# AdeeshKolluru/AdsorbDiff

Hardware: AMD Instinct MI355X
Metric: sampled adsorbate sites/sec (50 denoise steps, ~200-atom slabs) (higher is better)
Workload: dtype f32 (f16x3-split MFMA, fp32 accumulate; ADF_GEMM=f32 selects exact f32)

## Files before the change

adsorbdiff_amd/build.py:

```python
from __future__ import annotations

import os
import shutil
import subprocess
from pathlib import Path

PKG = Path(__file__).resolve().parent
CSRC = PKG / "csrc"
LIB = PKG / "libadsorbdiff_hip.so"
SOURCES = ["api.hip", "gemm.hip", "gemm16.hip", "graph.hip", "message.hip", "message_bwd.hip", "message_geo.hip", "energy_grad.hip", "rbf_wgrad.hip", "nodewise.hip", "stepper.hip", "peaks.hip", "collect.hip", "frames.hip", "train.hip", "optimizer.hip", "noising.hip", "s2ef_train.hip", "evaluate.hip", "incremental.hip", "eqv2_kernels.hip", "eqv2_gemm16.hip", "eqv2_api.hip", "lbfgs.hip", "active.hip", "anomaly.hip", "placement.hip", "unique.hip", "symmetry.hip", "sites.hip", "triangulate.hip", "voronoi.hip"]


def _hipcc() -> str:
    for cand in (os.environ.get("HIPCC"), shutil.which("hipcc"), "/opt/rocm/bin/hipcc"):
        if cand and Path(cand).exists():
            return cand
    raise RuntimeError("hipcc not found (set HIPCC or install ROCm)")


def needs_build() -> bool:
    if not LIB.exists():
        return True
    t = LIB.stat().st_mtime
    deps = [CSRC / s for s in SOURCES] + sorted(CSRC.glob("*.h")) + [PKG.parent / "include" / "adsorbdiff_hip.h"]
    return any(d.stat().st_mtime > t for d in deps)


FLAGS = [
    "--offload-arch=gfx950", "-O3", "-std=c++17", "-fPIC",
    "-fno-slp-vectorize",
]
EXTRA_FLAGS = {
    "lbfgs.hip": ["-ffp-contract=off"],
}
OBJ_DIR = CSRC / "build"


def _compile_one(args):
    cc, src, obj = args
    res = subprocess.run([cc, *FLAGS, *EXTRA_FLAGS.get(src.name, []), "-c", str(src), "-o", str(obj)],
                         capture_output=True, text=True)
    return src.name, res.returncode, res.stdout + res.stderr


def build(force: bool = False, verbose: bool = False) -> Path:
    if not force and not needs_build():
        return LIB
    from concurrent.futures import ThreadPoolExecutor

    cc = _hipcc()
    OBJ_DIR.mkdir(exist_ok=True)
    hdr_t = max([p.stat().st_mtime for p in CSRC.glob("*.h")] + [(PKG.parent / "include" / "adsorbdiff_hip.h").stat().st_mtime,
                                                                  Path(__file__).stat().st_mtime])
    jobs, objs = [], []
    for s in SOURCES:
        src, obj = CSRC / s, OBJ_DIR / (s + ".o")
        objs.append(obj)
        if force or not obj.exists() or obj.stat().st_mtime < max(src.stat().st_mtime, hdr_t):
            jobs.append((cc, src, obj))
    if verbose:
        print("compiling:", [j[1].name for j in jobs])
    with ThreadPoolExecutor(max_workers=min(8, max(1, len(jobs)))) as ex:
        for name, rc, out in ex.map(_compile_one, jobs):
            if rc != 0:
                raise RuntimeError(f"hipcc failed on {name}:\n{out}")
    res = subprocess.run([cc, "--offload-arch=gfx950", "-shared", "-fPIC", "-o", str(LIB)] + [str(o) for o in objs],
                         capture_output=True, text=True)
    if res.returncode != 0:
        raise RuntimeError(f"link failed:\n{res.stdout}\n{res.stderr}")
    return LIB


if __name__ == "__main__":
    print(build(force=True, verbose=True))
```

adsorbdiff_amd/csrc/api.hip:

```cpp
#include <stdarg.h>
#include <stdlib.h>
#include <string.h>

#include <new>

#include "common.h"

static thread_local char g_err[512] = "";

void adf_set_error(const char* fmt, ...) {
    va_list ap;
    va_start(ap, fmt);
    vsnprintf(g_err, sizeof(g_err), fmt, ap);
    va_end(ap);
}

extern "C" const char* adf_last_error(void) { return g_err; }
extern "C" const char* adf_version(void) { return "adsorbdiff_hip 0.5.0 (gfx950)"; }

adf_tune adf_tune_from_env() {
    auto off_is_0 = [](const char* name) { const char* e = getenv(name); return (e && atoi(e) == 0) ? 0 : 1; };
    auto is_f32 = [](const char* name) { const char* e = getenv(name); return e && strcmp(e, "f32") == 0; };
    adf_tune t = {};
    t.gemm_stream = off_is_0("ADF_GEMM_STREAM");
    t.head_gate_fused = off_is_0("ADF_HEAD_GATE_FUSED");
    t.lift_emit = off_is_0("ADF_LIFT_EMIT");
    t.graph_sys_csr = off_is_0("ADF_GRAPH_SYS_CSR");
    t.train_gemm16 = is_f32("ADF_TRAIN_GEMM") ? 0 : 1;
    t.wgrad_f32 = is_f32("ADF_WGRAD") ? 1 : 0;
    const char* gt = getenv("ADF_EQV2_GEMM_TILE");
    t.eqv2_gemm_tile256 = (gt && atoi(gt) == 128) ? 0 : 1;
    t.eqv2_rotin_generic = getenv("ADF_EQV2_ROTIN_GENERIC") != nullptr;
    t.eqv2_rotout_generic = getenv("ADF_EQV2_ROTOUT_GENERIC") != nullptr;
    return t;
}
const adf_tune& adf_tune_process() {
    static const adf_tune t = adf_tune_from_env();
    return t;
}
int adf_current_num_cus() {
    int dev = 0, n = 0;
    if (hipGetDevice(&dev) != hipSuccess || hipDeviceGetAttribute(&n, hipDeviceAttributeMultiprocessorCount, dev) != hipSuccess) return 0;
    return n;
}

extern "C" int32_t adf_profile_enable(adf_painn_t h, int32_t on) {
    if (!h) { adf_set_error("null handle"); return ADF_EINVAL; }
    h->prof.enable(on != 0);
    ADF_HIP_CHECK(hipMemset(h->kcount, 0, 8 * sizeof(unsigned long long)));
    return ADF_OK;
}

extern "C" int32_t adf_profile_read(adf_painn_t h, float* ms, int64_t* count, int64_t* message_ksteps, void* stream) {
    if (!h || !ms || !count) { adf_set_error("null argument"); return ADF_EINVAL; }
    ADF_HIP_CHECK(hipStreamSynchronize((hipStream_t)stream));
    if (message_ksteps) {
        unsigned long long k[8];
        ADF_HIP_CHECK(hipMemcpy(k, h->kcount, sizeof(k), hipMemcpyDeviceToHost));
        ADF_HIP_CHECK(hipMemset(h->kcount, 0, sizeof(k)));
        *message_ksteps = (int64_t)k[0];
    }
    return h->prof.read(ms, count, ADF_PROF_NCAT);
}

extern "C" int32_t adf_painn_create(const adf_painn_hparams* hp, adf_painn_t* out) {
    if (!hp || !out) { adf_set_error("null argument"); return ADF_EINVAL; }
    if (hp->hidden_channels % ADF_SLICE_CH != 0 || hp->hidden_channels < 128 || hp->hidden_channels > 1024) {
        adf_set_error("hidden_channels=%d must be a multiple of %d in [128,1024]", hp->hidden_channels, ADF_SLICE_CH);
        return ADF_EINVAL;
    }
    if (hp->num_rbf % 2 != 0 || hp->num_rbf > 128 || hp->num_rbf < 2) {
        adf_set_error("num_rbf=%d must be even and <= 128", hp->num_rbf);
        return ADF_EINVAL;
    }
    if (hp->max_neighbors < 1 || hp->max_neighbors > ADF_MAX_K) {
        adf_set_error("max_neighbors=%d must be in [1,%d]", hp->max_neighbors, ADF_MAX_K);
        return ADF_EINVAL;
    }
    if (hp->num_layers < 1 || hp->num_layers > 16 || hp->num_heads < 0 || hp->num_heads > 2) {
        adf_set_error("num_layers must be in [1,16], num_heads in [0,2]");
        return ADF_EINVAL;
    }
    adf_painn* h = new (std::nothrow) adf_painn();
    if (!h) { adf_set_error("host allocation failed"); return ADF_EOOM; }
    h->hp = *hp;
    hipDeviceProp_t prop;
    if (hipGetDevice(&h->device) != hipSuccess || hipGetDeviceProperties(&prop, h->device) != hipSuccess) {
        adf_set_error("no usable HIP device: %s", hipGetErrorString(hipGetLastError()));
        adf_painn_destroy(h);
        return ADF_EHIP;
    }
    h->num_cus = prop.multiProcessorCount;
    h->dist_floor = 1.0e-3f;
    {
        const char* e = getenv("ADF_INCREMENTAL");
        h->inc_on = !(e && e[0] == '0');
        const char* e2 = getenv("ADF_INC_SYNC");
        h->inc_sync = e2 && e2[0] == '1';
    }
    const int H = hp->hidden_channels, R = hp->num_rbf, L = hp->num_layers;
    adf_pool& m = h->m_life;
    int32_t st = m.alloc(&h->rbf_pack, (size_t)L * (H / ADF_SLICE_CH) * R * 192);
    if (st == ADF_OK) st = m.alloc(&h->rbf_bias_pack, (size_t)L * (H / ADF_SLICE_CH) * 192);
    if (st == ADF_OK) st = m.alloc(&h->rbf_pack16, (size_t)L * (H / ADF_SLICE_CH) * R * 192 * 2 * sizeof(uint16_t));
    if (st == ADF_OK) st = m.alloc(&h->rbf_bias_pack16, (size_t)L * (H / ADF_SLICE_CH) * 192);
    if (st == ADF_OK) st = m.alloc(&h->rbf_scales, 16);
    if (st == ADF_OK) st = m.alloc(&h->flags, ADF_NFLAGS);
    if (st == ADF_OK && hipMemset(h->flags, 0, sizeof(int32_t) * ADF_NFLAGS) != hipSuccess) st = ADF_EHIP;
    {
        const size_t HH = (size_t)H * H;
        const size_t per_layer = HH + 3 * HH + 2 * HH + 2 * HH + 3 * HH;
        const size_t per_head = HH + HH / 2 + 2 * HH + HH + HH / 4 + HH / 2;
        const size_t elems = (size_t)L * per_layer + (size_t)hp->num_heads * per_head;
        h->w16_bytes = elems * 2 * sizeof(uint16_t) + 4096;
        if (st == ADF_OK) st = m.alloc(&h->w16_arena, h->w16_bytes);
        if (st == ADF_OK) st = m.alloc(&h->w16_scales, 256);
        if (st == ADF_OK) st = m.alloc(&h->w16_bias_perm, (size_t)L * 2 * 3 * H);
        if (st == ADF_OK) st = m.alloc(&h->w16_scratch, 1);
        if (st == ADF_OK) st = m.alloc(&h->wfrag_arena, h->w16_bytes);
        const char* e = getenv("ADF_GEMM");
        h->gemm_f32 = e && strcmp(e, "f32") == 0;
        const char* el = getenv("ADF_LIFT");
        h->lift_on = !(el && strcmp(el, "0") == 0);
        const char* e2 = getenv("ADF_MSG");
        h->msg_f32 = e2 ? strcmp(e2, "f32") == 0 : h->gemm_f32;
        h->msg_f32_only = hp->num_rbf % 8 != 0;
        h->msg_f32 = h->msg_f32 || h->msg_f32_only;
        const char* er = getenv("ADF_ROW_MAXIMA");
        h->rmx = (er && atoi(er) == 0) ? 0 : 1;
        h->tune = adf_tune_from_env();
    }
    if (st == ADF_OK) st = m.alloc(&h->kcount, 8);
    if (st == ADF_OK && hipMemset(h->kcount, 0, 8 * sizeof(unsigned long long)) != hipSuccess) st = ADF_EHIP;
    if (st != ADF_OK) { adf_painn_destroy(h); return st; }
    *out = h;
    return ADF_OK;
}

static void inc_free(adf_painn* h) {
    h->m_inc.release();
    h->inc_tmp_bytes = 0;
    h->inc_capN = 0; h->inc_valid = false;
}

static void free_workspaces(adf_painn* h) {
    h->m_ws.release();
    h->inc_valid = false;
    h->scan_tmp_bytes = 0;
    h->lift.cap = 0; h->mag_v3_valid = false;
    h->xpart = h->catpart = h->vpart = nullptr; h->part_stride = 0;
    h->part_x = h->part_vec = nullptr; h->dbg_msg_rows = h->dbg_cat_rows = h->dbg_comb_rows = 0; h->dbg_mag = nullptr;
    h->cache_valid = false;
    h->capN = h->capB = h->capE = 0;
}

extern "C" int32_t adf_painn_destroy(adf_painn_t h) {
    if (!h) return ADF_OK;
    if (h->inc_cnt_host) (void)hipHostFree(h->inc_cnt_host);
    for (int i = 0; i < 2; ++i)
        if (h->inc_ev[i]) (void)hipEventDestroy((hipEvent_t)h->inc_ev[i]);
    adf_grad_free(h);
    delete h;
    return ADF_OK;
}

extern "C" int32_t adf_painn_set_weights(adf_painn_t h, int32_t n_weights, const void* const* w,
                                         const float* scale_factors, void* stream) {
    if (!h || !w || !scale_factors) { adf_set_error("null argument"); return ADF_EINVAL; }
    const int L = h->hp.num_layers;
    const int expect = 2 + ADF_WEIGHTS_PER_LAYER * L + ADF_WEIGHTS_PER_HEAD * h->hp.num_heads;
    if (n_weights != expect) {
        adf_set_error("expected %d weight tensors, got %d", expect, n_weights);
        return ADF_EINVAL;
    }
    for (int i = 0; i < n_weights; ++i)
        if (!w[i]) { adf_set_error("weight %d is null", i); return ADF_EINVAL; }
    auto f = [&](int i) { return reinterpret_cast<const float*>(w[i]); };
    h->emb = f(0);
    h->rbf_offset = f(1);
    int k = 2;
    for (int l = 0; l < L; ++l) {
        adf_layer_weights& lw = h->layer[l];
        lw.ln_w = f(k++); lw.ln_b = f(k++); lw.xp0_w = f(k++); lw.xp0_b = f(k++); lw.xp2_w = f(k++); lw.xp2_b = f(k++);
        lw.rbf_w = f(k++); lw.rbf_b = f(k++); lw.vp_w = f(k++); lw.xv0_w = f(k++); lw.xv0_b = f(k++);
        lw.xv2_w = f(k++); lw.xv2_b = f(k++);
        h->scale[l] = scale_factors[l];
    }
    for (int hd = 0; hd < h->hp.num_heads; ++hd)
        for (int b = 0; b < 2; ++b) {
            adf_block_weights& bw = h->head[hd][b];
            bw.vec1_w = f(k++); bw.vec2_w = f(k++); bw.un0_w = f(k++); bw.un0_b = f(k++); bw.un2_w = f(k++);
            bw.un2_b = f(k++);
        }
    ADF_TRY(adf_pack_rbf(h, (hipStream_t)stream));
    {
        hipStream_t s = (hipStream_t)stream;
        const long long H = h->hp.hidden_channels, HH = H * H;
        unsigned char* cur = h->w16_arena;
        unsigned char* fcur = h->wfrag_arena;
        int nscale = 0;
        float* bperm = h->w16_bias_perm;
        auto split = [&](const float* w, long long rows, long long K, adf_w16* out, const float* fused_bias = nullptr,
                         bool pair_perm = false) -> int32_t {
            const long long n = rows * K;
            out->hi = cur; cur += n * 2;
            out->lo = cur; cur += n * 2;
            out->inv_scale = h->w16_scales + nscale++;
            out->bias_perm = nullptr;
            out->frag = nullptr;
            if (fused_bias) {
                out->bias_perm = bperm; bperm += 3 * H;
                ADF_TRY(adf_split_weight(w, n, out, h->w16_scratch, s, (int)H, (int)H, fused_bias));
            } else if (pair_perm) {
                ADF_TRY(adf_split_weight(w, n, out, h->w16_scratch, s, (int)H, (int)H, nullptr, 2));
            } else {
                ADF_TRY(adf_split_weight(w, n, out, h->w16_scratch, s));
            }
            if (rows % 32 == 0 && K % 16 == 0) {
                out->frag = fcur; fcur += n * 4;
                ADF_TRY(adf_pack_frag(out, (int)rows, (int)K, out->frag, s));
            }
            return ADF_OK;
        };
        for (int l = 0; l < L; ++l) {
            adf_layer_weights& lw = h->layer[l];
            ADF_TRY(split(lw.xp0_w, H, H, &lw.xp0_16));
            ADF_TRY(split(lw.xp2_w, 3 * H, H, &lw.xp2_16, lw.xp2_b));
            ADF_TRY(split(lw.vp_w, 2 * H, H, &lw.vp_16, nullptr, true));
            ADF_TRY(split(lw.xv0_w, H, 2 * H, &lw.xv0_16));
            ADF_TRY(split(lw.xv2_w, 3 * H, H, &lw.xv2_16, lw.xv2_b));
        }
        for (int hd = 0; hd < h->hp.num_heads; ++hd) {
            adf_block_weights& b0 = h->head[hd][0];
            adf_block_weights& b1 = h->head[hd][1];
            ADF_TRY(split(b0.vec1_w, H, H, &b0.vec1_16));
            ADF_TRY(split(b0.vec2_w, H / 2, H, &b0.vec2_16));
            ADF_TRY(split(b0.un0_w, H, 2 * H, &b0.un0_16));
            ADF_TRY(split(b0.un2_w, H, H, &b0.un2_16));
            ADF_TRY(split(b1.vec1_w, H / 2, H / 2, &b1.vec1_16));
            ADF_TRY(split(b1.un0_w, H / 2, H, &b1.un0_16));
        }
        if ((size_t)(cur - h->w16_arena) > h->w16_bytes || (size_t)(fcur - h->wfrag_arena) > h->w16_bytes || nscale > 256) {
            adf_set_error("internal: fp16 weight arena overflow");
            return ADF_EINVAL;
        }
    }
    h->weights_set = true;
    h->rec0_valid = false;
    h->inc_valid = false;
    adf_grad_invalidate(h);
    return ADF_OK;
}

static int32_t ensure_capacity(adf_painn* h, int64_t N, int64_t B) {
    if (N <= h->capN && B <= h->capB) return ADF_OK;
    const int64_t capN = N > h->capN ? N : h->capN;
    const int64_t capB = B > h->capB ? B : h->capB;
    ADF_HIP_CHECK(hipDeviceSynchronize());
    free_workspaces(h);
    const int64_t H = h->hp.hidden_channels, K = h->hp.max_neighbors;
    const int64_t capE = 2 * capN * K;
    int32_t st = ADF_OK;
#define ALLOC(field, count) if (st == ADF_OK) st = h->m_ws.alloc(&h->field, (size_t)(count))
    ALLOC(nbr_cnt, capN);
    ALLOC(nbr_src, capN * K);
    ALLOC(nbr_shift, capN * K);
    ALLOC(cache_d2, capN * K);
    ALLOC(cache_cid, capN * K);
    ALLOC(cache_cnt, capN);
    ALLOC(deg, capN + 1);
    ALLOC(nptr, capN + 1);
    ALLOC(cursor, capN);
    ALLOC(img_cnt, capB);
    ALLOC(sys_slow, capB);
    ALLOC(e_src, capE);
    ALLOC(e_geom, capE);
    if (h->inc_on) {
        ALLOC(prev_nptr, capN + 1);
        ALLOC(prev_src, capE);
        ALLOC(prev_geom, capE);
    }
    if (st == ADF_OK) {
        h->scan_tmp_bytes = adf_scan_temp_bytes(capN + 1);
        st = h->m_ws.alloc(&h->scan_tmp, h->scan_tmp_bytes + 16);
    }
    ALLOC(x, capN * H);
    ALLOC(vecA, capN * 3 * H);
    ALLOC(vecB, capN * 3 * H);
    ALLOC(rec, (capN + 1) * 5 * H);
    ALLOC(y, capN * H);
    ALLOC(xh, capN * 3 * H);
    ALLOC(vv, capN * 6 * H);
    ALLOC(cat, capN * 2 * H);
    ALLOC(dot, capN * H);
    ALLOC(sys, capB * 16);
    ALLOC(lift.buf, capN * 3);
    ALLOC(mag_a, capN);
    ALLOC(mag_b, capN);
    ALLOC(mag_v3, capN * 3);
    const int64_t ps = (capN + 31) / 32 * 32, ns = H / ADF_SLICE_CH;
    if (h->rmx) ALLOC(rmx_part, (4 * ns + H / 32 + 4) * ps);
#undef ALLOC
    h->lift.cap = st == ADF_OK ? capN * 3 : 0;
    if (st != ADF_OK) { free_workspaces(h); return st; }
    if (h->rmx) {
        h->part_stride = ps;
        h->xpart = h->rmx_part; h->catpart = h->xpart + ns * ps; h->vpart = h->catpart + (H / 32) * ps;
        h->dbg_mag = h->vpart + 3 * ns * ps;
    }
    h->capN = capN; h->capB = capB; h->capE = capE;
    return ADF_OK;
}

static int32_t check_batch(const adf_painn* h, const adf_batch* b) {
    if (!h || !b) { adf_set_error("null argument"); return ADF_EINVAL; }
    if (b->num_atoms <= 0 || b->num_systems <= 0) { adf_set_error("empty batch"); return ADF_EINVAL; }
    if (!b->pos || !b->cell || !b->batch || !b->atom_offset) { adf_set_error("null batch array"); return ADF_EINVAL; }
    for (int k = 0; k < 3; ++k)
        if (b->reps[k] < 0 || b->reps[k] > 16) { adf_set_error("reps[%d]=%d out of range", k, b->reps[k]); return ADF_EINVAL; }
    return ADF_OK;
}

static int32_t read_flags(adf_painn* h, hipStream_t s) {
    int32_t f[ADF_NFLAGS];
    ADF_HIP_CHECK(hipMemcpyAsync(f, h->flags, sizeof(f), hipMemcpyDeviceToHost, s));
    ADF_HIP_CHECK(hipMemsetAsync(h->flags, 0, sizeof(f), s));
    ADF_HIP_CHECK(hipStreamSynchronize(s));
    if (f[4]) { adf_set_error("atomic number outside [1, %d] (rows of the embedding table)", h->hp.num_elements); return ADF_EINVAL; }
    if (f[0]) { adf_set_error("a centre atom has more than %d in-cutoff candidates", ADF_MAX_CAND); return ADF_EOVERFLOW; }
    if (f[2]) { adf_set_error("edge buffer overflow"); return ADF_EOVERFLOW; }
    if (f[3]) { adf_set_error("an atom has more than %d incoming edges", ADF_MAX_INDEG); return ADF_EOVERFLOW; }
    if (f[1]) { adf_set_error("An image has no neighbors"); return ADF_ENONEIGHBOR; }
    if (f[6]) { adf_set_error("energy gradient: an edge row has no reverse row in its partner's segment (asymmetric graph)"); return ADF_EINVAL; }
    if (f[5]) {
        adf_set_error("non-finite model output%s", h->gemm_f32 ? " (exact-f32 arithmetic: the inputs or weights are not finite)"
                      : " in f16x3 arithmetic: an activation left the fp16 range or the inputs are not finite; "
                        "adf_painn_set_arithmetic(h, 1) selects exact f32");
        return ADF_ENUMERIC;
    }
    return ADF_OK;
}

extern "C" int32_t adf_graph_set_moving(adf_painn_t h, const int32_t* moving, const int32_t* mov_idx,
                                        const int32_t* mov_off) {
    if (!h) { adf_set_error("null handle"); return ADF_EINVAL; }
    if (moving && (!mov_idx || !mov_off)) { adf_set_error("moving mask needs mov_idx and mov_off"); return ADF_EINVAL; }
    h->moving = moving; h->mov_idx = mov_idx; h->mov_off = mov_off;
    ADF_HIP_CHECK(hipMemset(h->flags, 0, sizeof(int32_t) * ADF_NFLAGS));
    h->cache_valid = false;
    h->rec0_valid = false;
    h->inc_valid = false;
    return ADF_OK;
}

extern "C" int32_t adf_graph_build(adf_painn_t h, const adf_batch* b, void* stream, int64_t* num_edges) {
    ADF_TRY(check_batch(h, b));
    ADF_TRY(ensure_capacity(h, b->num_atoms, b->num_systems));
    hipStream_t s = (hipStream_t)stream;
    ADF_TRY(adf_graph_build_impl(h, b, s));
    if (num_edges) {
        int32_t e = 0;
        ADF_HIP_CHECK(hipMemcpyAsync(&e, h->nptr + b->num_atoms, sizeof(int32_t), hipMemcpyDeviceToHost, s));
        ADF_TRY(read_flags(h, s));
        *num_edges = e;
    }
    return ADF_OK;
}

__global__ void adf_export_edges_kernel(const int32_t* nptr, const int32_t* e_src, const float4* eg, int N,
                                        int32_t* src, int32_t* dst, float* dist, float* vec, long long cap) {
    const int n = blockIdx.x * 4 + (threadIdx.x >> 6);
    if (n >= N) return;
    for (int e = nptr[n] + (threadIdx.x & 63); e < nptr[n + 1]; e += 64) {
        if (e >= cap) continue;
        if (src) src[e] = e_src[e];
        if (dst) dst[e] = n;
        const float4 q = eg[e];
        if (dist) dist[e] = q.w;
        if (vec) { vec[3 * (size_t)e] = q.x; vec[3 * (size_t)e + 1] = q.y; vec[3 * (size_t)e + 2] = q.z; }
    }
}

__global__ void adf_export_shift_kernel(const int32_t* nbr_shift, int32_t* out, long long n, int r0, int r1, int r2) {
    const long long i = (long long)blockIdx.x * blockDim.x + threadIdx.x;
    if (i >= n) return;
    const int c = nbr_shift[i];
    const int n2 = 2 * r2 + 1, n1 = 2 * r1 + 1;
    const int ia = c / (n1 * n2), rem = c - ia * (n1 * n2);
    out[3 * i] = ia - r0;
    out[3 * i + 1] = rem / n2 - r1;
    out[3 * i + 2] = rem % n2 - r2;
}

extern "C" int32_t adf_graph_export(adf_painn_t h, int32_t* nbr_count, int32_t* nbr_src, int32_t* nbr_shift,
                                    int64_t edge_capacity, int32_t* edge_src, int32_t* edge_dst, float* edge_dist,
                                    float* edge_vec, int64_t* num_edges, void* stream) {
    if (!h || h->lastN <= 0) { adf_set_error("no graph built"); return ADF_EINVAL; }
    hipStream_t s = (hipStream_t)stream;
    const int64_t N = h->lastN, K = h->hp.max_neighbors;
    if (nbr_count) ADF_HIP_CHECK(hipMemcpyAsync(nbr_count, h->nbr_cnt, sizeof(int32_t) * N, hipMemcpyDeviceToDevice, s));
    if (nbr_src) ADF_HIP_CHECK(hipMemcpyAsync(nbr_src, h->nbr_src, sizeof(int32_t) * N * K, hipMemcpyDeviceToDevice, s));
    if (nbr_shift)
        hipLaunchKernelGGL(adf_export_shift_kernel, dim3((unsigned)((N * K + 255) / 256)), dim3(256), 0, s, h->nbr_shift,
                           nbr_shift, (long long)(N * K), h->last_reps[0], h->last_reps[1], h->last_reps[2]);
    if (edge_src || edge_dst || edge_dist || edge_vec)
        hipLaunchKernelGGL(adf_export_edges_kernel, dim3((unsigned)((N + 3) / 4)), dim3(256), 0, s, h->nptr, h->e_src,
                           h->e_geom, (int)N, edge_src, edge_dst, edge_dist, edge_vec, (long long)edge_capacity);
    ADF_HIP_CHECK(hipGetLastError());
    int32_t e = 0;
    ADF_HIP_CHECK(hipMemcpyAsync(&e, h->nptr + N, sizeof(int32_t), hipMemcpyDeviceToHost, s));
    ADF_HIP_CHECK(hipStreamSynchronize(s));
    if (num_edges) *num_edges = e;
    return ADF_OK;
}

static int32_t zero_pad_rows(adf_painn* h, int N, hipStream_t s) {
    const size_t row = (size_t)5 * h->hp.hidden_channels;
    ADF_HIP_CHECK(hipMemsetAsync(h->rec + (size_t)N * row, 0, sizeof(float) * row, s));
    return ADF_OK;
}

static int32_t make_records(adf_painn* h, int l, int n, const float* x, const float* vec, bool vec_is_zero, float* rec,
                            const int32_t* row_map, hipStream_t s) {
    const int H = h->hp.hidden_channels;
    const adf_layer_weights& w = h->layer[l];
    if (n <= 0) return ADF_OK;
    adf_prof_begin(h, ADF_PROF_NODE, s);
    const bool lift = h->lift_on && !h->gemm_f32;
    const bool em = lift && h->tune.lift_emit;
    ADF_TRY(adf_nodewise_layernorm(x, w.ln_w, w.ln_b, h->y, n, H, s, em ? h->mag_a : nullptr, h->rows_dev));
    ADF_TRY(adf_linear(h, h->y, H, w.xp0_w, &w.xp0_16, w.xp0_b, h->cat, H, n, H, H, 1, s, em ? h->mag_a : nullptr,
                       em ? h->mag_b : nullptr));
    if (h->gemm_f32) {
        if (row_map) { adf_set_error("internal: mapped records need the f16x3 path"); return ADF_EINVAL; }
        ADF_TRY(adf_launch_gemm(h->cat, H, w.xp2_w, H, w.xp2_b, h->xh, 3 * H, n, 3 * H, H, 0, s));
        ADF_TRY(adf_pack_records(h, n, h->xh, vec, vec_is_zero, s, rec));
    } else {
        adf_epi ep = {};
        ep.vec_in = vec; ep.rec = rec ? rec : h->rec; ep.H = H; ep.vec_is_zero = vec_is_zero ? 1 : 0;
        ep.row_map = row_map;
        ep.rmag = em ? h->mag_b : nullptr;
        ep.m_dev = h->rows_dev;
        ADF_TRY(adf_launch_gemm16_fused(h->cat, H, &w.xp2_16, n, H, H, 1, &ep, s, h->tune, lift ? &h->lift : nullptr));
    }
    adf_prof_end(h, s);
    return ADF_OK;
}

static int32_t message_layer(adf_painn* h, int l, int N, const float* x, const float* vec, float* x_out,
                             float* vec_out, bool vec_is_zero, hipStream_t s, const int32_t* tlist = nullptr,
                             int n_targets = 0, float* rec = nullptr, bool records_ready = false) {
    if (!records_ready) ADF_TRY(make_records(h, l, N, x, vec, vec_is_zero, rec, nullptr, s));
    adf_prof_begin(h, ADF_PROF_MESSAGE, s);
    const int items = tlist ? n_targets : N;
    const bool emit = h->rmx && h->lift_on && !h->gemm_f32 && !h->msg_f32 && items > 0 && items <= h->part_stride;
    h->part_x = h->part_vec = nullptr;
    const int32_t st = adf_message_impl(h, l, N, x, h->xh, vec, x_out, vec_out, vec_is_zero, s, tlist, n_targets, rec,
                                        tlist ? h->rows_dev : nullptr, emit ? h->xpart : nullptr, h->vpart, h->part_stride);
    if (st == ADF_OK && emit) {
        h->part_x = x_out; h->part_vec = vec_out; h->part_n = items; h->part_dev = tlist ? h->rows_dev : nullptr;
        h->dbg_msg_rows = items;
    }
    adf_prof_end(h, s);
    return st;
}

static int32_t update_layer(adf_painn* h, int l, int N, float* x, float* vec, hipStream_t s, bool from_message = true) {
    const int H = h->hp.hidden_channels;
    const adf_layer_weights& w = h->layer[l];
    adf_prof_begin(h, ADF_PROF_NODE, s);
    const bool parts = from_message && h->rmx && h->lift_on && !h->gemm_f32 && N > 0 && h->part_x == x && h->part_vec == vec &&
                       h->part_n == N && h->part_dev == h->rows_dev;
    h->part_x = h->part_vec = nullptr;
    if (h->gemm_f32) {
        ADF_TRY(adf_launch_gemm(vec, H, w.vp_w, H, nullptr, h->vv, 2 * H, 3 * N, 2 * H, H, 0, s));
        ADF_TRY(adf_nodewise_update_prep(h->vv, x, h->cat, h->dot, N, H, s));
        ADF_TRY(adf_linear(h, h->cat, 2 * H, w.xv0_w, &w.xv0_16, w.xv0_b, h->y, H, N, H, 2 * H, 1, s));
    } else {
        adf_epi ep = {};
        ep.v1 = h->vv; ep.dotw = h->dot; ep.cat = h->cat; ep.H = H; ep.m_dev = h->rows_dev;
        const adf_lift* lf = h->lift_on ? &h->lift : nullptr;
        if (parts) {
            ADF_TRY(adf_launch_rowmax_combine(h->vpart, 3 * h->part_stride, H / ADF_SLICE_CH, 3ll * N, h->lift.buf, s, h->rows_dev, 3));
            ep.rmag = h->lift.buf;
            if (h->dbg_capture) ADF_HIP_CHECK(hipMemcpyAsync(h->dbg_mag, h->lift.buf, sizeof(float) * 3 * (size_t)N, hipMemcpyDeviceToDevice, s));
        }
        if (parts || (h->dbg_capture && h->rmx && lf && N <= h->part_stride)) {
            ep.catpart = h->catpart; ep.part_stride = h->part_stride; h->dbg_cat_rows = N;
        }
        ADF_TRY(adf_launch_gemm16_fused(vec, H, &w.vp_16, N, H, H, 3, &ep, s, h->tune, lf));
        if (parts) {
            ADF_TRY(adf_launch_rowmax_combine(h->xpart, h->part_stride, H / ADF_SLICE_CH + H / 32, N, h->lift.buf, s, h->rows_dev, 1));
            if (h->dbg_capture) {
                ADF_HIP_CHECK(hipMemcpyAsync(h->dbg_mag + 3 * h->part_stride, h->lift.buf, sizeof(float) * (size_t)N, hipMemcpyDeviceToDevice, s));
                h->dbg_comb_rows = N;
            }
        }
        adf_epi e0 = {};
        e0.A2 = h->cat; e0.K1 = H; e0.m_dev = h->rows_dev;
        e0.rmag = parts ? h->lift.buf : nullptr;
        e0.out_mag = h->lift_on ? reinterpret_cast<unsigned int*>(h->mag_b) : nullptr;
        ADF_TRY(adf_launch_gemm16(x, H, &w.xv0_16, w.xv0_b, h->y, H, N, H, 2 * H, 1, &e0, s, lf, h->tune, h->num_cus));
    }
    int32_t st;
    if (h->gemm_f32) {
        ADF_TRY(adf_launch_gemm(h->y, H, w.xv2_w, H, w.xv2_b, h->xh, 3 * H, N, 3 * H, H, 0, s));
        st = adf_nodewise_update_apply(h->xh, h->dot, h->vv, x, vec, h->scale[l], N, H, s);
    } else {
        adf_epi ep = {};
// ... 158 lines not shown
    const size_t cap = (size_t)h->inc_capN, row = (size_t)5 * H;
    if (out_idx && n_out == 0) return ADF_OK;
    adf_prof_begin(h, ADF_PROF_GRAPH, s);
    if (first) {
        ADF_TRY(adf_nodewise_embed(h, Z, N, h->incX[0], s));
        for (int l = 0; l < L; ++l) ADF_HIP_CHECK(hipMemsetAsync(h->incR[l] + (size_t)N * row, 0, sizeof(float) * row, s));
        ADF_HIP_CHECK(hipMemsetAsync(h->inc_pend, 0, cap * L, s));
    } else {
        ADF_TRY(adf_inc_compare(h, N, s));
    }
    ADF_HIP_CHECK(hipMemsetAsync(h->inc_cnt, 0, sizeof(int32_t) * (2 * ADF_MAX_LAYERS + 1), s));
    if (out_idx) ADF_TRY(adf_inc_need_from_list(h, N, L, out_idx, n_out, s));
    for (int l = 0; l < L; ++l) ADF_TRY(adf_inc_plan_layer(h, l, N, first, out_idx != nullptr, s));
    ADF_HIP_CHECK(hipMemcpyAsync(h->inc_cnt + 2 * L, h->nptr + N, sizeof(int32_t), hipMemcpyDeviceToDevice, s));
    const int slot = h->inc_slot;
    h->inc_slot ^= 1;
    if (h->inc_ev_live[slot]) ADF_TRY(inc_harvest(h, slot, true));
    int32_t* host = h->inc_cnt_host + (size_t)slot * (2 * ADF_MAX_LAYERS + 1);
    ADF_HIP_CHECK(hipMemcpyAsync(host, h->inc_cnt, sizeof(int32_t) * (2 * L + 1), hipMemcpyDeviceToHost, s));
    ADF_HIP_CHECK(hipEventRecord((hipEvent_t)h->inc_ev[slot], s));
    h->inc_ev_live[slot] = true;
    h->inc_pend_N[slot] = N;
    ADF_TRY(inc_harvest(h, slot ^ 1, false));
    if (h->inc_sync) ADF_TRY(inc_harvest(h, slot, true, true));
    adf_prof_end(h, s);
    if (first) ADF_TRY(make_records(h, 0, N, h->incX[0], nullptr, true, h->incR[0], nullptr, s));
    for (int l = 0; l < L; ++l) {
        const int n_seen = h->inc_seen_valid ? h->inc_seen[l] : N;
        const bool whole = first || !h->inc_seen_valid || h->inc_pend_Nseen != N || (long long)n_seen * 10 >= (long long)N * 9;
        h->inc_pend_whole[slot][l] = whole ? 1 : 0;
        if (h->inc_sync && !whole && n_seen == 0) continue;
        const float* vin = l == 0 ? h->vecA : h->incV[l];
        if (whole) {
            ADF_TRY(message_layer(h, l, N, h->incX[l], vin, h->incX[l + 1], h->incV[l + 1], l == 0, s, nullptr, 0,
                                  h->incR[l], true));
            ADF_TRY(update_layer(h, l, N, h->incX[l + 1], h->incV[l + 1], s));
            if (l + 1 < L)
                ADF_TRY(make_records(h, l + 1, N, h->incX[l + 1], h->incV[l + 1], false, h->incR[l + 1], nullptr, s));
            continue;
        }
        const int32_t* list = h->inc_list + cap * l;
        const int ncap = h->inc_sync ? n_seen : N;
        h->rows_dev = h->inc_cnt + l;
        int32_t st = message_layer(h, l, N, h->incX[l], vin, h->x, h->vecB, l == 0, s, list, ncap, h->incR[l], true);
        if (st == ADF_OK) st = update_layer(h, l, ncap, h->x, h->vecB, s);
        if (st == ADF_OK) {
            adf_prof_begin(h, ADF_PROF_NODE, s);
            st = adf_inc_scatter_rows(h->x, list, ncap, H, h->incX[l + 1], s, h->rows_dev);
            if (st == ADF_OK) st = adf_inc_scatter_rows(h->vecB, list, ncap, 3 * H, h->incV[l + 1], s, h->rows_dev);
            adf_prof_end(h, s);
        }
        if (st == ADF_OK && l + 1 < L) st = make_records(h, l + 1, ncap, h->x, h->vecB, false, h->incR[l + 1], list, s);
        h->rows_dev = nullptr;
        ADF_TRY(st);
    }
    adf_prof_begin(h, ADF_PROF_HEADS, s);
    if (!out_idx) {
        if (heads >= 1) ADF_TRY(adf_head_forward(h, 0, N, h->incX[L], h->incV[L], f1, s));
        if (heads == 2) ADF_TRY(adf_head_forward(h, 1, N, h->incX[L], h->incV[L], f2, s));
        h->x_last = h->incX[L];
    } else {
        ADF_TRY(ensure_subset(h, n_out));
        ADF_TRY(adf_inc_gather_rows(h->incX[L], out_idx, n_out, H, h->sub_x, s));
        ADF_TRY(adf_inc_gather_rows(h->incV[L], out_idx, n_out, 3 * H, h->sub_vec, s));
        for (int hd = 0; hd < heads; ++hd) {
            ADF_TRY(adf_head_forward(h, hd, n_out, h->sub_x, h->sub_vec, h->sub_f, s));
            hipLaunchKernelGGL(adf_scatter_rows3_kernel, dim3((3 * n_out + 255) / 256), dim3(256), 0, s, h->sub_f, out_idx,
                               n_out, hd == 0 ? f1 : f2);
        }
        ADF_HIP_CHECK(hipGetLastError());
    }
    adf_prof_end(h, s);
    h->inc_valid = true;
    return ADF_OK;
}

static int32_t forward_impl(adf_painn_t h, const adf_batch* b, const int32_t* out_idx, int32_t n_out, float* f1,
                            float* f2, void* stream, bool head1_only = false) {
    ADF_TRY(check_batch(h, b));
    if (!h->weights_set) { adf_set_error("weights not set"); return ADF_EINVAL; }
    const int heads = head1_only ? 1 : h->hp.num_heads;
    if (heads > h->hp.num_heads) { adf_set_error("the model has no force head"); return ADF_EINVAL; }
    if (!b->atomic_numbers || (heads >= 1 && !f1) || (heads == 2 && !f2)) { adf_set_error("null argument"); return ADF_EINVAL; }
    h->x_last = nullptr;
    hipStream_t s = (hipStream_t)stream;
    const int N = b->num_atoms;
    ADF_TRY(ensure_capacity(h, N, b->num_systems));
    const int inc = inc_prepare(h, N);
    adf_prof_begin(h, ADF_PROF_GRAPH, s);
    ADF_TRY(adf_graph_build_impl(h, b, s));
    adf_prof_end(h, s);
    if (inc) {
        h->inc_serial = h->build_serial;
        return forward_incremental(h, N, b->atomic_numbers, out_idx, n_out, f1, f2, inc == 2, heads, s);
    }
    ADF_TRY(zero_pad_rows(h, N, s));
    ADF_TRY(adf_nodewise_embed(h, b->atomic_numbers, N, h->x, s));
    float* vin = h->vecA;
    float* vout = h->vecB;
    const int L = h->hp.num_layers, H = h->hp.hidden_channels;
    float* rec0 = nullptr;
    bool rec0_ready = false;
    if (h->moving) {
        const size_t row = (size_t)5 * H;
        if ((int64_t)N + 1 > h->rec0_cap) {
            h->rec0_cap = 0; h->rec0_valid = false;
            ADF_TRY(h->m_rec0.alloc(&h->rec0, ((size_t)N + 1) * row));
            h->rec0_cap = (int64_t)N + 1;
        }
        rec0 = h->rec0;
        rec0_ready = h->rec0_valid && h->rec0_N == N;
        if (!rec0_ready) ADF_HIP_CHECK(hipMemsetAsync(rec0 + (size_t)N * row, 0, sizeof(float) * row, s));
        h->rec0_valid = true; h->rec0_N = N;
    }
    if (!out_idx) {
        for (int l = 0; l < L; ++l) {
            if (l == 0) ADF_TRY(message_layer(h, 0, N, h->x, vin, h->x, vout, true, s, nullptr, 0, rec0, rec0_ready));
            else
            ADF_TRY(message_layer(h, l, N, h->x, vin, h->x, vout, l == 0, s));
            ADF_TRY(update_layer(h, l, N, h->x, vout, s));
            float* t = vin; vin = vout; vout = t;
        }
        adf_prof_begin(h, ADF_PROF_HEADS, s);
        if (heads >= 1) ADF_TRY(adf_head_forward(h, 0, N, h->x, vin, f1, s));
        if (heads == 2) ADF_TRY(adf_head_forward(h, 1, N, h->x, vin, f2, s));
        adf_prof_end(h, s);
        h->x_last = h->x;
        return ADF_OK;
    }
    if (n_out == 0) return ADF_OK;
    ADF_TRY(ensure_subset(h, n_out));
    for (int l = 0; l + 1 < L; ++l) {
        if (l == 0) ADF_TRY(message_layer(h, 0, N, h->x, vin, h->x, vout, true, s, nullptr, 0, rec0, rec0_ready));
        else
        ADF_TRY(message_layer(h, l, N, h->x, vin, h->x, vout, l == 0, s));
        ADF_TRY(update_layer(h, l, N, h->x, vout, s));
        float* t = vin; vin = vout; vout = t;
    }
    ADF_TRY(message_layer(h, L - 1, N, h->x, vin, h->sub_x, h->sub_vec, L == 1, s, out_idx, n_out,
                          L == 1 ? rec0 : nullptr, L == 1 && rec0_ready));
    ADF_TRY(update_layer(h, L - 1, n_out, h->sub_x, h->sub_vec, s));
    adf_prof_begin(h, ADF_PROF_HEADS, s);
    for (int hd = 0; hd < heads; ++hd) {
        ADF_TRY(adf_head_forward(h, hd, n_out, h->sub_x, h->sub_vec, h->sub_f, s));
        hipLaunchKernelGGL(adf_scatter_rows3_kernel, dim3((3 * n_out + 255) / 256), dim3(256), 0, s, h->sub_f, out_idx,
                           n_out, hd == 0 ? f1 : f2);
    }
    ADF_HIP_CHECK(hipGetLastError());
    adf_prof_end(h, s);
    return ADF_OK;
}

extern "C" int32_t adf_painn_forward(adf_painn_t h, const adf_batch* b, float* f1, float* f2, void* stream) {
    return forward_impl(h, b, nullptr, 0, f1, f2, stream);
}

extern "C" int32_t adf_painn_forward_subset(adf_painn_t h, const adf_batch* b, const int32_t* out_idx, int32_t n_out,
                                            float* f1, float* f2, void* stream) {
    if (!out_idx || n_out < 0) { adf_set_error("forward_subset: null index list"); return ADF_EINVAL; }
    return forward_impl(h, b, out_idx, n_out, f1, f2, stream);
}

extern "C" int32_t adf_painn_set_energy_head(adf_painn_t h, int32_t n_weights, const void* const* w, void* stream) {
    if (!h || !w) { adf_set_error("null argument"); return ADF_EINVAL; }
    if (n_weights != 4) { adf_set_error("set_energy_head: expected 4 tensors (out_energy.0.weight/bias, out_energy.2.weight/bias), got %d", n_weights); return ADF_EINVAL; }
    for (int i = 0; i < 4; ++i)
        if (!w[i]) { adf_set_error("energy-head tensor %d is null", i); return ADF_EINVAL; }
    const int H = h->hp.hidden_channels, H2 = H / 2;
    const size_t n = (size_t)H2 * H;
    if (!h->oe0_buf) ADF_TRY(h->m_life.alloc(&h->oe0_buf, n * 4 + 64));
    h->oe0_w = reinterpret_cast<const float*>(w[0]);
    h->oe0_b = reinterpret_cast<const float*>(w[1]);
    h->oe2_w = reinterpret_cast<const float*>(w[2]);
    h->oe2_b = reinterpret_cast<const float*>(w[3]);
    adf_w16& e = h->oe0_16;
    e = adf_w16{};
    e.hi = h->oe0_buf; e.lo = h->oe0_buf + n * 2; e.inv_scale = reinterpret_cast<float*>(h->oe0_buf + n * 4);
    ADF_TRY(adf_split_weight(h->oe0_w, (long long)n, &e, reinterpret_cast<unsigned int*>(h->oe0_buf + n * 4 + 16),
                             (hipStream_t)stream));
    h->energy_set = true;
    adf_grad_invalidate(h);
    return ADF_OK;
}

extern "C" int32_t adf_painn_set_distance_floor(adf_painn_t h, float floor) {
    if (!h || !(floor > 0.f)) { adf_set_error("set_distance_floor: null handle or non-positive floor"); return ADF_EINVAL; }
    if (floor != h->dist_floor) {
        h->dist_floor = floor;
        h->cache_valid = false;
        h->rec0_valid = false;
        h->inc_valid = false;
    }
    return ADF_OK;
}

__global__ __launch_bounds__(256) void adf_energy_sum_kernel(const float* __restrict__ y, int H2, const float* __restrict__ w,
                                                             const float* __restrict__ bias, const int32_t* __restrict__ atom_offset,
                                                             float* __restrict__ energy) {
    __shared__ float part[4];
    const int b = blockIdx.x, lane = threadIdx.x & 63, wave = threadIdx.x >> 6;
    const int a0 = atom_offset[b], a1 = atom_offset[b + 1];
    const float b0 = bias[0];
    float acc = 0.f;
    for (int a = a0 + wave; a < a1; a += 4) {
        const float* row = y + (size_t)a * H2;
        float d = 0.f;
        for (int c = lane; c < H2; c += 64) d = fmaf(row[c], w[c], d);
        d = adf_wave_sum(d);
        acc = __fadd_rn(acc, __fadd_rn(d, b0));
    }
    if (lane == 0) part[wave] = acc;
    __syncthreads();
    if (threadIdx.x == 0) energy[b] = __fadd_rn(__fadd_rn(part[0], part[1]), __fadd_rn(part[2], part[3]));
}

int32_t adf_energy_sum(const float* y, int H2, const float* w, const float* bias, const int32_t* atom_offset, float* energy,
                       int num_systems, hipStream_t s) {
    hipLaunchKernelGGL(adf_energy_sum_kernel, dim3(num_systems), dim3(256), 0, s, y, H2, w, bias, atom_offset, energy);
    ADF_HIP_CHECK(hipGetLastError());
    return ADF_OK;
}

extern "C" int32_t adf_painn_forward_energy(adf_painn_t h, const adf_batch* b, float* energy, float* forces, void* stream) {
    ADF_TRY(check_batch(h, b));
    if (!h->energy_set) { adf_set_error("forward_energy: energy head not set (adf_painn_set_energy_head)"); return ADF_EINVAL; }
    if (!energy || (h->hp.num_heads >= 1 && !forces)) { adf_set_error("forward_energy: null output"); return ADF_EINVAL; }
    if (h->hp.num_heads > 1) { adf_set_error("forward_energy: the S2EF model has one force head"); return ADF_EINVAL; }
    hipStream_t s = (hipStream_t)stream;
    ADF_TRY(forward_impl(h, b, nullptr, 0, forces, nullptr, stream));
    if (!h->x_last) { adf_set_error("internal: no node features after the forward"); return ADF_EINVAL; }
    const int N = b->num_atoms, H = h->hp.hidden_channels, H2 = H / 2;
    adf_prof_begin(h, ADF_PROF_HEADS, s);
    ADF_TRY(adf_linear(h, h->x_last, H, h->oe0_w, &h->oe0_16, h->oe0_b, h->y, H2, N, H2, H, 1, s));
    ADF_TRY(adf_energy_sum(h->y, H2, h->oe2_w, h->oe2_b, b->atom_offset, energy, b->num_systems, s));
    adf_prof_end(h, s);
    return ADF_OK;
}

extern "C" int32_t adf_linear_forward(const float* A, const float* W, const float* bias, float* C, int32_t M,
                                      int32_t N, int32_t K, int32_t act_ssilu, int32_t mode, void* stream) {
    hipStream_t s = (hipStream_t)stream;
    if (!A || !W || !C || M <= 0 || N <= 0 || K <= 0) { adf_set_error("bad argument"); return ADF_EINVAL; }
    if (mode == 0) return adf_launch_gemm(A, K, W, K, bias, C, N, M, N, K, act_ssilu, s);
    adf_pool tmp;
    unsigned char* buf = nullptr;
    const size_t n = (size_t)N * K;
    ADF_TRY(tmp.alloc(&buf, n * 4 + 64));
    adf_w16 w16 = {};
    w16.hi = buf; w16.lo = buf + n * 2; w16.inv_scale = reinterpret_cast<float*>(buf + n * 4);
    unsigned int* scratch = reinterpret_cast<unsigned int*>(buf + n * 4 + 16);
    int32_t st = adf_split_weight(W, (long long)n, &w16, scratch, s);
    float* mags = nullptr;
    const char* el = getenv("ADF_LIFT");
    const bool lift = !(el && strcmp(el, "0") == 0);
    if (st == ADF_OK && lift) st = tmp.alloc(&mags, (size_t)M);
    adf_lift lf = {mags, M};
    if (st == ADF_OK) st = adf_launch_gemm16(A, K, &w16, bias, C, N, M, N, K, act_ssilu, nullptr, s, lift ? &lf : nullptr,
                                             adf_tune_process(), adf_current_num_cus());
    (void)hipStreamSynchronize(s);
    return st;
}

extern "C" int32_t adf_painn_set_arithmetic(adf_painn_t h, int32_t exact_f32) {
    if (!h) { adf_set_error("null handle"); return ADF_EINVAL; }
    h->gemm_f32 = exact_f32 != 0;
    h->msg_f32 = exact_f32 != 0 || h->msg_f32_only;
    h->rec0_valid = false;
    h->inc_valid = false;
    return ADF_OK;
}

extern "C" int32_t adf_painn_set_incremental(adf_painn_t h, int32_t on) {
    if (!h) { adf_set_error("null handle"); return ADF_EINVAL; }
    if ((on != 0) != h->inc_on) {
        ADF_HIP_CHECK(hipDeviceSynchronize());
        h->inc_on = on != 0;
        if (!h->inc_on) inc_free(h);
        if (h->inc_on && h->capN > 0 && !h->prev_nptr) {
            int32_t st = h->m_ws.alloc(&h->prev_nptr, (size_t)h->capN + 1);
            if (st == ADF_OK) st = h->m_ws.alloc(&h->prev_src, (size_t)h->capE);
            if (st == ADF_OK) st = h->m_ws.alloc(&h->prev_geom, (size_t)h->capE);
            if (st != ADF_OK) { h->inc_on = false; return st; }
        }
    }
    h->inc_valid = false;
    (void)inc_harvest(h, h->inc_slot, true);
    (void)inc_harvest(h, h->inc_slot ^ 1, true);
    h->inc_seen_valid = false;
    h->inc_rows = h->inc_rows_full = h->inc_edges = h->inc_launches = 0;
    return ADF_OK;
}

extern "C" int32_t adf_check_flags(adf_painn_t h, void* stream) {
    if (!h) { adf_set_error("null handle"); return ADF_EINVAL; }
    return read_flags(h, (hipStream_t)stream);
}

static int32_t model_check(void* h, const adf_batch* b) { return check_batch((adf_painn*)h, b); }
static int32_t model_grow(void* h, const adf_batch* b, float** sys) {
    adf_painn* p = (adf_painn*)h;
    ADF_TRY(ensure_capacity(p, b->num_atoms, b->num_systems));
    *sys = p->sys;
    return ADF_OK;
}
static int32_t model_forward(void* h, const adf_batch* b, const int32_t* out_idx, int32_t n_out, float* f1, float* f2,
                             hipStream_t s) {
    return forward_impl((adf_painn*)h, b, out_idx, out_idx ? n_out : 0, f1, f2, s, !f2);
}
static void model_prof(void* h, bool begin, hipStream_t s) {
    if (begin) adf_prof_begin((adf_painn*)h, ADF_PROF_STEPPER, s);
    else adf_prof_end((adf_painn*)h, s);
}
static adf_model model(adf_painn_t h) {
    return {h, model_check, model_grow, model_forward, model_prof, h ? h->ps_state : nullptr, h ? h->ps_B : 0};
}

extern "C" int32_t adf_painn_set_per_system_stop(adf_painn_t h, int32_t* sys_state, int32_t B) {
    if (!h) { adf_set_error("null handle"); return ADF_EINVAL; }
    return adf_model_set_per_system_stop(&h->ps_state, &h->ps_B, sys_state, B);
}

extern "C" int32_t adf_sde_init_placement(adf_painn_t h, const adf_batch* b, float* pos, const int32_t* tags,
                                          const float* noise, void* stream) {
    return adf_model_init_placement(model(h), b, pos, tags, noise, (hipStream_t)stream);
}

extern "C" int32_t adf_sde_step(adf_painn_t h, const adf_batch* b, float* pos, const int32_t* tags,
                                const int32_t* fixed, const float* f1, const float* f2, const adf_step_coef* coef,
                                const float* z_tr, const float* z_rot, int32_t early_stop_count, int32_t* state,
                                float* dcom, float* drot, void* stream) {
    return adf_model_sde_step(model(h), b, pos, tags, fixed, f1, f2, coef, nullptr, 0, z_tr, z_rot, early_stop_count, state,
                              dcom, drot, (hipStream_t)stream);
}

extern "C" int32_t adf_sde_step_scheduled(adf_painn_t h, const adf_batch* b, float* pos, const int32_t* tags,
                                          const int32_t* fixed, const float* f1, const float* f2,
                                          const adf_step_coef* coefs_dev, int32_t num_steps, const float* z_tr,
                                          const float* z_rot, int32_t early_stop_count, int32_t* state, float* dcom,
                                          float* drot, void* stream) {
    return adf_model_sde_step(model(h), b, pos, tags, fixed, f1, f2, nullptr, coefs_dev, num_steps, z_tr, z_rot,
                              early_stop_count, state, dcom, drot, (hipStream_t)stream);
}

extern "C" int32_t adf_sample(adf_painn_t h, const adf_batch* b, float* pos, const int32_t* tags, const int32_t* fixed,
                              const adf_step_coef* coefs_dev, int32_t num_steps, const float* z_tr_all,
                              const float* z_rot_all, int32_t early_stop_count, int32_t poll_every, int32_t* state,
                              const int32_t* out_idx, int32_t n_out, float* f1, float* f2, void* stream) {
    return adf_model_sample(model(h), b, pos, tags, fixed, coefs_dev, num_steps, z_tr_all, z_rot_all, early_stop_count,
                            poll_every, state, out_idx, n_out, f1, f2, nullptr, 0, (hipStream_t)stream);
}

extern "C" int32_t adf_sample_traj(adf_painn_t h, const adf_batch* b, float* pos, const int32_t* tags, const int32_t* fixed,
                                   const adf_step_coef* coefs_dev, int32_t num_steps, const float* z_tr_all,
                                   const float* z_rot_all, int32_t early_stop_count, int32_t poll_every, int32_t* state,
                                   const int32_t* out_idx, int32_t n_out, float* f1, float* f2, adf_frames_t sink,
                                   int32_t frame_every, void* stream) {
    if (!sink) { adf_set_error("sample_traj: null sink"); return ADF_EINVAL; }
    return adf_model_sample(model(h), b, pos, tags, fixed, coefs_dev, num_steps, z_tr_all, z_rot_all, early_stop_count,
                            poll_every, state, out_idx, n_out, f1, f2, sink, frame_every, (hipStream_t)stream);
}

extern "C" int32_t adf_tr_step(adf_painn_t h, const adf_batch* b, float* pos, const int32_t* tags, const float* f1,
                               const adf_tr_coef* coef, const adf_tr_coef* coefs_dev, int32_t num_steps, const float* z,
                               int32_t early_stop_count, int32_t* state, float* dcom, void* stream) {
    return adf_model_tr_step(model(h), b, pos, tags, f1, coef, coefs_dev, num_steps, z, early_stop_count, state, dcom,
                             (hipStream_t)stream);
}

extern "C" int32_t adf_tr_sample(adf_painn_t h, const adf_batch* b, float* pos, const int32_t* tags,
                                 const adf_tr_coef* coefs_dev, int32_t num_steps, const float* z_all,
                                 int32_t early_stop_count, int32_t poll_every, int32_t* state, const int32_t* out_idx,
                                 int32_t n_out, float* f1, void* stream) {
    return adf_model_tr_sample(model(h), b, pos, tags, coefs_dev, num_steps, z_all, early_stop_count, poll_every, state,
                               out_idx, n_out, f1, nullptr, 0, (hipStream_t)stream);
}

extern "C" int32_t adf_tr_sample_traj(adf_painn_t h, const adf_batch* b, float* pos, const int32_t* tags,
                                      const adf_tr_coef* coefs_dev, int32_t num_steps, const float* z_all,
                                      int32_t early_stop_count, int32_t poll_every, int32_t* state, const int32_t* out_idx,
                                      int32_t n_out, float* f1, adf_frames_t sink, int32_t frame_every, void* stream) {
    if (!sink) { adf_set_error("tr_sample_traj: null sink"); return ADF_EINVAL; }
    return adf_model_tr_sample(model(h), b, pos, tags, coefs_dev, num_steps, z_all, early_stop_count, poll_every, state,
                               out_idx, n_out, f1, sink, frame_every, (hipStream_t)stream);
}

extern "C" int32_t adf_get_counters(adf_painn_t h, adf_counters* out, void* stream) {
    if (!h || !out || h->lastN <= 0) { adf_set_error("no forward has run"); return ADF_EINVAL; }
    hipStream_t s = (hipStream_t)stream;
    const int64_t N = h->lastN, H = h->hp.hidden_channels, R = h->hp.num_rbf, L = h->hp.num_layers;
    int32_t e = 0;
    ADF_HIP_CHECK(hipMemcpyAsync(&e, h->nptr + N, sizeof(int32_t), hipMemcpyDeviceToHost, s));
    ADF_HIP_CHECK(hipStreamSynchronize(s));
    const int64_t E = e;
    out->num_edges = E;
    out->num_atoms = N;
    out->message_bytes_per_layer = E * (3 * H * 4 + 12 + 8) + N * (3 * H * 4 + 3 * H * 4) + N * (H * 4 + 3 * H * 4);
    const int64_t head = 2 * (3 * N * H * H + 3 * N * H * H / 2 + N * 2 * H * H + N * H * H + 3 * N * (H / 2) * (H / 2) +
                              N * H * H / 2);
    out->dense_flops = L * (30 * H * H * N + 2 * R * 3 * H * E) + h->hp.num_heads * head;
    ADF_TRY(inc_harvest(h, h->inc_slot, true));
    ADF_TRY(inc_harvest(h, h->inc_slot ^ 1, true));
    out->inc_rows = (int64_t)h->inc_rows; out->inc_rows_full = (int64_t)h->inc_rows_full;
    out->inc_msg_launches = (int64_t)h->inc_launches; out->inc_msg_edges = (int64_t)h->inc_edges;
    return ADF_OK;
}
```

adsorbdiff_amd/csrc/base.h:

```cpp
#pragma once
#include <hip/hip_runtime.h>
#include <stdint.h>
#include <stdio.h>
#include <string>
#include <vector>

#include "../../include/adsorbdiff_hip.h"

void adf_set_error(const char* fmt, ...);

#define ADF_HIP_CHECK(expr)                                                             \
    do {                                                                                \
        hipError_t _e = (expr);                                                         \
        if (_e != hipSuccess) {                                                         \
            adf_set_error("%s failed: %s (%s:%d)", #expr, hipGetErrorString(_e),        \
                          __FILE__, __LINE__);                                          \
            return (_e == hipErrorOutOfMemory) ? ADF_EOOM : ADF_EHIP;                   \
        }                                                                               \
    } while (0)

#define ADF_TRY(expr)                     \
    do {                                  \
        int32_t _s = (expr);              \
        if (_s != ADF_OK) return _s;      \
    } while (0)

struct adf_pool {
    std::vector<void**> slots;
    adf_pool() = default;
    adf_pool(const adf_pool&) = delete;
    adf_pool& operator=(const adf_pool&) = delete;
    ~adf_pool() { release(); }
    int32_t alloc(void** field, size_t bytes) {
        bool known = false;
        for (void** s : slots) known = known || s == field;
        if (known) { if (*field) (void)hipFree(*field); } else slots.push_back(field);
        *field = nullptr;
        if (bytes == 0) bytes = 16;
        const hipError_t e = hipMalloc(field, bytes);
        if (e == hipSuccess) return ADF_OK;
        *field = nullptr;
        (void)hipGetLastError();
        adf_set_error("device allocation of %zu bytes failed: %s", bytes, hipGetErrorString(e));
        return ADF_EOOM;
    }
    template <typename T>
    int32_t alloc(T** field, size_t count) { return alloc(reinterpret_cast<void**>(field), count * sizeof(T)); }
    void release() {
        for (void** s : slots) {
            if (*s) (void)hipFree(*s);
            *s = nullptr;
        }
        slots.clear();
    }
};

struct adf_prof {
    bool on = false;
    bool open = false;
    std::vector<hipEvent_t> ev;
    std::vector<int> cat;
    size_t used = 0;
    adf_prof() = default;
    adf_prof(const adf_prof&) = delete;
    adf_prof& operator=(const adf_prof&) = delete;
    ~adf_prof() { for (hipEvent_t e : ev) (void)hipEventDestroy(e); }
    void begin(int c, hipStream_t s) {
        open = false;
        if (!on) return;
        if (used + 2 > ev.size())
            for (int i = 0; i < 512; ++i) {
                hipEvent_t e;
                if (hipEventCreate(&e) != hipSuccess) { (void)hipGetLastError(); break; }
                ev.push_back(e);
            }
        if (used + 2 > ev.size()) return;
        cat.resize(used / 2);
        cat.push_back(c);
        (void)hipEventRecord(ev[used], s);
        open = true;
    }
    void end(hipStream_t s) {
        if (!on || !open) return;
        (void)hipEventRecord(ev[used + 1], s);
        used += 2;
        open = false;
    }
    void enable(bool o) { on = o; open = false; used = 0; cat.clear(); }
    int32_t read(float* ms, int64_t* count, int ncat) {
        for (int c = 0; c < ncat; ++c) { ms[c] = 0.f; count[c] = 0; }
        for (size_t i = 0; i < used; i += 2) {
            float t = 0.f;
            ADF_HIP_CHECK(hipEventElapsedTime(&t, ev[i], ev[i + 1]));
            ms[cat[i / 2]] += t;
            count[cat[i / 2]] += 1;
        }
        enable(on);
        return ADF_OK;
    }
    struct scope {
        adf_prof& p; hipStream_t s;
        scope(adf_prof& p_, int c, hipStream_t s_) : p(p_), s(s_) { p.begin(c, s); }
        ~scope() { p.end(s); }
    };
};
```

adsorbdiff_amd/csrc/common.h:

```cpp
#pragma once
#include "base.h"
#include "arith.h"
#include "lanes.h"

#define ADF_GROUP_NODES 32
#define ADF_SLICE_CH 64
#define ADF_MAX_CAND 1024
#define ADF_MAX_K 128
#define ADF_NFLAGS 8
#define ADF_MAX_INDEG 1024
#define ADF_MAX_LAYERS 16

struct adf_w16 {
    void* hi;
    void* lo;
    float* inv_scale;
    float* bias_perm;
    void* frag;
};
struct adf_epi {
    const float* vec_in;
    float* rec;
    float* x;
    float* vec;
    const float* dot;
    const float* vv;
    float* v1;
    float* dotw;
    float* cat;
    float scale;
    int H;
    int vec_is_zero;
    const float* A2;
    int K1;
    const int32_t* row_map;
    const float* rmag;
    unsigned int* out_mag;
    const int32_t* m_dev;
    int accumulate;
    const float* gate;
    int gate_ld;
    float* catpart;
    long long part_stride;
};
struct adf_lift {
    float* buf;
    long long cap;
};
struct adf_layer_weights {
    const float *ln_w, *ln_b, *xp0_w, *xp0_b, *xp2_w, *xp2_b, *rbf_w, *rbf_b;
    const float *vp_w, *xv0_w, *xv0_b, *xv2_w, *xv2_b;
    adf_w16 xp0_16, xp2_16, vp_16, xv0_16, xv2_16;
};
struct adf_block_weights {
    const float *vec1_w, *vec2_w, *un0_w, *un0_b, *un2_w, *un2_b;
    adf_w16 vec1_16, vec2_16, un0_16, un2_16;
};

struct adf_painn {
    adf_painn_hparams hp;
    int device;
    bool weights_set;
    const float* emb;
    const float* rbf_offset;
    adf_layer_weights layer[16];
    adf_block_weights head[2][2];
    float scale[16];
    float* rbf_pack;
    float* rbf_bias_pack;
    void* rbf_pack16;
    float* rbf_bias_pack16;
    float* rbf_scales;
    unsigned char* w16_arena;
    size_t w16_bytes;
    float* w16_scales;
    float* w16_bias_perm;
    unsigned int* w16_scratch;
    unsigned char* wfrag_arena;
    bool gemm_f32;
    bool msg_f32;
    bool msg_f32_only;
    adf_tune tune;
    bool lift_on;
    adf_lift lift;
    float *mag_a, *mag_b;
    float* mag_v3;
    bool mag_v3_valid;
    int rmx;
    float* rmx_part;
    float *xpart, *catpart, *vpart;
    int64_t part_stride;
    const float *part_x, *part_vec;
    int part_n;
    const int32_t* part_dev;
    int dbg_msg_rows, dbg_cat_rows;
    bool dbg_capture;
    float* dbg_mag;
    int dbg_comb_rows;

    int64_t capN, capB, capE;
    int32_t* nbr_cnt;
    int32_t* nbr_src;
    int32_t* nbr_shift;
    int32_t* deg;
    int32_t* nptr;
    int32_t* cursor;
    int32_t* img_cnt;
    int32_t* sys_slow;
    void* scan_tmp;
    size_t scan_tmp_bytes;
    const int32_t* moving;
    const int32_t* mov_idx;
    const int32_t* mov_off;
    float* cache_d2;
    int32_t* cache_cid;
    int32_t* cache_cnt;
    bool cache_valid;
    int32_t* e_src;
    float4* e_geom;
    int32_t* flags;
    float *x, *vecA, *vecB, *y, *xh, *vv, *cat, *dot;
    float* rec;
    bool rbf_uniform;
    float* rec0;
    int64_t rec0_cap, rec0_N;
    bool rec0_valid;
    bool inc_on;
    bool inc_valid;
    int64_t inc_capN, inc_N;
    int inc_layers;
    float* incX[ADF_MAX_LAYERS + 1];
    float* incV[ADF_MAX_LAYERS + 1];
    float* incR[ADF_MAX_LAYERS];
    int32_t *prev_nptr, *prev_src;
    float4* prev_geom;
    unsigned char *inc_c0, *inc_chg;
    unsigned char *inc_pend, *inc_need, *inc_tf;
    int32_t* inc_list;
    int32_t* inc_cnt;
    int32_t* inc_cnt_host;
    void* inc_ev[2];
    bool inc_ev_live[2];
    int inc_slot;
    bool inc_sync;
    int32_t inc_seen[2 * ADF_MAX_LAYERS + 1];
    bool inc_seen_valid;
    unsigned char inc_pend_whole[2][ADF_MAX_LAYERS];
    int32_t inc_pend_N[2];
    int32_t inc_pend_Nseen;
    const int32_t* rows_dev;
    void* inc_tmp; size_t inc_tmp_bytes;
    unsigned long long inc_rows, inc_rows_full, inc_edges, inc_launches;
    unsigned long long build_serial, inc_serial;
    float *sub_x, *sub_vec, *sub_f;
    int64_t capS;
    float* sys;
    int32_t* ps_state = nullptr; int32_t ps_B = 0;
    const float *oe0_w, *oe0_b, *oe2_w, *oe2_b;
    adf_w16 oe0_16;
    unsigned char* oe0_buf;
    bool energy_set;
    const float* x_last;
    float dist_floor;
    void* grad;
    int64_t lastN, lastB;
    int32_t last_reps[3];
    int num_cus;
    adf_prof prof;
    unsigned long long* kcount;
    adf_pool m_life;
    adf_pool m_ws;
    adf_pool m_inc;
    adf_pool m_sub;
    adf_pool m_rec0;
};

enum { ADF_PROF_GRAPH = 0, ADF_PROF_MESSAGE = 1, ADF_PROF_NODE = 2, ADF_PROF_HEADS = 3, ADF_PROF_STEPPER = 4 };
static inline void adf_prof_begin(adf_painn* h, int cat, hipStream_t s) { h->prof.begin(cat, s); }
static inline void adf_prof_end(adf_painn* h, hipStream_t s) { h->prof.end(s); }

int32_t adf_launch_gemm(const float* A, int lda, const float* W, int ldw, const float* bias, float* C, int ldc,
                        int M, int N, int K, int act_ssilu, hipStream_t s);
adf_tune adf_tune_from_env();
const adf_tune& adf_tune_process();
int adf_current_num_cus();
int32_t adf_launch_gemm16(const float* A, int lda, const adf_w16* W, const float* bias, float* C, int ldc, int M,
                          int N, int K, int act_ssilu, const adf_epi* ep, hipStream_t s, const adf_lift* lf,
                          const adf_tune& tune, int num_cus);
int32_t adf_launch_rowmag(const float* A, int lda, int K1, const float* A2, int K2, long long M, float* mag, hipStream_t s,
                          const int32_t* m_dev = nullptr, int m_mul = 1);
int32_t adf_launch_rowmax_combine(const float* part, long long stride, int nparts, long long M, float* mag, hipStream_t s,
                                  const int32_t* m_dev = nullptr, int m_mul = 1);
int32_t adf_split_weight(const float* w, long long n, adf_w16* out, unsigned int* scratch_bits, hipStream_t s,
                         int perm_H = 0, int K = 0, const float* bias = nullptr, int parts = 3);
int32_t adf_launch_gemm16_vecnorm(const float* A, int lda, const adf_w16* W, float* nrm, int M, int N, int K,
                                  hipStream_t s, const adf_tune& tune, const adf_lift* lf = nullptr,
                                  const float* premag = nullptr);
int32_t adf_launch_gemm16_fused(const float* A, int lda, const adf_w16* W, int M, int H, int K, int epi,
                                const adf_epi* ep, hipStream_t s, const adf_tune& tune, const adf_lift* lf = nullptr);
static inline int32_t adf_linear(const adf_painn* h, const float* A, int lda, const float* W, const adf_w16* W16,
                                 const float* bias, float* C, int ldc, int M, int N, int K, int act, hipStream_t s,
                                 const float* premag = nullptr, float* out_mag = nullptr) {
    if (h->gemm_f32) return adf_launch_gemm(A, lda, W, K, bias, C, ldc, M, N, K, act, s);
    adf_epi ep = {};
    ep.m_dev = h->rows_dev;
    if (h->lift_on) { ep.rmag = premag; ep.out_mag = reinterpret_cast<unsigned int*>(out_mag); }
    return adf_launch_gemm16(A, lda, W16, bias, C, ldc, M, N, K, act, &ep, s, h->lift_on ? &h->lift : nullptr, h->tune,
                             h->num_cus);
}
int32_t adf_pack_frag(const adf_w16* w, int N, int K, void* out, hipStream_t s);
int32_t adf_graph_build_impl(adf_painn* h, const adf_batch* b, hipStream_t s);
int32_t adf_energy_sum(const float* y, int H2, const float* w, const float* bias, const int32_t* atom_offset, float* energy,
                       int num_systems, hipStream_t s);
void adf_grad_invalidate(adf_painn* h);
void adf_grad_free(adf_painn* h);
bool adf_message_geo_supported(const adf_painn* h);
int32_t adf_message_geo(adf_painn* h, int layer, const float* xh, const float* vec, bool vec_is_zero, float4* part,
                        long long ecap, bool accumulate, hipStream_t s);
size_t adf_inc_temp_bytes(int64_t n);
int32_t adf_inc_compare(adf_painn* h, int N, hipStream_t s);
int32_t adf_inc_need_from_list(adf_painn* h, int N, int L, const int32_t* out_idx, int n_out, hipStream_t s);
int32_t adf_inc_plan_layer(adf_painn* h, int l, int N, bool first, bool have_need, hipStream_t s);
int32_t adf_inc_scatter_rows(const float* src, const int32_t* idx, int n, int width, float* dst, hipStream_t s,
                             const int32_t* n_dev = nullptr);
int32_t adf_inc_gather_rows(const float* src, const int32_t* idx, int n, int width, float* dst, hipStream_t s);
size_t adf_scan_temp_bytes(int64_t n);
int32_t adf_message_impl(adf_painn* h, int layer, int N, const float* x, const float* xh, const float* vec,
                         float* x_out, float* vec_out, bool vec_is_zero, hipStream_t s,
                         const int32_t* tlist = nullptr, int n_targets = 0, const float* rec = nullptr,
                         const int32_t* n_targets_dev = nullptr,
                         float* xpart = nullptr, float* vpart = nullptr, long long part_stride = 0);
int32_t adf_pack_rbf(adf_painn* h, hipStream_t s);
int32_t adf_pack_rbf_layer(adf_painn* h, int l, hipStream_t s);
int32_t adf_pack_records(adf_painn* h, int N, const float* xh, const float* vec, bool vec_is_zero, hipStream_t s,
                         float* rec = nullptr);
int32_t adf_nodewise_embed(adf_painn* h, const int32_t* Z, int N, float* x, hipStream_t s);
int32_t adf_nodewise_layernorm(const float* x, const float* w, const float* b, float* y, int N, int H, hipStream_t s,
                               float* out_mag = nullptr, const int32_t* n_dev = nullptr);
int32_t adf_nodewise_update_prep(const float* vv, const float* x, float* cat, float* dot, int N, int H, hipStream_t s);
int32_t adf_nodewise_update_apply(const float* h3, const float* dot, const float* vv, float* x, float* vec,
                                  float scale, int N, int H, hipStream_t s);
int32_t adf_head_forward(adf_painn* h, int head, int N, const float* x, const float* vec, float* out, hipStream_t s);
int32_t adf_stepper_init(const adf_batch* b, float* pos, const int32_t* tags, const float* noise,
                         hipStream_t s);
int32_t adf_stepper_step(float* sys, const adf_batch* b, float* pos, const int32_t* tags, const int32_t* fixed,
                         const float* f1, const float* f2, const adf_step_coef* coef, const adf_step_coef* coefs_dev,
                         int num_steps, const float* z_tr, const float* z_rot, int32_t early_stop_count,
                         int32_t* state, float* dcom, float* drot, hipStream_t s, int32_t* sys_state = nullptr);
int32_t adf_stepper_tr_step(float* sys, const adf_batch* b, float* pos, const int32_t* tags, const float* f1,
                            const adf_tr_coef* coef, const adf_tr_coef* coefs_dev, int num_steps, const float* z,
                            int32_t early_stop_count, int32_t* state, float* dcom, hipStream_t s,
                            int32_t* sys_state = nullptr);

struct adf_model {
    void* h;
    int32_t (*check)(void* h, const adf_batch* b);
    int32_t (*grow)(void* h, const adf_batch* b, float** sys);
    int32_t (*forward)(void* h, const adf_batch* b, const int32_t* out_idx, int32_t n_out, float* f1, float* f2,
                       hipStream_t s);
    void (*prof)(void* h, bool begin, hipStream_t s);
    int32_t* sys_state;
    int32_t sys_B;
};
int32_t adf_model_set_per_system_stop(int32_t** slot, int32_t* slot_B, int32_t* sys_state, int32_t B);
int32_t adf_frames_push_impl(adf_frames* f, const float* src, hipStream_t s);
int32_t adf_model_init_placement(const adf_model& m, const adf_batch* b, float* pos, const int32_t* tags,
                                 const float* noise, hipStream_t s);
int32_t adf_model_sde_step(const adf_model& m, const adf_batch* b, float* pos, const int32_t* tags, const int32_t* fixed,
                           const float* f1, const float* f2, const adf_step_coef* coef, const adf_step_coef* coefs_dev,
                           int32_t num_steps, const float* z_tr, const float* z_rot, int32_t early_stop_count,
                           int32_t* state, float* dcom, float* drot, hipStream_t s);
int32_t adf_model_tr_step(const adf_model& m, const adf_batch* b, float* pos, const int32_t* tags, const float* f1,
                          const adf_tr_coef* coef, const adf_tr_coef* coefs_dev, int32_t num_steps, const float* z,
                          int32_t early_stop_count, int32_t* state, float* dcom, hipStream_t s);
int32_t adf_model_sample(const adf_model& m, const adf_batch* b, float* pos, const int32_t* tags, const int32_t* fixed,
                         const adf_step_coef* coefs_dev, int32_t num_steps, const float* z_tr_all, const float* z_rot_all,
                         int32_t early_stop_count, int32_t poll_every, int32_t* state, const int32_t* out_idx,
                         int32_t n_out, float* f1, float* f2, adf_frames* sink, int32_t frame_every, hipStream_t s);
int32_t adf_model_tr_sample(const adf_model& m, const adf_batch* b, float* pos, const int32_t* tags,
                            const adf_tr_coef* coefs_dev, int32_t num_steps, const float* z_all, int32_t early_stop_count,
                            int32_t poll_every, int32_t* state, const int32_t* out_idx, int32_t n_out, float* f1,
                            adf_frames* sink, int32_t frame_every, hipStream_t s);
```

adsorbdiff_amd/csrc/stepper.hip:

```cpp
#include "common.h"

struct StepParams {
    const float* cell;
    const int32_t* atom_offset;
    const int32_t* tags;
    const int32_t* fixed;
    float* pos;
    const float* f1;
    const float* f2;
    const float* z_tr;
    const float* z_rot;
    float* sys;
    int32_t* state;
    float* dcom_out;
    float* drot_out;
    int B;
    adf_step_coef c;
    const adf_step_coef* coefs_dev;
    int num_steps;
    int early_stop_count;
};

__device__ __forceinline__ float pymod1(float x) {
    float r = fmodf(x, 1.0f);
    if (r < 0.f) r += 1.0f;
    return r;
}

__device__ void solve3(const float* A, const float* v, float* f) {
    float m[3][4];
    for (int r = 0; r < 3; ++r) { for (int c = 0; c < 3; ++c) m[r][c] = A[3 * r + c]; m[r][3] = v[r]; }
    for (int col = 0; col < 3; ++col) {
        int piv = col;
        for (int r = col + 1; r < 3; ++r) if (fabsf(m[r][col]) > fabsf(m[piv][col])) piv = r;
        if (piv != col) for (int c = 0; c < 4; ++c) { float t = m[col][c]; m[col][c] = m[piv][c]; m[piv][c] = t; }
        for (int r = col + 1; r < 3; ++r) {
            const float l = m[r][col] / m[col][col];
            for (int c = col; c < 4; ++c) m[r][c] = m[r][c] - l * m[col][c];
        }
    }
    f[2] = m[2][3] / m[2][2];
    f[1] = (m[1][3] - m[1][2] * f[2]) / m[1][1];
    f[0] = (m[0][3] - m[0][1] * f[1] - m[0][2] * f[2]) / m[0][0];
}

__global__ __launch_bounds__(64) void adf_init_placement_kernel(const float* cell, const int32_t* atom_offset,
                                                                 const int32_t* tags, float* pos, const float* noise,
                                                                 int B) {
    const int b = blockIdx.x, lane = threadIdx.x;
    const int a0 = atom_offset[b], a1 = atom_offset[b + 1];
    float sx = 0.f, sy = 0.f, sz = 0.f, cnt = 0.f;
    for (int a = a0 + lane; a < a1; a += 64)
        if (tags[a] == 2) { sx += pos[3 * a]; sy += pos[3 * a + 1]; sz += pos[3 * a + 2]; cnt += 1.f; }
    sx = adf_wave_sum(sx); sy = adf_wave_sum(sy); sz = adf_wave_sum(sz); cnt = adf_wave_sum(cnt);
    const float inv = 1.0f / fmaxf(cnt, 1.0f);
    const float cx = sx * inv, cy = sy * inv, cz = sz * inv;
    const float* cl = cell + 9 * b;
    const float* nz = noise + 3 * b;
    const float nx = cl[0] * nz[0] + cl[1] * nz[1] + cl[2] * nz[2];
    const float ny = cl[3] * nz[0] + cl[4] * nz[1] + cl[5] * nz[2];
    (void)cz;
    for (int a = a0 + lane; a < a1; a += 64)
        if (tags[a] == 2) {
            pos[3 * a] = (pos[3 * a] - cx) + nx;
            pos[3 * a + 1] = (pos[3 * a + 1] - cy) + ny;
            pos[3 * a + 2] = (pos[3 * a + 2] - cz) + cz;
        }
}

__device__ __forceinline__ void step_sums(const StepParams& p, int a0, int a1, int lane, float* s) {
#pragma unroll
    for (int i = 0; i < 10; ++i) s[i] = 0.f;
    for (int a = a0 + lane; a < a1; a += 64)
        if (p.tags[a] == 2) {
            const float keep = (p.fixed && p.fixed[a] == 1) ? 0.f : 1.f;
            s[0] += p.pos[3 * a]; s[1] += p.pos[3 * a + 1]; s[2] += p.pos[3 * a + 2];
            s[3] += p.f1[3 * a]; s[4] += p.f1[3 * a + 1]; s[5] += p.f1[3 * a + 2];
            s[6] += p.f2[3 * a] * keep; s[7] += p.f2[3 * a + 1] * keep; s[8] += p.f2[3 * a + 2] * keep;
            s[9] += 1.f;
        }
#pragma unroll
    for (int i = 0; i < 10; ++i) s[i] = adf_wave_sum(s[i]);
}

__device__ __forceinline__ bool step_wrap(const float* cl, const float* tgt, const float* com, float* dcom) {
    float fr[3];
    solve3(cl, tgt, fr);
    for (int k = 0; k < 3; ++k) fr[k] = pymod1(pymod1(fr[k]));
    bool conv = true;
    for (int j = 0; j < 3; ++j) {
        const float w = cl[3 * j] * fr[0] + cl[3 * j + 1] * fr[1] + cl[3 * j + 2] * fr[2];
        dcom[j] = w - com[j];
        conv = conv && (fabsf(dcom[j]) <= 1.0e-3f);
    }
    return conv;
}

__device__ __forceinline__ bool step_increment(const StepParams& p, int b, const float* s, float* com, float* dcom,
                                               float* drot) {
    const float cnt = fmaxf(s[9], 1.0f);
    adf_step_coef c = p.c;
    if (p.coefs_dev) c = p.coefs_dev[min(p.state[4], p.num_steps - 1)];
    for (int k = 0; k < 3; ++k) {
        com[k] = s[k] / cnt;
        const float str = s[3 + k] / cnt;
        const float srot = s[6 + k] / cnt;
        float d = __fmul_rn(c.coef_tr, str);
        float r = __fmul_rn(__fmul_rn(__fmul_rn(c.rot_pre, srot), c.rot_dt), c.rot_g2);
        if (p.z_tr) d = __fadd_rn(d, __fmul_rn(c.noise_tr, p.z_tr[3 * b + k]));
        if (p.z_rot) r = __fadd_rn(r, __fmul_rn(c.noise_rot, p.z_rot[3 * b + k]));
        dcom[k] = d;
        drot[k] = r;
    }
    dcom[2] = 0.f;
    const float tgt[3] = {com[0] + dcom[0], com[1] + dcom[1], com[2] + dcom[2]};
    return step_wrap(p.cell + 9 * b, tgt, com, dcom);
}

__device__ __forceinline__ void step_rigid_update(float* pos, const int32_t* tags, int a0, int a1, int lane, float cx,
                                                  float cy, float cz, float tx, float ty, float tz, float ax, float ay,
                                                  float az) {
    const float ang = sqrtf(ax * ax + ay * ay + az * az);
    const float half = 0.5f * ang;
    float k;
    if (fabsf(ang) < 1e-6f) k = 0.5f - (ang * ang) / 48.0f;
    else k = sinf(half) / ang;
    const float qr = cosf(half), qi = ax * k, qj = ay * k, qk = az * k;
    const float two_s = 2.0f / (qr * qr + qi * qi + qj * qj + qk * qk);
    const float R00 = 1 - two_s * (qj * qj + qk * qk), R01 = two_s * (qi * qj - qk * qr), R02 = two_s * (qi * qk + qj * qr);
    const float R10 = two_s * (qi * qj + qk * qr), R11 = 1 - two_s * (qi * qi + qk * qk), R12 = two_s * (qj * qk - qi * qr);
    const float R20 = two_s * (qi * qk - qj * qr), R21 = two_s * (qj * qk + qi * qr), R22 = 1 - two_s * (qi * qi + qj * qj);
    for (int a = a0 + lane; a < a1; a += 64)
        if (tags[a] == 2) {
            const float rx = pos[3 * a] - cx, ry = pos[3 * a + 1] - cy, rz = pos[3 * a + 2] - cz;
            pos[3 * a] = ((rx * R00 + ry * R01 + rz * R02) + tx) + cx;
            pos[3 * a + 1] = ((rx * R10 + ry * R11 + rz * R12) + ty) + cy;
            pos[3 * a + 2] = ((rx * R20 + ry * R21 + rz * R22) + tz) + cz;
        }
}

__global__ __launch_bounds__(64) void adf_step_reduce_kernel(StepParams p) {
    const int b = blockIdx.x, lane = threadIdx.x;
    const int a0 = p.atom_offset[b], a1 = p.atom_offset[b + 1];
    float s[10];
    step_sums(p, a0, a1, lane, s);
    if (lane != 0) return;
    float com[3], dcom[3], drot[3];
    const bool conv = step_increment(p, b, s, com, dcom, drot);
    float* o = p.sys + 16 * b;
    for (int k = 0; k < 3; ++k) { o[k] = com[k]; o[3 + k] = dcom[k]; o[6 + k] = drot[k]; }
    if (!conv) atomicAnd(&p.state[2], 0);
    if (p.dcom_out) for (int k = 0; k < 3; ++k) p.dcom_out[3 * b + k] = dcom[k];
    if (p.drot_out) for (int k = 0; k < 3; ++k) p.drot_out[3 * b + k] = drot[k];
}

__global__ void adf_step_decide_kernel(int32_t* state, int early_stop_count) {
    if (threadIdx.x == 0 && blockIdx.x == 0) {
        if (!state[1]) {
            if (state[2]) {
                state[0] += 1;
                if (early_stop_count > 0 && state[0] == early_stop_count) state[1] = 1;
            }
            if (!state[1]) state[3] += 1;
        }
        state[2] = 1;
        state[4] += 1;
    }
}

__global__ __launch_bounds__(64) void adf_step_apply_kernel(StepParams p) {
    if (p.state[1]) return;
    const int b = blockIdx.x, lane = threadIdx.x;
    const int a0 = p.atom_offset[b], a1 = p.atom_offset[b + 1];
    const float* o = p.sys + 16 * b;
    step_rigid_update(p.pos, p.tags, a0, a1, lane, o[0], o[1], o[2], o[3], o[4], o[5], o[6], o[7], o[8]);
}

__device__ __forceinline__ bool system_decide(int32_t* st, int32_t* state, int cvg, bool conv, int early_stop_count,
                                              int lane) {
    bool freeze = false;
    if (conv) {
        cvg += 1;
        freeze = early_stop_count > 0 && cvg == early_stop_count;
    }
    if (lane == 0) {
        st[0] = cvg;
        if (freeze) {
            st[1] = 1;
            st[3] = state[4];
            atomicAdd(&state[0], 1);
        } else {
            const int applied = st[2] + 1;
            st[2] = applied;
            atomicMax(&state[3], applied);
        }
    }
    return !freeze;
}

__global__ __launch_bounds__(64) void adf_step_system_kernel(StepParams p, int32_t* sys_state) {
    const int b = blockIdx.x, lane = threadIdx.x;
    int32_t* st = sys_state + 4 * b;
    const int cvg = st[0], frozen = st[1];
    if (frozen) {
        if (lane < 3) {
            if (p.dcom_out) p.dcom_out[3 * b + lane] = 0.f;
            if (p.drot_out) p.drot_out[3 * b + lane] = 0.f;
        }
        return;
    }
    const int a0 = p.atom_offset[b], a1 = p.atom_offset[b + 1];
    float s[10];
    step_sums(p, a0, a1, lane, s);
    float com[3], dcom[3], drot[3];
    const bool conv = step_increment(p, b, s, com, dcom, drot);
    if (lane < 3) {
        if (p.dcom_out) p.dcom_out[3 * b + lane] = dcom[lane];
        if (p.drot_out) p.drot_out[3 * b + lane] = drot[lane];
    }
    if (system_decide(st, p.state, cvg, conv, p.early_stop_count, lane))
        step_rigid_update(p.pos, p.tags, a0, a1, lane, com[0], com[1], com[2], dcom[0], dcom[1], dcom[2], drot[0], drot[1],
                          drot[2]);
}

__global__ void adf_step_system_finish_kernel(int32_t* state, int B) {
    if (threadIdx.x == 0 && blockIdx.x == 0) {
        state[1] = state[0] >= B ? 1 : 0;
        state[4] += 1;
    }
}

int32_t adf_stepper_init(const adf_batch* b, float* pos, const int32_t* tags, const float* noise,
                         hipStream_t s) {
    hipLaunchKernelGGL(adf_init_placement_kernel, dim3(b->num_systems), dim3(64), 0, s, b->cell, b->atom_offset, tags,
                       pos, noise, b->num_systems);
    ADF_HIP_CHECK(hipGetLastError());
    return ADF_OK;
}

int32_t adf_stepper_step(float* sys, const adf_batch* b, float* pos, const int32_t* tags, const int32_t* fixed,
                         const float* f1, const float* f2, const adf_step_coef* coef, const adf_step_coef* coefs_dev,
                         int num_steps, const float* z_tr, const float* z_rot, int32_t early_stop_count,
                         int32_t* state, float* dcom, float* drot, hipStream_t s, int32_t* sys_state) {
    StepParams p;
    p.cell = b->cell; p.atom_offset = b->atom_offset; p.tags = tags; p.fixed = fixed; p.pos = pos;
    p.f1 = f1; p.f2 = f2; p.z_tr = z_tr; p.z_rot = z_rot; p.sys = sys; p.state = state;
    p.dcom_out = dcom; p.drot_out = drot; p.B = b->num_systems; p.early_stop_count = early_stop_count;
    if (coef) p.c = *coef; else p.c = adf_step_coef{};
    p.coefs_dev = coefs_dev; p.num_steps = num_steps;
    if (sys_state) {
        hipLaunchKernelGGL(adf_step_system_kernel, dim3(p.B), dim3(64), 0, s, p, sys_state);
        hipLaunchKernelGGL(adf_step_system_finish_kernel, dim3(1), dim3(64), 0, s, state, p.B);
        ADF_HIP_CHECK(hipGetLastError());
        return ADF_OK;
    }
    hipLaunchKernelGGL(adf_step_reduce_kernel, dim3(p.B), dim3(64), 0, s, p);
    hipLaunchKernelGGL(adf_step_decide_kernel, dim3(1), dim3(64), 0, s, state, early_stop_count);
    hipLaunchKernelGGL(adf_step_apply_kernel, dim3(p.B), dim3(64), 0, s, p);
    ADF_HIP_CHECK(hipGetLastError());
    return ADF_OK;
}

struct TrParams {
    const float* cell;
    const int32_t* atom_offset;
    const int32_t* tags;
    float* pos;
    const float* f1;
    const float* z;
    float* sys;
    int32_t* state;
    float* dcom_out;
    adf_tr_coef c;
    const adf_tr_coef* coefs_dev;
    int num_steps;
};

__device__ __forceinline__ void tr_sums(const TrParams& p, int a0, int a1, int lane, float* s) {
#pragma unroll
    for (int i = 0; i < 7; ++i) s[i] = 0.f;
    for (int a = a0 + lane; a < a1; a += 64)
        if (p.tags[a] == 2) {
            s[0] += p.pos[3 * a]; s[1] += p.pos[3 * a + 1]; s[2] += p.pos[3 * a + 2];
            s[3] += p.f1[3 * a]; s[4] += p.f1[3 * a + 1]; s[5] += p.f1[3 * a + 2];
            s[6] += 1.f;
        }
#pragma unroll
    for (int i = 0; i < 7; ++i) s[i] = adf_wave_sum(s[i]);
}

__device__ __forceinline__ bool tr_increment(const TrParams& p, int b, const float* s, float* com, float* dcom) {
    const float cnt = fmaxf(s[6], 1.0f);
    adf_tr_coef c = p.c;
    if (p.coefs_dev) c = p.coefs_dev[min(p.state[4], p.num_steps - 1)];
    for (int k = 0; k < 3; ++k) {
        com[k] = s[k] / cnt;
        float d = __fmul_rn(c.coef, s[3 + k] / cnt);
        if (p.z) d = __fadd_rn(d, __fmul_rn(c.noise, p.z[3 * b + k]));
        dcom[k] = d;
    }
    dcom[2] = 0.f;
    const float tgt[3] = {__fadd_rn(com[0], dcom[0]), __fadd_rn(com[1], dcom[1]), __fadd_rn(com[2], dcom[2])};
    return step_wrap(p.cell + 9 * b, tgt, com, dcom);
}

__device__ __forceinline__ void tr_update(float* pos, const int32_t* tags, int a0, int a1, int lane, float tx, float ty,
                                          float tz) {
    for (int a = a0 + lane; a < a1; a += 64)
        if (tags[a] == 2) {
            pos[3 * a] = __fadd_rn(pos[3 * a], tx);
            pos[3 * a + 1] = __fadd_rn(pos[3 * a + 1], ty);
            pos[3 * a + 2] = __fadd_rn(pos[3 * a + 2], tz);
        }
}

__global__ __launch_bounds__(64) void adf_tr_reduce_kernel(TrParams p) {
    const int b = blockIdx.x, lane = threadIdx.x;
    const int a0 = p.atom_offset[b], a1 = p.atom_offset[b + 1];
    float s[7];
    tr_sums(p, a0, a1, lane, s);
    if (lane != 0) return;
    float com[3], dcom[3];
    const bool conv = tr_increment(p, b, s, com, dcom);
    float* o = p.sys + 16 * b;
    for (int k = 0; k < 3; ++k) { o[k] = com[k]; o[3 + k] = dcom[k]; }
    if (!conv) atomicAnd(&p.state[2], 0);
    if (p.dcom_out) for (int k = 0; k < 3; ++k) p.dcom_out[3 * b + k] = dcom[k];
}

__global__ __launch_bounds__(64) void adf_tr_apply_kernel(TrParams p) {
    if (p.state[1]) return;
    const int b = blockIdx.x, lane = threadIdx.x;
    const int a0 = p.atom_offset[b], a1 = p.atom_offset[b + 1];
    const float* o = p.sys + 16 * b;
    tr_update(p.pos, p.tags, a0, a1, lane, o[3], o[4], o[5]);
}

__global__ __launch_bounds__(64) void adf_tr_system_kernel(TrParams p, int32_t* sys_state, int early_stop_count) {
    const int b = blockIdx.x, lane = threadIdx.x;
    int32_t* st = sys_state + 4 * b;
    const int cvg = st[0], frozen = st[1];
    if (frozen) {
        if (lane < 3 && p.dcom_out) p.dcom_out[3 * b + lane] = 0.f;
        return;
    }
    const int a0 = p.atom_offset[b], a1 = p.atom_offset[b + 1];
    float s[7];
    tr_sums(p, a0, a1, lane, s);
    float com[3], dcom[3];
    const bool conv = tr_increment(p, b, s, com, dcom);
    if (lane < 3 && p.dcom_out) p.dcom_out[3 * b + lane] = dcom[lane];
    if (system_decide(st, p.state, cvg, conv, early_stop_count, lane))
        tr_update(p.pos, p.tags, a0, a1, lane, dcom[0], dcom[1], dcom[2]);
}

int32_t adf_stepper_tr_step(float* sys, const adf_batch* b, float* pos, const int32_t* tags, const float* f1,
                            const adf_tr_coef* coef, const adf_tr_coef* coefs_dev, int num_steps, const float* z,
                            int32_t early_stop_count, int32_t* state, float* dcom, hipStream_t s, int32_t* sys_state) {
    TrParams p;
    p.cell = b->cell; p.atom_offset = b->atom_offset; p.tags = tags; p.pos = pos; p.f1 = f1; p.z = z; p.sys = sys;
    p.state = state; p.dcom_out = dcom;
    if (coef) p.c = *coef; else p.c = adf_tr_coef{};
    p.coefs_dev = coef ? nullptr : coefs_dev; p.num_steps = num_steps;
    const int B = b->num_systems;
    if (sys_state) {
        hipLaunchKernelGGL(adf_tr_system_kernel, dim3(B), dim3(64), 0, s, p, sys_state, early_stop_count);
        hipLaunchKernelGGL(adf_step_system_finish_kernel, dim3(1), dim3(64), 0, s, state, B);
        ADF_HIP_CHECK(hipGetLastError());
        return ADF_OK;
    }
    hipLaunchKernelGGL(adf_tr_reduce_kernel, dim3(B), dim3(64), 0, s, p);
    hipLaunchKernelGGL(adf_step_decide_kernel, dim3(1), dim3(64), 0, s, state, early_stop_count);
    hipLaunchKernelGGL(adf_tr_apply_kernel, dim3(B), dim3(64), 0, s, p);
    ADF_HIP_CHECK(hipGetLastError());
    return ADF_OK;
}

int32_t adf_model_set_per_system_stop(int32_t** slot, int32_t* slot_B, int32_t* sys_state, int32_t B) {
    if (sys_state && B <= 0) { adf_set_error("set_per_system_stop: B must be positive"); return ADF_EINVAL; }
    *slot = sys_state;
    *slot_B = sys_state ? B : 0;
    return ADF_OK;
}
static int32_t check_per_system(const adf_model& m, const adf_batch* b) {
    if (m.sys_state && m.sys_B != b->num_systems) {
        adf_set_error("per-system stop is set for %d systems, the batch has %d", (int)m.sys_B, (int)b->num_systems);
        return ADF_EINVAL;
    }
    return ADF_OK;
}

int32_t adf_model_init_placement(const adf_model& m, const adf_batch* b, float* pos, const int32_t* tags,
                                 const float* noise, hipStream_t s) {
    ADF_TRY(m.check(m.h, b));
    if (!pos || !tags || !noise) { adf_set_error("null argument"); return ADF_EINVAL; }
    return adf_stepper_init(b, pos, tags, noise, s);
}

int32_t adf_model_sde_step(const adf_model& m, const adf_batch* b, float* pos, const int32_t* tags, const int32_t* fixed,
                           const float* f1, const float* f2, const adf_step_coef* coef, const adf_step_coef* coefs_dev,
                           int32_t num_steps, const float* z_tr, const float* z_rot, int32_t early_stop_count,
                           int32_t* state, float* dcom, float* drot, hipStream_t s) {
    ADF_TRY(m.check(m.h, b));
    if (!pos || !tags || !f1 || !f2 || (!coef && !coefs_dev) || !state) { adf_set_error("null argument"); return ADF_EINVAL; }
    if (!coef && num_steps <= 0) { adf_set_error("num_steps must be positive"); return ADF_EINVAL; }
    ADF_TRY(check_per_system(m, b));
    float* sys = nullptr;
    ADF_TRY(m.grow(m.h, b, &sys));
    m.prof(m.h, true, s);
    const int32_t st = adf_stepper_step(sys, b, pos, tags, fixed, f1, f2, coef, coef ? nullptr : coefs_dev, num_steps, z_tr,
                                        z_rot, early_stop_count, state, dcom, drot, s, m.sys_state);
    m.prof(m.h, false, s);
    return st;
}

int32_t adf_model_tr_step(const adf_model& m, const adf_batch* b, float* pos, const int32_t* tags, const float* f1,
                          const adf_tr_coef* coef, const adf_tr_coef* coefs_dev, int32_t num_steps, const float* z,
                          int32_t early_stop_count, int32_t* state, float* dcom, hipStream_t s) {
    ADF_TRY(m.check(m.h, b));
    if (!pos || !tags || !f1 || (!coef && !coefs_dev) || !state) { adf_set_error("tr_step: null argument"); return ADF_EINVAL; }
    if (!coef && num_steps <= 0) { adf_set_error("tr_step: num_steps must be positive"); return ADF_EINVAL; }
    ADF_TRY(check_per_system(m, b));
    float* sys = nullptr;
    ADF_TRY(m.grow(m.h, b, &sys));
    m.prof(m.h, true, s);
    const int32_t st = adf_stepper_tr_step(sys, b, pos, tags, f1, coef, coefs_dev, num_steps, z, early_stop_count, state,
                                           dcom, s, m.sys_state);
    m.prof(m.h, false, s);
    return st;
}

template <class Step>
static int32_t sample_loop(const adf_model& m, const adf_batch* b, float* pos, const int32_t* tags, const void* coefs_dev,
                           int32_t num_steps, int32_t early_stop_count, int32_t poll_every, int32_t* state,
                           const int32_t* out_idx, int32_t n_out, float* f1, float* f2, adf_frames* sink,
                           int32_t frame_every, hipStream_t s, Step step) {
    ADF_TRY(m.check(m.h, b));
    if (num_steps <= 0 || !f1 || !state || !coefs_dev || !pos || !tags || (out_idx && n_out < 0)) {
        adf_set_error("sample: bad argument");
        return ADF_EINVAL;
    }
    if (sink && frame_every <= 0) { adf_set_error("sample: frame_every must be positive"); return ADF_EINVAL; }
    ADF_TRY(check_per_system(m, b));
    for (int t = 0; t < num_steps; ++t) {
        ADF_TRY(m.forward(m.h, b, out_idx, n_out, f1, f2, s));
        ADF_TRY(step((size_t)t * b->num_systems * 3));
        if (sink && ((t + 1) % frame_every == 0 || t + 1 == num_steps)) ADF_TRY(adf_frames_push_impl(sink, pos, s));
        if (early_stop_count > 0 && poll_every > 0 && (t % poll_every) == poll_every - 1 && t + 1 < num_steps) {
            int32_t frozen = 0;
            ADF_HIP_CHECK(hipMemcpyAsync(&frozen, state + 1, sizeof(int32_t), hipMemcpyDeviceToHost, s));
            ADF_HIP_CHECK(hipStreamSynchronize(s));
            if (frozen) break;
        }
    }
    return ADF_OK;
}

int32_t adf_model_sample(const adf_model& m, const adf_batch* b, float* pos, const int32_t* tags, const int32_t* fixed,
                         const adf_step_coef* coefs_dev, int32_t num_steps, const float* z_tr_all, const float* z_rot_all,
                         int32_t early_stop_count, int32_t poll_every, int32_t* state, const int32_t* out_idx,
                         int32_t n_out, float* f1, float* f2, adf_frames* sink, int32_t frame_every, hipStream_t s) {
    if (!f2) { adf_set_error("sample: f2 is null"); return ADF_EINVAL; }
    if ((z_tr_all == nullptr) != (z_rot_all == nullptr)) { adf_set_error("sample: need both noise tables or none"); return ADF_EINVAL; }
    return sample_loop(m, b, pos, tags, coefs_dev, num_steps, early_stop_count, poll_every, state, out_idx, n_out, f1, f2,
                       sink, frame_every, s, [&](size_t z) {
                           return adf_model_sde_step(m, b, pos, tags, fixed, f1, f2, nullptr, coefs_dev, num_steps,
                                                     z_tr_all ? z_tr_all + z : nullptr, z_rot_all ? z_rot_all + z : nullptr,
                                                     early_stop_count, state, nullptr, nullptr, s);
                       });
}

int32_t adf_model_tr_sample(const adf_model& m, const adf_batch* b, float* pos, const int32_t* tags,
                            const adf_tr_coef* coefs_dev, int32_t num_steps, const float* z_all, int32_t early_stop_count,
                            int32_t poll_every, int32_t* state, const int32_t* out_idx, int32_t n_out, float* f1,
                            adf_frames* sink, int32_t frame_every, hipStream_t s) {
    return sample_loop(m, b, pos, tags, coefs_dev, num_steps, early_stop_count, poll_every, state, out_idx, n_out, f1,
                       nullptr, sink, frame_every, s, [&](size_t z) {
                           return adf_model_tr_step(m, b, pos, tags, f1, nullptr, coefs_dev, num_steps,
                                                    z_all ? z_all + z : nullptr, early_stop_count, state, nullptr, s);
                       });
}

__global__ __launch_bounds__(64) void adf_lift_kernel(float* pos, const int32_t* tags, const int32_t* atom_offset,
                                                       float min_gap, float* lifted) {
    const int b = blockIdx.x, lane = threadIdx.x;
    const int a0 = atom_offset[b], a1 = atom_offset[b + 1];
    float zs = -3.0e38f, za = 3.0e38f;
    for (int a = a0 + lane; a < a1; a += 64) {
        const float z = pos[3 * a + 2];
        if (tags[a] == 1) zs = fmaxf(zs, z);
        if (tags[a] == 2) za = fminf(za, z);
    }
#pragma unroll
    for (int o = 32; o > 0; o >>= 1) { zs = fmaxf(zs, __shfl_xor(zs, o)); za = fminf(za, __shfl_xor(za, o)); }
    float shift = 0.f;
    if (zs > -1.0e38f && za < 1.0e38f) {
        const float diff = za - zs;
        if (diff < min_gap) shift = fabsf(diff) + min_gap;
    }
    if (shift != 0.f)
        for (int a = a0 + lane; a < a1; a += 64)
            if (tags[a] == 2) pos[3 * a + 2] = pos[3 * a + 2] + shift;
    if (lifted && lane == 0) lifted[b] = shift;
}

extern "C" int32_t adf_lift_adsorbates(float* pos, const int32_t* tags, const int32_t* atom_offset, int32_t B, float min_gap,
                                       float* lifted, void* stream) {
    if (!pos || !tags || !atom_offset || B <= 0) { adf_set_error("lift_adsorbates: bad argument"); return ADF_EINVAL; }
    hipLaunchKernelGGL(adf_lift_kernel, dim3(B), dim3(64), 0, (hipStream_t)stream, pos, tags, atom_offset, min_gap, lifted);
    ADF_HIP_CHECK(hipGetLastError());
    return ADF_OK;
}
```

adsorbdiff_amd/denoising_torch.py:

```python
from __future__ import annotations

import logging
from pathlib import Path
from typing import Callable, List, Optional

import numpy as np
import torch

from . import lib as _lib


def schedule_coefs(params: dict) -> List[_lib.StepCoef]:
    lo, hi = params["ads_std_low"], params["ads_std_high"]
    rlo, rhi = params["rot_std_low"], params["rot_std_high"]
    T = int(params["num_steps"])
    ode = params.get("ode", True)
    sched = torch.tensor(np.linspace(1, 0, T + 1)[:-1], dtype=torch.float32)
    out = []
    for t_idx in range(T):
        t = sched[t_idx]
        tr_sigma = lo ** (1 - t) * hi**t
        rot_sigma = rlo ** (1 - t) * rhi**t
        tr_g = tr_sigma * (2 * np.log(hi / lo)) ** 0.5
        rot_g = 2 * rot_sigma * torch.sqrt(torch.tensor(np.log(rhi / rlo)))
# ... 51 lines not shown
def per_system_stop_steps(conv, count: int = 10):
    conv = torch.as_tensor(conv).to(torch.bool)
    if conv.dim() != 2:
        raise ValueError(f"per_system_stop_steps: [T,B] expected, got {list(conv.shape)}")
    T, B = conv.shape
    cum = torch.cumsum(conv.to(torch.int64), 0)
    hit = (cum == int(count)) & conv if count > 0 else torch.zeros_like(conv)
    any_hit = hit.any(0)
    first = torch.argmax(hit.to(torch.int64), 0)
    stop_step = torch.where(any_hit, first, torch.full_like(first, -1))
    steps = torch.where(any_hit, first, torch.full_like(first, T))
    return steps, stop_step


class DiffTorchCalc:

    def __init__(self, model, transform=None) -> None:
        self.model = model
        self.transform = transform

    def get_denoising_prediction(self, atoms, apply_constraint: bool = True):
        predictions = self.model.predict_denoising(atoms, per_image=False, disable_tqdm=True)
        positions = predictions["positions"]
        if "positions_free" in predictions and apply_constraint:
            positions_free = predictions["positions_free"]
            positions_free[atoms.fixed.to(positions_free.device) == 1] = 0
            return positions, positions_free
        return positions

    def update_graph(self, atoms):
        raise NotImplementedError(
            "pre-computed graphs (otf_graph=False) are not part of the HIP sampling path; "
            "the graph is rebuilt on the device every step"
        )


class Denoiser:
    def __init__(
        self,
        batch,
        model: DiffTorchCalc,
        denoising_pos_params: dict,
        device: str = "cuda:0",
        save_full_traj: bool = True,
        traj_dir: Optional[Path] = None,
        traj_names=None,
        early_stop_batch: bool = False,
        logger=None,
        noise_fn: Optional[Callable[[int, int], tuple]] = None,
    ) -> None:
        self.batch = batch
        self.model = model
        self.device = device
        self.save_full = save_full_traj
        self.traj_dir = traj_dir
        self.traj_names = traj_names
        self.early_stop_batch = early_stop_batch
        self.otf_graph = model.model._unwrapped_model.otf_graph
        self.denoising_pos_params = denoising_pos_params
        self.noise_fn = noise_fn
        self.steps_applied = 0
        self.stop_step = None
        self.per_system = bool(denoising_pos_params.get("per_system", False))
        if self.per_system and denoising_pos_params.get("use_graph", False):
            raise ValueError("denoising_pos_params: per_system with use_graph - the per-system rule ends the loop by a read "
                             "of the frozen count, which a replayed graph does not make")
        self.noise_seed = denoising_pos_params.get("noise_seed")
        self._noise_keys = self._noise_site = None
        if self.noise_seed is not None:
            self._init_noise_keys()
        assert not self.traj_dir or (
            traj_dir and len(traj_names)
        ), "Trajectory names should be specified to save trajectories"
        if not self.otf_graph:
            raise NotImplementedError("the HIP sampling path requires otf_graph=True")

    def _init_noise_keys(self) -> None:
        from .noising import noise_key_source, noise_keys

        batch = self.batch
        B = int(batch.natoms.shape[0])
        keys = noise_keys(batch).detach().cpu().reshape(-1)
        if noise_key_source(batch) == "index":
            logging.warning("adsorbdiff_amd: noise_seed without batch.noise_key or batch.sid: the keys are the positions in "
                            "the batch, so this run is NOT batch-invariant")
        site = getattr(batch, "site_index", None)
        site = torch.zeros(B, dtype=torch.int32) if site is None else torch.as_tensor(site).detach().cpu().reshape(-1).to(torch.int32)
        if site.numel() != B:
            raise ValueError(f"batch.site_index: [{B}] expected, got [{site.numel()}]")
        if site.numel() and (int(site.min()) < 0 or int(site.max()) >= (1 << 30)):
            raise ValueError("batch.site_index outside [0, 2^30)")
        pairs = set(zip(keys.tolist(), site.tolist()))
        if len(pairs) != B:
            raise ValueError("noise_seed: two systems of the batch share (noise key, site_index) and would be sampled "
                             "identically; give them distinct batch.noise_key / sid or batch.site_index")
        self._noise_keys, self._noise_site = keys, site

    def _keyed_draws(self, dev, T: int, place: bool = False, z_a: bool = False, z_b: bool = False):
        from .engine import sampler_draws

        return sampler_draws(int(self.noise_seed), self._noise_keys, self._noise_site, T, dev, place=place, z_a=z_a, z_b=z_b)

    SAMPLERS = ("sde_rot", "sde", "langevin")

    def run(self):
        sampler = self.denoising_pos_params.get("sampler", "sde_rot")
        if sampler not in self.SAMPLERS:
            raise ValueError(f"denoising_pos_params['sampler'] = {sampler!r}: expected one of {self.SAMPLERS}")
        if sampler == "sde":
            self.reverse_sde_sampling()
        elif sampler == "langevin":
            self.langevin_dynamics()
        else:
            self.reverse_sde_sampling_rot()
        return self.batch

    def _engine(self):
        net = self.model.model._unwrapped_model
        if not hasattr(net, "engine"):
            raise RuntimeError(
                "Denoiser needs an adsorbdiff_amd score model (PaiNN with a HIP engine); got "
                f"{type(net).__name__}"
            )
        return net.engine(torch.device(self.device))

    def reverse_sde_sampling_rot(self):
        params = self.denoising_pos_params
        if "ads_std_low" not in params:
            return
        T = int(params["num_steps"])
        ode = params.get("ode", True)
        coefs = schedule_coefs(params)
        early = 10 if params.get("early_stop", True) else 0
        use_graph = bool(params.get("use_graph", False))

        def begin(eng, prep, pos):
            B, N, dev = prep.num_systems, prep.num_atoms, pos.device
            coefs_dev = torch.tensor(
                [[c.coef_tr, c.rot_pre, c.rot_dt, c.rot_g2, c.noise_tr, c.noise_rot] for c in coefs],
                dtype=torch.float32, device=dev)

            def fused(f1, state, out_idx, poll_every, sink):
                f2 = torch.zeros(N, 3, dtype=torch.float32, device=dev)
                zt = zr = None
                if not ode and self.noise_seed is not None:
                    _, zt, zr = self._keyed_draws(dev, T, z_a=True, z_b=True)
                elif not ode:
                    zt = torch.empty(T, B, 3, dtype=torch.float32, device=dev)
                    zr = torch.empty(T, B, 3, dtype=torch.float32, device=dev)
                    for t_idx in range(T):
                        zt[t_idx].normal_()
                        zr[t_idx].normal_()
                eng.sample(prep, pos, f1, f2, coefs_dev, T, state, zt, zr, early_stop_count=early, poll_every=poll_every,
                           out_idx=out_idx, sink=sink, frame_every=1)

            def per_step(f1, state, out_idx):
                f2 = torch.zeros(N, 3, dtype=torch.float32, device=dev)
                z_tr = z_rot = graph = keyed = None
                if not ode:
                    z_tr = torch.empty(B, 3, dtype=torch.float32, device=dev)
                    z_rot = torch.empty(B, 3, dtype=torch.float32, device=dev)
                    if self.noise_fn is None and self.noise_seed is not None:
                        keyed = self._keyed_draws(dev, T, z_a=True, z_b=True)[1:]

                def one_step():
                    eng.forward_prepared(prep, pos, f1, f2, out_idx)
                    eng.sde_step_scheduled(prep, pos, f1, f2, coefs_dev, T, state, z_tr, z_rot, early_stop_count=early)

                def step(t_idx):
                    nonlocal graph
                    if not ode:
                        if self.noise_fn is not None:
                            a, b_ = self.noise_fn(t_idx, B)
                            z_tr.copy_(a.to(dev, torch.float32))
                            z_rot.copy_(b_.to(dev, torch.float32))
                        elif keyed is not None:
                            z_tr.copy_(keyed[0][t_idx])
                            z_rot.copy_(keyed[1][t_idx])
                        else:
                            z_tr.normal_()
                            z_rot.normal_()
                    if graph is not None:
                        graph.replay()
                        return
                    one_step()
                    if use_graph and t_idx == 0 and T > 2:
                        torch.cuda.synchronize(dev)
                        graph = torch.cuda.CUDAGraph()
                        snapshot = (pos.clone(), state.clone())
                        with torch.cuda.graph(graph):
                            one_step()
                        assert torch.equal(state, snapshot[1])

                return step

            return fused, per_step

        self._sample(T, early, begin, fused=not use_graph and self.noise_fn is None and params.get("step_hook") is None,
                     incremental=not use_graph)

    def reverse_sde_sampling(self):
        params = self.denoising_pos_params
        if "ads_std_low" not in params:
            return
        coefs = ode_tr_coefs(params)
        self._tr_sampling(coefs, False, None, 10 if params.get("early_stop", True) else 0)

    def langevin_dynamics(self):
        params = self.denoising_pos_params
        if "ads_std_low" not in params:
            return
        coefs = langevin_coefs(params)
        self._tr_sampling(coefs, True, params.get("langevin_noise"), 0)

    def _tr_sampling(self, coefs, langevin: bool, noise_table, early: int) -> None:
        T = len(coefs)

        def begin(eng, prep, pos):
            B, N, dev = prep.num_systems, prep.num_atoms, pos.device
            z_all = None
            if langevin:
                if noise_table is None and self.noise_seed is not None:
                    z_all = self._keyed_draws(dev, T, z_a=True)[1]
                elif noise_table is None:
                    z_all = torch.empty(T, B, 3, dtype=torch.float32, device=dev)
                    for t_idx in range(T):
                        z_all[t_idx].normal_()
                else:
                    z_all = torch.as_tensor(noise_table, dtype=torch.float32)
                    if tuple(z_all.shape) != (T, B, 3):
                        raise ValueError(f"langevin_noise has shape {tuple(z_all.shape)}, expected {(T, B, 3)}")
                    z_all = z_all.to(dev).contiguous()
            coefs_dev = torch.tensor([[c.coef, c.noise] for c in coefs], dtype=torch.float32, device=dev)

            def fused(f1, state, out_idx, poll_every, sink):
                eng.tr_sample(prep, pos, f1, coefs_dev, T, state, z_all, early_stop_count=early, poll_every=poll_every,
                              out_idx=out_idx, sink=sink, frame_every=1)

            def per_step(f1, state, out_idx):
                f2 = torch.zeros(N, 3, dtype=torch.float32, device=dev) if eng.num_heads == 2 else None

                def step(t_idx):
                    eng.forward_prepared(prep, pos, f1, f2, out_idx)
                    eng.tr_step(prep, pos, f1, state, coefs_dev=coefs_dev, num_steps=T,
                                z=z_all[t_idx] if z_all is not None else None, early_stop_count=early)

                return step

            return fused, per_step

        self._sample(T, early, begin, fused=self.denoising_pos_params.get("step_hook") is None, incremental=True)

    def _sample(self, T: int, early: int, begin, fused: bool, incremental: bool) -> None:
        params = self.denoising_pos_params
        trainer = self.model.model
        dev = torch.device(self.device)
        trainer._unwrapped_model.eval()
        ema = getattr(trainer, "ema", None)
        if ema:
            ema.store()
            ema.copy_to()
        try:
            eng = self._engine()
            batch = self.batch.to(dev)
            if batch.pos.dtype != torch.float32 or not batch.pos.is_contiguous():
                batch.pos = batch.pos.to(torch.float32).contiguous()
            pos = batch.pos
            prep = eng.prepare(batch, params.get("image_repeats"))
            if prep.tags is None:
                raise ValueError("batch.tags is required (tag 2 marks the adsorbate)")
            eng.bind_condition(batch, prep.num_systems)
            B, N = prep.num_systems, prep.num_atoms
            fused_run, per_step = begin(eng, prep, pos)

            noise = params.get("placement_noise")
            if noise is None and self.noise_seed is not None:
                noise = self._keyed_draws(dev, 0, place=True)[0]
            elif noise is None:
                noise = torch.rand(B, 3)
            else:
                noise = torch.as_tensor(noise, dtype=torch.float32).reshape(B, 3).cpu()
            eng.init_placement(prep, pos, noise.to(dev))
            if params.get("static_atom_cache", True):
                eng.set_moving_atoms(prep, prep.tags == 2)
            eng.set_incremental(bool(params.get("incremental_layers", True)) and incremental)

            step_hook = params.get("step_hook")
            check_every = 1 if B <= 8 else 5
            ads_only = params.get("scores_on_adsorbate_only")
            if ads_only is None:
                ads_only = fused
            pos0 = pos.clone()

            def attempt():
                f1 = torch.zeros(N, 3, dtype=torch.float32, device=dev)
                state = torch.tensor([0, 0, 1, 0, 0, 0, 0, 0], dtype=torch.int32, device=dev)
                sys_state = None
                if self.per_system:
                    sys_state = torch.tensor([[0, 0, 0, -1]] * B, dtype=torch.int32, device=dev)
                    eng.set_per_system_stop(sys_state)
                out_idx = torch.nonzero(prep.tags == 2).reshape(-1).to(torch.int32).contiguous() if ads_only else None
                if fused:
                    self._run_fused(eng, batch, pos, state, T,
                                    lambda sink: fused_run(f1, state, out_idx, check_every if early else 0, sink), sys_state)
                    return state, None, sys_state
                frames = [] if self.traj_dir else None
                step = per_step(f1, state, out_idx)
# ... 146 lines not shown
```

adsorbdiff_amd/engine.py:

```python
from __future__ import annotations

import ctypes as C
import logging
import os
from dataclasses import dataclass
from typing import List, Optional, Sequence

import torch

from . import lib as _lib


def cell_repeats(cell: torch.Tensor, radius: float, pbc: Sequence[bool] = (True, True, True)) -> List[int]:
    cell = cell.detach().to("cpu", torch.float32).reshape(-1, 3, 3)
    a1, a2, a3 = cell[:, 0], cell[:, 1], cell[:, 2]
    c23 = torch.cross(a2, a3, dim=-1)
    vol = torch.sum(a1 * c23, dim=-1, keepdim=True)
    crosses = (c23, torch.cross(a3, a1, dim=-1), torch.cross(a1, a2, dim=-1))
    reps = []
    for k in range(3):
        if pbc[k]:
            inv_min_dist = torch.norm(crosses[k] / vol, p=2, dim=-1)
            reps.append(int(torch.ceil(radius * inv_min_dist).max().item()))
        else:
            reps.append(0)
    return reps


def batch_pbc(data) -> List[bool]:
    pbc = [True, True, True]
    if hasattr(data, "pbc") and getattr(data, "pbc") is not None:
        flags = torch.atleast_2d(data.pbc).to("cpu")
        for i in range(3):
            if not torch.any(flags[:, i]).item():
                pbc[i] = False
            elif torch.all(flags[:, i]).item():
                pbc[i] = True
            else:
                raise RuntimeError(
                    "Different structures in the batch have different PBC configurations. "
                    "This is not currently supported."
                )
    return pbc


@dataclass
class PreparedBatch:

    num_systems: int
    num_atoms: int
    cell: torch.Tensor
    atomic_numbers: torch.Tensor
    batch: torch.Tensor
    atom_offset: torch.Tensor
    reps: List[int]
    tags: Optional[torch.Tensor] = None
    fixed: Optional[torch.Tensor] = None

    def desc(self, pos: torch.Tensor) -> _lib.BatchDesc:
        d = _lib.BatchDesc()
        d.num_systems, d.num_atoms = self.num_systems, self.num_atoms
        d.pos = pos.data_ptr()
        d.cell = self.cell.data_ptr()
        d.atomic_numbers = self.atomic_numbers.data_ptr()
        d.batch = self.batch.data_ptr()
        d.atom_offset = self.atom_offset.data_ptr()
        d.reps[0], d.reps[1], d.reps[2] = self.reps
        return d


def image_repeats(batch, cutoff: float) -> List[int]:
    return cell_repeats(batch.cell, float(cutoff), batch_pbc(batch))


def _require_gpu(t: torch.Tensor, what: str) -> None:
    if not t.is_cuda:
        raise RuntimeError(
            f"{what} is on {t.device}: the adsorbdiff_amd HIP path only runs on a ROCm device "
            "(there is no CPU fallback)"
        )


def _ptr(t: Optional[torch.Tensor]):
    return t.data_ptr() if t is not None else None


def _numel(t: Optional[torch.Tensor]) -> int:
    return int(t.numel()) if t is not None else 0


def sampler_draws(seed: int, keys: torch.Tensor, site: Optional[torch.Tensor], num_steps: int, device, place: bool = True,
                  z_a: bool = False, z_b: bool = False):
    dev = torch.device(device)
    keys = torch.as_tensor(keys, dtype=torch.int64).reshape(-1).to(dev).contiguous()
    B, T = int(keys.shape[0]), int(num_steps)
    if site is not None:
        site = torch.as_tensor(site).reshape(-1).to(dev, torch.int32).contiguous()
        if site.shape[0] != B:
            raise ValueError(f"sampler_draws: {B} keys, {site.shape[0]} site indices")
    out = [torch.empty(shape, dtype=torch.float32, device=dev) if want else None
           for want, shape in ((place, (B, 3)), (z_a, (T, B, 3)), (z_b, (T, B, 3)))]
    seed = int(seed) & 0xFFFFFFFFFFFFFFFF
    seed = seed - (1 << 64) if seed >= (1 << 63) else seed
    with torch.cuda.device(dev):
        _lib.check(_lib.load().adf_sampler_draws(seed, keys.data_ptr(), _ptr(site), B, T, *[_ptr(t) for t in out],
                                                 C.c_void_p(torch.cuda.current_stream(dev).cuda_stream)))
    return tuple(out)


class Engine:

    SYMBOLS: dict = {}

    def __init__(self, model, device) -> None:
        self.lib = _lib.load()
        self.device = torch.device(device)
        if self.device.type != "cuda":
            raise RuntimeError(f"{type(self).__name__} needs a ROCm device, got {self.device} (no CPU fallback)")
        self.model = model
        self.exact_f32 = os.environ.get("ADF_GEMM") == "f32"
        self._weights_keepalive: List[torch.Tensor] = []
        self._moving_keepalive = None
        self._sys_state_keepalive = None

    def _c(self, role: str):
        return getattr(self.lib, self.SYMBOLS[role])

    def _stream(self) -> C.c_void_p:
        return C.c_void_p(torch.cuda.current_stream(self.device).cuda_stream)

    def prepare(self, data, image_repeats: Optional[Sequence[int]] = None) -> PreparedBatch:
        _require_gpu(data.pos, "data.pos")
        dev = self.device
        natoms = data.natoms.to(dev, torch.int64).reshape(-1)
        B = int(natoms.shape[0])
        N = int(data.pos.shape[0])
        off = torch.zeros(B + 1, dtype=torch.int32, device=dev)
        off[1:] = torch.cumsum(natoms, 0).to(torch.int32)
        cell = data.cell.to(dev, torch.float32).reshape(B, 3, 3).contiguous()
        reps = cell_repeats(cell, float(self.model.cutoff), batch_pbc(data))
        if image_repeats is not None:
            if len(image_repeats) != 3:
                raise ValueError(f"image_repeats: three counts expected, got {list(image_repeats)}")
            reps = [max(int(r), int(f)) if r > 0 else 0 for r, f in zip(reps, image_repeats)]
        prep = PreparedBatch(
            num_systems=B, num_atoms=N, cell=cell,
            atomic_numbers=data.atomic_numbers.to(dev).long().to(torch.int32).contiguous(),
            batch=data.batch.to(dev, torch.int32).contiguous(),
            atom_offset=off, reps=reps,
        )
        if hasattr(data, "tags") and data.tags is not None:
            prep.tags = data.tags.to(dev, torch.int32).contiguous()
        if hasattr(data, "fixed") and data.fixed is not None:
            prep.fixed = data.fixed.to(dev, torch.int32).contiguous()
        return prep

    def bind_condition(self, data, num_systems: int) -> None:
        """What a conditional model reads from the batch besides the atoms; nothing for the others."""

    def set_moving_atoms(self, prep: Optional[PreparedBatch], moving_mask: Optional[torch.Tensor]) -> None:
        if moving_mask is None or prep is None:
            self._moving_keepalive = None
            _lib.check(self._c("set_moving")(self.handle, None, None, None))
            return
        mask = moving_mask.to(self.device, torch.int32).contiguous()
        idx = torch.nonzero(mask).reshape(-1).to(torch.int32).contiguous()
        per_sys = torch.bincount(prep.batch[idx.long()].long(), minlength=prep.num_systems)
        off = torch.zeros(prep.num_systems + 1, dtype=torch.int32, device=self.device)
        off[1:] = torch.cumsum(per_sys, 0).to(torch.int32)
        self._moving_keepalive = (mask, idx, off)
        _lib.check(self._c("set_moving")(self.handle, mask.data_ptr(), idx.data_ptr(), off.data_ptr()))

    def check_flags(self) -> None:
        with torch.cuda.device(self.device):
            _lib.check(self._c("check_flags")(self.handle, self._stream()))

    def use_exact_f32(self) -> bool:
        if self.exact_f32:
            return False
        logging.warning("adsorbdiff_amd: non-finite output in f16x3 arithmetic; re-running in exact f32 "
                        "(this engine stays in exact f32)")
        _lib.check(self._c("set_arithmetic")(self.handle, 1))
        self.exact_f32 = True
        return True

    def set_incremental(self, on: bool = True) -> None:
        _lib.check(self._c("set_incremental")(self.handle, 1 if on else 0))

    def set_per_system_stop(self, sys_state: Optional[torch.Tensor]) -> None:
        if sys_state is None:
            self._sys_state_keepalive = None
            _lib.check(self._c("set_per_system_stop")(self.handle, None, 0))
            return
        if (sys_state.dtype != torch.int32 or sys_state.dim() != 2 or sys_state.shape[1] != 4 or not sys_state.is_contiguous()
                or sys_state.device != self.device):
            raise ValueError("set_per_system_stop: contiguous int32 [B,4] on the engine's device expected")
        self._sys_state_keepalive = sys_state
        _lib.check(self._c("set_per_system_stop")(self.handle, sys_state.data_ptr(), int(sys_state.shape[0])))

    def init_placement(self, prep: PreparedBatch, pos: torch.Tensor, noise: torch.Tensor) -> None:
        desc = prep.desc(pos)
        with torch.cuda.device(self.device):
            _lib.check(self._c("init_placement")(
                self.handle, C.byref(desc), pos.data_ptr(), prep.tags.data_ptr(), noise.data_ptr(), self._stream()))

    def sde_step(self, prep: PreparedBatch, pos, f1, f2, coef: _lib.StepCoef, state, z_tr=None, z_rot=None,
                 early_stop_count: int = 10, dcom=None, drot=None) -> None:
        self._sde_step(prep, pos, f1, f2, coef, None, 0, state, z_tr, z_rot, early_stop_count, dcom, drot)

    def sde_step_scheduled(self, prep: PreparedBatch, pos, f1, f2, coefs_dev: torch.Tensor, num_steps: int, state,
                           z_tr=None, z_rot=None, early_stop_count: int = 10) -> None:
        self._sde_step(prep, pos, f1, f2, None, coefs_dev, num_steps, state, z_tr, z_rot, early_stop_count, None, None)

    def _sde_entry(self, coef, coefs_dev, num_steps):
        return self._c("sde_step"), (C.byref(coef) if coef is not None else None, _ptr(coefs_dev), num_steps)

    def _sde_step(self, prep, pos, f1, f2, coef, coefs_dev, num_steps, state, z_tr, z_rot, early_stop_count, dcom, drot):
        desc = prep.desc(pos)
        entry, schedule = self._sde_entry(coef, coefs_dev, num_steps)
        with torch.cuda.device(self.device):
            _lib.check(entry(self.handle, C.byref(desc), pos.data_ptr(), prep.tags.data_ptr(), _ptr(prep.fixed),
                             f1.data_ptr(), f2.data_ptr(), *schedule, _ptr(z_tr), _ptr(z_rot), early_stop_count,
                             state.data_ptr(), _ptr(dcom), _ptr(drot), self._stream()))

    def sample(self, prep: PreparedBatch, pos, f1, f2, coefs_dev: torch.Tensor, num_steps: int, state,
               z_tr_all=None, z_rot_all=None, early_stop_count: int = 10, poll_every: int = 0,
               out_idx: Optional[torch.Tensor] = None, sink=None, frame_every: int = 1) -> None:
        self._loop("sample", prep, pos, [_ptr(prep.fixed), coefs_dev.data_ptr(), num_steps, _ptr(z_tr_all),
                                         _ptr(z_rot_all), early_stop_count, poll_every, state.data_ptr(), _ptr(out_idx),
                                         _numel(out_idx), f1.data_ptr(), f2.data_ptr()], sink, frame_every)

    def tr_step(self, prep: PreparedBatch, pos, f1, state, coef: Optional[_lib.TrCoef] = None,
                coefs_dev: Optional[torch.Tensor] = None, num_steps: int = 0, z=None, early_stop_count: int = 10,
                dcom=None) -> None:
        desc = prep.desc(pos)
        with torch.cuda.device(self.device):
            _lib.check(self._c("tr_step")(
                self.handle, C.byref(desc), pos.data_ptr(), prep.tags.data_ptr(), f1.data_ptr(),
                C.byref(coef) if coef is not None else None, _ptr(coefs_dev), int(num_steps), _ptr(z), early_stop_count,
                state.data_ptr(), _ptr(dcom), self._stream()))

    def tr_sample(self, prep: PreparedBatch, pos, f1, coefs_dev: torch.Tensor, num_steps: int, state, z_all=None,
                  early_stop_count: int = 10, poll_every: int = 0, out_idx=None, sink=None, frame_every: int = 1) -> None:
        self._loop("tr_sample", prep, pos, [coefs_dev.data_ptr(), int(num_steps), _ptr(z_all), early_stop_count,
                                            poll_every, state.data_ptr(), _ptr(out_idx), _numel(out_idx), f1.data_ptr()],
                   sink, frame_every)

    def _loop(self, role: str, prep: PreparedBatch, pos, args: list, sink, frame_every: int) -> None:
        desc = prep.desc(pos)
        head = [self.handle, C.byref(desc), pos.data_ptr(), prep.tags.data_ptr()]
        with torch.cuda.device(self.device):
            if sink is None:
                _lib.check(self._c(role)(*head, *args, self._stream()))
            else:
                _lib.check(self._c(role + "_traj")(*head, *args, sink.handle, int(frame_every), self._stream()))

    def profile_enable(self, on: bool = True) -> None:
        _lib.check(self._c("profile_enable")(self.handle, 1 if on else 0))

    def close(self) -> None:
        if getattr(self, "handle", None) is not None and self.handle:
            with torch.cuda.device(self.device):
                torch.cuda.synchronize(self.device)
                self._c("destroy")(self.handle)
            self.handle = None

    def __del__(self):
        try:
            self.close()
        except Exception:
            pass


class PaiNNEngine(Engine):
    SYMBOLS = dict(set_moving="adf_graph_set_moving", check_flags="adf_check_flags",
                   set_arithmetic="adf_painn_set_arithmetic", set_incremental="adf_painn_set_incremental",
                   init_placement="adf_sde_init_placement", sample="adf_sample", sample_traj="adf_sample_traj",
                   tr_step="adf_tr_step", tr_sample="adf_tr_sample", tr_sample_traj="adf_tr_sample_traj",
                   set_per_system_stop="adf_painn_set_per_system_stop",
                   profile_enable="adf_profile_enable", destroy="adf_painn_destroy")

    def __init__(self, model, device) -> None:
        super().__init__(model, device)
        hp = _lib.Hparams(
            hidden_channels=model.hidden_channels, num_layers=model.num_layers, num_rbf=model.num_rbf,
            num_elements=model.num_elements, max_neighbors=model.max_neighbors,
            envelope_exponent=int(model.radial_basis.envelope.p),
            num_heads=getattr(model, "num_force_heads", 2 if model.so3_denoising else 1),
            cutoff=float(model.cutoff),
        )
        self.num_heads = hp.num_heads
        self.handle = C.c_void_p()
        with torch.cuda.device(self.device):
            _lib.check(self.lib.adf_painn_create(C.byref(hp), C.byref(self.handle)))
        self._last_graph_N = 0
        floor = getattr(model, "distance_floor", None)
        if floor is not None:
            _lib.check(self.lib.adf_painn_set_distance_floor(self.handle, float(floor)))
        self.bind_weights()

    def _weight_list(self) -> List[torch.Tensor]:
        m = self.model
        sd = dict(m.named_parameters())
        sd.update(dict(m.named_buffers()))
        names = ["atom_emb.embeddings.weight", "radial_basis.rbf.offset"]
        for i in range(m.num_layers):
            p, u = f"message_layers.{i}.", f"update_layers.{i}."
            names += [
                p + "x_layernorm.weight", p + "x_layernorm.bias", p + "x_proj.0.weight", p + "x_proj.0.bias",
                p + "x_proj.2.weight", p + "x_proj.2.bias", p + "rbf_proj.weight", p + "rbf_proj.bias",
                u + "vec_proj.weight", u + "xvec_proj.0.weight", u + "xvec_proj.0.bias",
                u + "xvec_proj.2.weight", u + "xvec_proj.2.bias",
            ]
        heads = ["out_forces", "out_forces2"][:self.num_heads]
        for hname in heads:
            for b in range(2):
                q = f"{hname}.output_network.{b}."
                names += [q + "vec1_proj.weight", q + "vec2_proj.weight", q + "update_net.0.weight",
                          q + "update_net.0.bias", q + "update_net.2.weight", q + "update_net.2.bias"]
        out = []
        for n in names:
            t = sd[n].detach()
            _require_gpu(t, f"parameter {n}")
            if t.dtype != torch.float32 or not t.is_contiguous():
                t = t.to(torch.float32).contiguous()
            out.append(t)
        return out

    def bind_weights(self) -> None:
        ws = self._weight_list()
        self._weights_keepalive = ws
        ptrs = (C.c_void_p * len(ws))(*[w.data_ptr() for w in ws])
        scales = self.model.scale_factors()
        sf = (C.c_float * len(scales))(*scales)
        with torch.cuda.device(self.device):
            _lib.check(self.lib.adf_painn_set_weights(self.handle, len(ws), ptrs, sf, self._stream()))
        if getattr(self.model, "energy_head", False):
            oe = self.model.out_energy
            es = [t.detach().to(torch.float32).contiguous() for t in (oe[0].weight, oe[0].bias, oe[2].weight, oe[2].bias)]
            for t in es:
                _require_gpu(t, "out_energy parameter")
            self._weights_keepalive = ws + es
            eptrs = (C.c_void_p * 4)(*[t.data_ptr() for t in es])
            with torch.cuda.device(self.device):
                _lib.check(self.lib.adf_painn_set_energy_head(self.handle, 4, eptrs, self._stream()))

    def forward_prepared(self, prep: PreparedBatch, pos: torch.Tensor, f1: torch.Tensor, f2: Optional[torch.Tensor],
                         out_idx: Optional[torch.Tensor] = None) -> None:
        desc = prep.desc(pos)
        with torch.cuda.device(self.device):
            if out_idx is None:
                _lib.check(self.lib.adf_painn_forward(
                    self.handle, C.byref(desc), f1.data_ptr(), f2.data_ptr() if f2 is not None else None, self._stream()))
            else:
                assert out_idx.dtype == torch.int32 and out_idx.is_contiguous() and out_idx.device == pos.device
                _lib.check(self.lib.adf_painn_forward_subset(
                    self.handle, C.byref(desc), out_idx.data_ptr(), int(out_idx.numel()), f1.data_ptr(),
                    f2.data_ptr() if f2 is not None else None, self._stream()))

    def forward(self, data):
        prep = self.prepare(data)
        pos = data.pos.to(torch.float32).contiguous()
        f1 = torch.empty(prep.num_atoms, 3, dtype=torch.float32, device=self.device)
        f2 = torch.empty_like(f1) if self.model.so3_denoising else None
        self.forward_prepared(prep, pos, f1, f2)
        try:
            self.check_flags()
        except _lib.NumericRangeError:
            if not self.use_exact_f32():
                raise
            self.forward_prepared(prep, pos, f1, f2)
            self.check_flags()
        return f1, f2

    def forward_energy_prepared(self, prep: PreparedBatch, pos: torch.Tensor, energy: torch.Tensor,
                                forces: Optional[torch.Tensor]) -> None:
        desc = prep.desc(pos)
        with torch.cuda.device(self.device):
            _lib.check(self.lib.adf_painn_forward_energy(
                self.handle, C.byref(desc), energy.data_ptr(), forces.data_ptr() if forces is not None else None,
                self._stream()))

    def forward_energy(self, data):
        prep = self.prepare(data)
        pos = data.pos.to(torch.float32).contiguous()
        energy = torch.empty(prep.num_systems, dtype=torch.float32, device=self.device)
        forces = torch.empty(prep.num_atoms, 3, dtype=torch.float32, device=self.device) if self.num_heads else None
        self.forward_energy_prepared(prep, pos, energy, forces)
        try:
            self.check_flags()
        except _lib.NumericRangeError:
            if not self.use_exact_f32():
                raise
            self.forward_energy_prepared(prep, pos, energy, forces)
            self.check_flags()
        return energy, forces

    def forward_energy_gradient_prepared(self, prep: PreparedBatch, pos: torch.Tensor, energy: torch.Tensor,
                                         forces: torch.Tensor) -> None:
        desc = prep.desc(pos)
        with torch.cuda.device(self.device):
            _lib.check(self.lib.adf_painn_forward_energy_gradient(
                self.handle, C.byref(desc), energy.data_ptr(), forces.data_ptr(), self._stream()))

    def forward_energy_gradient(self, data):
        prep = self.prepare(data)
        pos = data.pos.to(torch.float32).contiguous()
        energy = torch.empty(prep.num_systems, dtype=torch.float32, device=self.device)
        forces = torch.empty(prep.num_atoms, 3, dtype=torch.float32, device=self.device)
        self.forward_energy_gradient_prepared(prep, pos, energy, forces)
        try:
            self.check_flags()
        except _lib.NumericRangeError:
            if not self.use_exact_f32():
                raise
            self.forward_energy_gradient_prepared(prep, pos, energy, forces)
            self.check_flags()
        return energy, forces

    def energy_gradient_workspace_bytes(self, num_atoms: int) -> int:
        n = C.c_int64(0)
        _lib.check(self.lib.adf_painn_energy_gradient_workspace(self.handle, int(num_atoms), C.byref(n)))
        return int(n.value)

    def get_tune(self) -> dict:
        t = _lib.Tune()
        _lib.check(self.lib.adf_painn_get_tune(self.handle, C.byref(t)))
        return {name: int(getattr(t, name)) for name, _ in _lib.Tune._fields_}

    def build_graph(self, data, prep=None):
        if prep is None:
            prep = self.prepare(data)
        pos = data.pos.to(torch.float32).contiguous()
        desc = prep.desc(pos)
        n = C.c_int64(0)
        with torch.cuda.device(self.device):
            _lib.check(self.lib.adf_graph_build(self.handle, C.byref(desc), self._stream(), C.byref(n)))
        self._last_graph_N = prep.num_atoms
        return int(n.value)

    def export_graph(self):
        N, K = self._last_graph_N, self.model.max_neighbors
        if N <= 0:
            raise RuntimeError("export_graph: call build_graph first")
        dev = self.device
        cnt = torch.empty(N, dtype=torch.int32, device=dev)
        src = torch.empty(N, K, dtype=torch.int32, device=dev)
        sh = torch.empty(N, K, 3, dtype=torch.int32, device=dev)
        cap = 2 * N * K
        es = torch.empty(cap, dtype=torch.int32, device=dev)
        ed = torch.empty(cap, dtype=torch.int32, device=dev)
        dist = torch.empty(cap, dtype=torch.float32, device=dev)
        vec = torch.empty(cap, 3, dtype=torch.float32, device=dev)
        n = C.c_int64(0)
        with torch.cuda.device(dev):
            _lib.check(self.lib.adf_graph_export(
                self.handle, cnt.data_ptr(), src.data_ptr(), sh.data_ptr(), cap, es.data_ptr(), ed.data_ptr(),
                dist.data_ptr(), vec.data_ptr(), C.byref(n), self._stream()))
        E = int(n.value)
        return cnt, src, sh, es[:E], ed[:E], dist[:E], vec[:E]

    def message_layer(self, layer: int, x: torch.Tensor, vec: torch.Tensor):
        x_out, vec_out = torch.empty_like(x), torch.empty_like(vec)
        with torch.cuda.device(self.device):
            _lib.check(self.lib.adf_painn_message_layer(
                self.handle, layer, x.shape[0], x.data_ptr(), vec.data_ptr(), x_out.data_ptr(), vec_out.data_ptr(),
                self._stream()))
        return x_out, vec_out

    def update_layer(self, layer: int, x: torch.Tensor, vec: torch.Tensor):
        with torch.cuda.device(self.device):
            _lib.check(self.lib.adf_painn_update_layer(
                self.handle, layer, x.shape[0], x.data_ptr(), vec.data_ptr(), self._stream()))
        return x, vec

    def _sde_entry(self, coef, coefs_dev, num_steps):
        if coef is not None:
            return self.lib.adf_sde_step, (C.byref(coef),)
        return self.lib.adf_sde_step_scheduled, (coefs_dev.data_ptr(), num_steps)

    def counters(self) -> _lib.Counters:
        c = _lib.Counters()
        with torch.cuda.device(self.device):
            _lib.check(self.lib.adf_get_counters(self.handle, C.byref(c), self._stream()))
        return c

    PROFILE_CATEGORIES = ("graph", "message", "node_dense", "heads", "stepper")

    def profile_read(self):
        ms = (C.c_float * 5)()
        cnt = (C.c_int64 * 5)()
        ksteps = C.c_int64(0)
        with torch.cuda.device(self.device):
            _lib.check(self.lib.adf_profile_read(self.handle, ms, cnt, C.byref(ksteps), self._stream()))
        out = {k: (float(ms[i]), int(cnt[i])) for i, k in enumerate(self.PROFILE_CATEGORIES)}
        out["message_ksteps"] = int(ksteps.value)
        return out

    def measure_peaks(self):
# ... 5 lines not shown
```

adsorbdiff_amd/lib.py:

```python
from __future__ import annotations

import ctypes as C
import re
from pathlib import Path

ADF_OK, ADF_EINVAL, ADF_EOOM, ADF_ENONEIGHBOR, ADF_EHIP, ADF_EOVERFLOW, ADF_ENUMERIC = 0, 1, 2, 3, 4, 5, 6


class NumericRangeError(ArithmeticError):
    """Non-finite model output (ADF_ENUMERIC).  Not a RuntimeError on purpose: ``ml_diffuse`` must not answer it by
    splitting the batch; the engine answers it by re-running in exact f32."""


class Hparams(C.Structure):
    _fields_ = [
        ("hidden_channels", C.c_int32), ("num_layers", C.c_int32), ("num_rbf", C.c_int32),
        ("num_elements", C.c_int32), ("max_neighbors", C.c_int32), ("envelope_exponent", C.c_int32),
        ("num_heads", C.c_int32), ("cutoff", C.c_float),
    ]


class EqV2Hparams(C.Structure):
    _fields_ = [
        ("lmax", C.c_int32), ("mmax", C.c_int32), ("num_layers", C.c_int32), ("sphere_channels", C.c_int32),
        ("attn_hidden_channels", C.c_int32), ("num_heads", C.c_int32), ("attn_alpha_channels", C.c_int32),
        ("attn_value_channels", C.c_int32), ("ffn_hidden_channels", C.c_int32), ("grid_resolution", C.c_int32),
        ("edge_channels", C.c_int32), ("num_distance_basis", C.c_int32), ("max_num_elements", C.c_int32),
        ("max_neighbors", C.c_int32), ("max_radius", C.c_float), ("avg_degree", C.c_float),
    ]


class EqV2Counters(C.Structure):
    _fields_ = [("num_edges", C.c_int64), ("num_atoms", C.c_int64), ("dense_flops", C.c_int64), ("conv_flops", C.c_int64),
                ("inc_rows", C.c_int64), ("inc_rows_full", C.c_int64), ("forwards_total", C.c_int64),
                ("conv_flops_total", C.c_int64)]


class Tune(C.Structure):
    _fields_ = [(name, C.c_int32) for name in (
        "gemm_stream", "head_gate_fused", "lift_emit", "graph_sys_csr", "train_gemm16", "wgrad_f32",
        "eqv2_gemm_tile256", "eqv2_rotin_generic", "eqv2_rotout_generic")]


class BatchDesc(C.Structure):
    _fields_ = [
        ("num_systems", C.c_int32), ("num_atoms", C.c_int32), ("pos", C.c_void_p), ("cell", C.c_void_p),
        ("atomic_numbers", C.c_void_p), ("batch", C.c_void_p), ("atom_offset", C.c_void_p), ("reps", C.c_int32 * 3),
    ]


class ActiveField(C.Structure):
    _fields_ = [("src", C.c_void_p), ("dst", C.c_void_p), ("row_bytes", C.c_int32), ("per_system", C.c_int32)]


class StepCoef(C.Structure):
    _fields_ = [
        ("coef_tr", C.c_float), ("rot_pre", C.c_float), ("rot_dt", C.c_float), ("rot_g2", C.c_float),
        ("noise_tr", C.c_float), ("noise_rot", C.c_float),
    ]


class TrCoef(C.Structure):
    _fields_ = [("coef", C.c_float), ("noise", C.c_float)]


class Counters(C.Structure):
    _fields_ = [
        ("num_edges", C.c_int64), ("num_atoms", C.c_int64), ("message_bytes_per_layer", C.c_int64),
        ("dense_flops", C.c_int64),
        ("inc_rows", C.c_int64), ("inc_rows_full", C.c_int64), ("inc_msg_launches", C.c_int64),
        ("inc_msg_edges", C.c_int64),
    ]


HEADER = Path(__file__).resolve().parent.parent / "include" / "adsorbdiff_hip.h"

_SCALARS = {"int32_t": C.c_int32, "int64_t": C.c_int64, "float": C.c_float, "double": C.c_double}
_RETURNS = {"int32_t": C.c_int32, "int64_t": C.c_int64, "const char*": C.c_char_p}
_BYREF = {"adf_batch": BatchDesc, "adf_painn_hparams": Hparams, "adf_eqv2_hparams": EqV2Hparams, "adf_tune": Tune,
          "adf_counters": Counters, "adf_eqv2_counters": EqV2Counters, "adf_active_field": ActiveField}


def parse_header(text: str) -> dict:
    text = re.sub(r"/\*.*?\*/|//[^\n]*", " ", text, flags=re.S)
    text = re.sub(r"^[ \t]*#.*$", " ", text, flags=re.M)
    structs = set(re.findall(r"typedef\s+struct\s*\w*\s*\{[^}]*\}\s*(\w+)\s*;", text))
    text = re.sub(r"(typedef\s+struct|enum)\s*\w*\s*\{[^}]*\}\s*\w*\s*;", " ", text)
    handles = set(re.findall(r"typedef\s+struct\s+\w+\s*\*\s*(adf_\w+_t)\s*;", text))
    text = re.sub(r"typedef\s+struct\s+\w+\s*\*\s*adf_\w+_t\s*;|extern\s+\"C\"\s*\{|\}", " ", text)
    pointees = set(_SCALARS) | structs | handles | {"void", "char", "uint8_t"}

    def argtype(fn: str, param: str):
        tokens = [t for t in re.findall(r"\w+|\*|\S", param) if t != "const"]
        base, stars, name = tokens[:1], tokens[1:-1], tokens[-1:]
        if len(tokens) < 2 or any(t != "*" for t in stars) or not re.fullmatch(r"[A-Za-z_]\w*", name[0]) or name[0] in pointees:
            raise ValueError(f"{fn}: parameter {param.strip()!r} is not `type name`")
        base = base[0]
        if stars:
            if base not in pointees:
                raise ValueError(f"{fn}: parameter {param.strip()!r} points to the unknown type {base!r}")
            return C.POINTER(_BYREF[base]) if base in _BYREF and len(stars) == 1 else C.c_void_p
        if base in handles:
            return C.c_void_p
        if base not in _SCALARS:
            raise ValueError(f"{fn}: parameter {param.strip()!r} has the unknown type {base!r}")
        return _SCALARS[base]

    out = {}
    for stmt in filter(None, (s.strip() for s in text.split(";"))):
        m = re.fullmatch(r"(.*?)\b(adf_[a-z_0-9]+)\s*\((.*)\)", stmt, flags=re.S)
        if m is None:
            raise ValueError(f"not a prototype, an enum, a struct or a handle typedef: {' '.join(stmt.split())!r}")
        ret, fn, params = re.sub(r"\s*\*\s*", "*", " ".join(m.group(1).split())), m.group(2), m.group(3).strip()
        if ret not in _RETURNS:
            raise ValueError(f"{fn}: unknown return type {ret!r}")
        if fn in out:
            raise ValueError(f"{fn}: declared twice")
        out[fn] = (_RETURNS[ret], [] if params == "void" else [argtype(fn, p) for p in params.split(",")])
    return out


SIGNATURES = parse_header(HEADER.read_text())
EXPORTS = tuple(SIGNATURES)

_LIB = None


def lib_path() -> Path:
    import os

    override = os.environ.get("ADF_LIB_PATH")
    if override:
        return Path(override)
    return Path(__file__).resolve().parent / "libadsorbdiff_hip.so"


def load():
    global _LIB
    if _LIB is not None:
        return _LIB
    path = lib_path()
    if not path.exists():
        raise RuntimeError(
            f"{path} not found: build it with `python -m adsorbdiff_amd.build` "
            "(the HIP path has no CPU fallback)"
        )
    lib = C.CDLL(str(path))
    for name, (restype, argtypes) in SIGNATURES.items():
        fn = getattr(lib, name)
        fn.restype, fn.argtypes = restype, argtypes
    _LIB = lib
    return lib


def check(status: int) -> None:
    if status == ADF_OK:
        return
    msg = load().adf_last_error().decode("utf-8", "replace")
    if status == ADF_ENONEIGHBOR:
        raise ValueError(msg)
    if status == ADF_EOVERFLOW:
        raise ValueError(f"adsorbdiff_hip: capacity exceeded: {msg}")
    if status == ADF_EOOM:
        raise RuntimeError(f"HIP out of memory: {msg}")
    if status == ADF_ENUMERIC:
        raise NumericRangeError(msg)
    if status == ADF_EINVAL:
        raise ValueError(f"adsorbdiff_hip: invalid argument: {msg}")
    raise RuntimeError(f"adsorbdiff_hip error {status}: {msg}")
```

include/adsorbdiff_hip.h:

```cpp
#ifndef ADSORBDIFF_HIP_H
#define ADSORBDIFF_HIP_H

#include <stdint.h>

#ifdef __cplusplus
extern "C" {
#endif

#define ADF_OK 0
#define ADF_EINVAL 1
#define ADF_EOOM 2
#define ADF_ENONEIGHBOR 3
#define ADF_EHIP 4
#define ADF_EOVERFLOW 5
#define ADF_ENUMERIC 6

typedef struct adf_painn* adf_painn_t;

typedef struct {
    int32_t hidden_channels;
    int32_t num_layers;
    int32_t num_rbf;
    int32_t num_elements;
    int32_t max_neighbors;
    int32_t envelope_exponent;
    int32_t num_heads;
    float cutoff;
} adf_painn_hparams;

#define ADF_WEIGHTS_PER_LAYER 13
#define ADF_WEIGHTS_PER_HEAD 12

int32_t adf_painn_create(const adf_painn_hparams* hp, adf_painn_t* out);
int32_t adf_painn_destroy(adf_painn_t h);

int32_t adf_painn_set_weights(adf_painn_t h, int32_t n_weights, const void* const* weights,
                              const float* scale_factors, void* stream);

typedef struct {
    int32_t num_systems;
    int32_t num_atoms;
    const float* pos;
    const float* cell;
    const int32_t* atomic_numbers;
    const int32_t* batch;
    const int32_t* atom_offset;
    int32_t reps[3];
} adf_batch;

int32_t adf_graph_build(adf_painn_t h, const adf_batch* b, void* stream, int64_t* num_edges);

int32_t adf_graph_set_moving(adf_painn_t h, const int32_t* moving, const int32_t* mov_idx, const int32_t* mov_off);

int32_t adf_painn_set_arithmetic(adf_painn_t h, int32_t exact_f32);

int32_t adf_painn_set_incremental(adf_painn_t h, int32_t on);

typedef struct adf_tune {
    int32_t gemm_stream;
    int32_t head_gate_fused;
    int32_t lift_emit;
    int32_t graph_sys_csr;
    int32_t train_gemm16;
    int32_t wgrad_f32;
    int32_t eqv2_gemm_tile256;
    int32_t eqv2_rotin_generic;
    int32_t eqv2_rotout_generic;
} adf_tune;
int32_t adf_painn_get_tune(adf_painn_t h, adf_tune* out);

int32_t adf_check_flags(adf_painn_t h, void* stream);

int32_t adf_graph_export(adf_painn_t h, int32_t* nbr_count, int32_t* nbr_src, int32_t* nbr_shift,
                         int64_t edge_capacity, int32_t* edge_src, int32_t* edge_dst, float* edge_dist,
                         float* edge_vec, int64_t* num_edges, void* stream);

int32_t adf_painn_forward(adf_painn_t h, const adf_batch* b, float* f1, float* f2, void* stream);

int32_t adf_painn_forward_subset(adf_painn_t h, const adf_batch* b, const int32_t* out_idx, int32_t n_out, float* f1,
                                 float* f2, void* stream);

int32_t adf_painn_message_layer(adf_painn_t h, int32_t layer, int32_t num_atoms, const float* x,
                                const float* vec, float* x_out, float* vec_out, void* stream);
int32_t adf_painn_update_layer(adf_painn_t h, int32_t layer, int32_t num_atoms, float* x, float* vec,
                               void* stream);
int32_t adf_painn_debug_row_maxima(adf_painn_t h, int32_t which, float* out, int64_t capacity, int32_t* rows,
                                   void* stream);

int32_t adf_linear_forward(const float* A, const float* W, const float* bias, float* C, int32_t M, int32_t N,
                           int32_t K, int32_t act_ssilu, int32_t mode, void* stream);

typedef struct {
    float coef_tr;
    float rot_pre;
    float rot_dt;
    float rot_g2;
    float noise_tr;
    float noise_rot;
} adf_step_coef;

int32_t adf_sde_init_placement(adf_painn_t h, const adf_batch* b, float* pos, const int32_t* tags,
                               const float* noise, void* stream);

int32_t adf_sde_step(adf_painn_t h, const adf_batch* b, float* pos, const int32_t* tags,
                     const int32_t* fixed, const float* f1, const float* f2, const adf_step_coef* coef,
                     const float* z_tr, const float* z_rot, int32_t early_stop_count, int32_t* state,
                     float* dcom, float* drot, void* stream);

int32_t adf_sde_step_scheduled(adf_painn_t h, const adf_batch* b, float* pos, const int32_t* tags,
                               const int32_t* fixed, const float* f1, const float* f2,
                               const adf_step_coef* coefs_dev, int32_t num_steps, const float* z_tr,
                               const float* z_rot, int32_t early_stop_count, int32_t* state, float* dcom,
                               float* drot, void* stream);

int32_t adf_sample(adf_painn_t h, const adf_batch* b, float* pos, const int32_t* tags, const int32_t* fixed,
                   const adf_step_coef* coefs_dev, int32_t num_steps, const float* z_tr_all, const float* z_rot_all,
                   int32_t early_stop_count, int32_t poll_every, int32_t* state, const int32_t* out_idx,
                   int32_t n_out, float* f1, float* f2, void* stream);

typedef struct {
    float coef;
    float noise;
} adf_tr_coef;

int32_t adf_tr_step(adf_painn_t h, const adf_batch* b, float* pos, const int32_t* tags, const float* f1,
                    const adf_tr_coef* coef, const adf_tr_coef* coefs_dev, int32_t num_steps, const float* z,
                    int32_t early_stop_count, int32_t* state, float* dcom, void* stream);
int32_t adf_tr_sample(adf_painn_t h, const adf_batch* b, float* pos, const int32_t* tags, const adf_tr_coef* coefs_dev,
                      int32_t num_steps, const float* z_all, int32_t early_stop_count, int32_t poll_every,
                      int32_t* state, const int32_t* out_idx, int32_t n_out, float* f1, void* stream);

typedef struct {
    int64_t num_edges;
    int64_t num_atoms;
    int64_t message_bytes_per_layer;
    int64_t dense_flops;
    int64_t inc_rows, inc_rows_full, inc_msg_launches, inc_msg_edges;
} adf_counters;
int32_t adf_get_counters(adf_painn_t h, adf_counters* out, void* stream);

int32_t adf_painn_set_per_system_stop(adf_painn_t h, int32_t* sys_state, int32_t B);

#define ADF_PROF_NCAT 5
int32_t adf_profile_enable(adf_painn_t h, int32_t on);
int32_t adf_profile_read(adf_painn_t h, float* ms, int64_t* count, int64_t* message_ksteps, void* stream);

int32_t adf_measure_peaks(float* out_host3, void* stream);

typedef struct adf_frames* adf_frames_t;
int32_t adf_frames_create(int32_t device, int64_t frame_floats, int32_t slots, adf_frames_t* out);
int32_t adf_frames_destroy(adf_frames_t f);
int32_t adf_frames_push(adf_frames_t f, const float* src, void* stream);
int32_t adf_frames_wait(adf_frames_t f, int64_t index, int32_t timeout_ms, const float** host_ptr);
int32_t adf_frames_release(adf_frames_t f, int64_t index);
int64_t adf_frames_pushed(adf_frames_t f);
int32_t adf_frames_abort(adf_frames_t f);
int32_t adf_sample_traj(adf_painn_t h, const adf_batch* b, float* pos, const int32_t* tags, const int32_t* fixed,
                        const adf_step_coef* coefs_dev, int32_t num_steps, const float* z_tr_all, const float* z_rot_all,
                        int32_t early_stop_count, int32_t poll_every, int32_t* state, const int32_t* out_idx,
                        int32_t n_out, float* f1, float* f2, adf_frames_t sink, int32_t frame_every, void* stream);
int32_t adf_tr_sample_traj(adf_painn_t h, const adf_batch* b, float* pos, const int32_t* tags,
                           const adf_tr_coef* coefs_dev, int32_t num_steps, const float* z_all, int32_t early_stop_count,
                           int32_t poll_every, int32_t* state, const int32_t* out_idx, int32_t n_out, float* f1,
                           adf_frames_t sink, int32_t frame_every, void* stream);

int32_t adf_lift_adsorbates(float* pos, const int32_t* tags, const int32_t* atom_offset, int32_t B, float min_gap,
                            float* lifted, void* stream);

int32_t adf_flag_anomalies(const adf_batch* b, const float* pos_final, const float* pos_slab_ref, const int32_t* tags,
                           const float* radii, int32_t num_radii, float skin, float surface_mult, float desorption_mult,
                           int32_t* flags, void* stream);

int32_t adf_select_best_sites(const float* energy, const int32_t* flags, const int32_t* group_offset, int32_t num_groups,
                              int32_t* best, float* best_energy, int32_t* n_valid, void* stream);

int32_t adf_site_pair_distances(const float* pos, const float* cell, const int32_t* tags, const int32_t* atomic_numbers,
                                const int32_t* atom_offset, const int32_t* group_offset, const int64_t* pair_offset,
                                int32_t num_atoms, int32_t num_sites, int32_t num_groups, int64_t out_len,
                                int32_t include_slab, int32_t permutation_invariant, float* out, void* stream);
int32_t adf_unique_sites(const float* dist, const int32_t* group_offset, const int64_t* pair_offset, int32_t num_sites,
                         int32_t num_groups, int64_t dist_len, const float* energy, const int32_t* flags, float tol,
                         float energy_tol, int32_t* rep, int32_t* n_unique, void* stream);
int32_t adf_select_top_sites(const float* energy, const int32_t* flags, const int32_t* rep, const int32_t* group_offset,
                             int32_t num_groups, int32_t k, int32_t* top, float* top_energy, void* stream);

int64_t adf_slab_symmetry_scratch(int32_t num_atoms, int32_t num_slabs);
int32_t adf_slab_symmetry_search(const float* pos, const float* cell, const int32_t* atomic_numbers,
                                 const int32_t* atom_offset, int32_t num_atoms, int32_t num_slabs, double symprec,
                                 int32_t proper_only, void* scratch, int32_t* n_ops, int32_t* n_ops_host, void* stream);
int32_t adf_slab_symmetry_emit(const int32_t* atom_offset, int32_t num_atoms, int32_t num_slabs, double symprec,
                               const void* scratch, const int32_t* op_offset, const int64_t* perm_offset, int32_t num_ops,
                               int64_t perm_len, double* rot, double* trans, int32_t* W, int32_t* perm, void* stream);
int32_t adf_site_pair_distances_sym(const float* pos, const float* cell, const int32_t* tags, const int32_t* atomic_numbers,
                                    const int32_t* atom_offset, const int32_t* group_offset, const int64_t* pair_offset,
                                    int32_t num_atoms, int32_t num_sites, int32_t num_groups, int64_t out_len,
                                    int32_t include_slab, int32_t permutation_invariant, const int32_t* op_offset,
                                    const double* rot, const double* trans, const int32_t* perm, const int64_t* perm_offset,
                                    int32_t num_ops, int64_t perm_len, float* out, int32_t* best_op, void* stream);

int32_t adf_place_draws(int64_t seed, const int64_t* keys, const int32_t* index, int32_t n, double* out, void* stream);
int32_t adf_place_adsorbates(const adf_batch* slabs, const int32_t* slab_of, const float* site, const double* draws,
                             const int32_t* ads_offset, const float* ads_pos, const int32_t* ads_Z, const float* radii,
                             int32_t num_radii, const float* masses, int32_t num_masses, float interstitial_gap,
                             int32_t mode, const int32_t* binding_idx, const int32_t* pbc, int32_t P,
                             const int32_t* out_row, int64_t out_rows, float* out_pos, double* scaled_normal,
                             int32_t* n_combos, double* rot_meta, void* stream);
int32_t adf_place_site_candidates(const float* tri, const int32_t* tri_offset, const int32_t* per_tri,
                                  const int32_t* cand_offset, const int32_t* cand_slab, const float* cell,
                                  const double* draws, int32_t B, int32_t num_candidates, float* cand, int32_t* keep,
                                  void* stream);
int32_t adf_interstitial_distances(const adf_batch* b, const int32_t* tags, const float* radii, int32_t num_radii,
                                   const float* masses, int32_t num_masses, const int32_t* pbc, float* out, void* stream);

int32_t adf_surface_site_candidates(const float* pos, const int32_t* tags, const int32_t* atom_offset, const float* cell,
                                    const float* tri, const int32_t* tri_offset, int32_t num_atoms, int32_t num_triangles,
                                    int32_t num_slabs, int32_t capacity, int32_t* seg_offset, float* cand, int32_t* valid,
                                    void* stream);
int32_t adf_reduce_sites(const float* cand, const int32_t* valid, const int32_t* seg_offset, const int32_t* seg_slab,
                         const float* cell, int32_t num_candidates, int32_t num_segments, int32_t num_slabs,
                         const int32_t* op_offset, const double* rot, const double* trans, int32_t num_ops, double tol,
// ... 294 lines not shown
```

Baseline: 250.3.

## Split sampling batch across a twin handle running on a second stream

Adds a twin model handle that borrows the parent's weight images and has its own stream and events. The sampling batch is cut into two halves of systems, and each half runs its denoise loop on a separate stream so the two sides can overlap on the GPU. The aim is better device occupancy and hiding of per-step serial gaps and host syncs. The cost is extra workspace for the twin, more bookkeeping (moving lists, incremental state, flags, profiling merged across both handles), and cache invalidation whenever the code switches between split and non-split paths.

```diff
diff --git a/adsorbdiff_amd/build.py b/adsorbdiff_amd/build.py
--- a/adsorbdiff_amd/build.py
+++ b/adsorbdiff_amd/build.py
@@ -22,7 +22,7 @@
     if not LIB.exists():
         return True
     t = LIB.stat().st_mtime
-    deps = [CSRC / s for s in SOURCES] + sorted(CSRC.glob("*.h")) + [PKG.parent / "include" / "adsorbdiff_hip.h"]
+    deps = [CSRC / s for s in SOURCES] + sorted(CSRC.glob("*.h")) + sorted((PKG.parent / "include").glob("*.h"))
     return any(d.stat().st_mtime > t for d in deps)
 
 
@@ -50,8 +50,8 @@
 
     cc = _hipcc()
     OBJ_DIR.mkdir(exist_ok=True)
-    hdr_t = max([p.stat().st_mtime for p in CSRC.glob("*.h")] + [(PKG.parent / "include" / "adsorbdiff_hip.h").stat().st_mtime,
-                                                                  Path(__file__).stat().st_mtime])
+    hdr_t = max([p.stat().st_mtime for p in CSRC.glob("*.h")] + [p.stat().st_mtime for p in (PKG.parent / "include").glob("*.h")] +
+                [Path(__file__).stat().st_mtime])
     jobs, objs = [], []
     for s in SOURCES:
         src, obj = CSRC / s, OBJ_DIR / (s + ".o")
diff --git a/adsorbdiff_amd/csrc/api.hip b/adsorbdiff_amd/csrc/api.hip
--- a/adsorbdiff_amd/csrc/api.hip
+++ b/adsorbdiff_amd/csrc/api.hip
@@ -32,6 +32,7 @@
     t.eqv2_gemm_tile256 = (gt && atoi(gt) == 128) ? 0 : 1;
     t.eqv2_rotin_generic = getenv("ADF_EQV2_ROTIN_GENERIC") != nullptr;
     t.eqv2_rotout_generic = getenv("ADF_EQV2_ROTOUT_GENERIC") != nullptr;
+    t.sample_split = off_is_0("ADF_SAMPLE_SPLIT");
     return t;
 }
 const adf_tune& adf_tune_process() {
@@ -48,6 +49,7 @@
     if (!h) { adf_set_error("null handle"); return ADF_EINVAL; }
     h->prof.enable(on != 0);
     ADF_HIP_CHECK(hipMemset(h->kcount, 0, 8 * sizeof(unsigned long long)));
+    if (h->twin) return adf_profile_enable(h->twin, on);
     return ADF_OK;
 }
 
@@ -60,7 +62,15 @@
         ADF_HIP_CHECK(hipMemset(h->kcount, 0, sizeof(k)));
         *message_ksteps = (int64_t)k[0];
     }
-    return h->prof.read(ms, count, ADF_PROF_NCAT);
+    ADF_TRY(h->prof.read(ms, count, ADF_PROF_NCAT));
+    if (h->twin) {
+        float ms2[ADF_PROF_NCAT];
+        int64_t count2[ADF_PROF_NCAT], k2 = 0;
+        ADF_TRY(adf_profile_read(h->twin, ms2, count2, message_ksteps ? &k2 : nullptr, h->twin->split_stream));
+        for (int c = 0; c < ADF_PROF_NCAT; ++c) { ms[c] += ms2[c]; count[c] += count2[c]; }
+        if (message_ksteps) *message_ksteps += k2;
+    }
+    return ADF_OK;
 }
 
 extern "C" int32_t adf_painn_create(const adf_painn_hparams* hp, adf_painn_t* out) {
@@ -156,6 +166,14 @@
 
 extern "C" int32_t adf_painn_destroy(adf_painn_t h) {
     if (!h) return ADF_OK;
+    if (h->twin) { adf_set_error("destroy: the handle has a live twin that reads its weight images; destroy the twin first"); return ADF_EINVAL; }
+    if (h->parent) {
+        h->parent->twin = nullptr;
+        h->parent->split_last = false;
+        if (h->split_stream) { (void)hipStreamSynchronize((hipStream_t)h->split_stream); (void)hipStreamDestroy((hipStream_t)h->split_stream); }
+        for (void* e : h->split_ev)
+            if (e) (void)hipEventDestroy((hipEvent_t)e);
+    }
     if (h->inc_cnt_host) (void)hipHostFree(h->inc_cnt_host);
     for (int i = 0; i < 2; ++i)
         if (h->inc_ev[i]) (void)hipEventDestroy((hipEvent_t)h->inc_ev[i]);
@@ -164,9 +182,88 @@
     return ADF_OK;
 }
 
+static void borrow_weights(adf_painn* t, const adf_painn* p, bool bound) {
+    t->emb = p->emb; t->rbf_offset = p->rbf_offset;
+    memcpy(t->layer, p->layer, sizeof(t->layer));
+    memcpy(t->head, p->head, sizeof(t->head));
+    memcpy(t->scale, p->scale, sizeof(t->scale));
+    t->rbf_pack = p->rbf_pack; t->rbf_bias_pack = p->rbf_bias_pack; t->rbf_pack16 = p->rbf_pack16;
+    t->rbf_bias_pack16 = p->rbf_bias_pack16; t->rbf_scales = p->rbf_scales; t->rbf_uniform = p->rbf_uniform;
+    t->w16_arena = p->w16_arena; t->w16_bytes = p->w16_bytes; t->w16_scales = p->w16_scales;
+    t->w16_bias_perm = p->w16_bias_perm; t->w16_scratch = p->w16_scratch; t->wfrag_arena = p->wfrag_arena;
+    t->weights_set = bound && p->weights_set;
+    t->rec0_valid = false;
+    t->inc_valid = false;
+}
+static void follow_settings(adf_painn* t, const adf_painn* p) {
+    if (t->gemm_f32 != p->gemm_f32 || t->msg_f32 != p->msg_f32 || t->dist_floor != p->dist_floor || t->lift_on != p->lift_on) {
+        t->cache_valid = false; t->rec0_valid = false; t->inc_valid = false;
+    }
+    t->gemm_f32 = p->gemm_f32; t->msg_f32 = p->msg_f32; t->msg_f32_only = p->msg_f32_only; t->dist_floor = p->dist_floor;
+    t->lift_on = p->lift_on; t->tune = p->tune; t->inc_sync = p->inc_sync;
+}
+
+extern "C" int32_t adf_painn_create_twin(adf_painn_t parent, adf_painn_t* out) {
+    if (!parent || !out) { adf_set_error("create_twin: null argument"); return ADF_EINVAL; }
+    if (parent->parent) { adf_set_error("create_twin: the handle is a twin itself"); return ADF_EINVAL; }
+    if (parent->twin) { adf_set_error("create_twin: the handle already has a twin"); return ADF_EINVAL; }
+    int dev = -1;
+    if (hipGetDevice(&dev) != hipSuccess || dev != parent->device) {
+        adf_set_error("create_twin: the parent lives on device %d, the current device is %d", parent->device, dev);
+        return ADF_EINVAL;
+    }
+    adf_painn* t = new (std::nothrow) adf_painn();
+    if (!t) { adf_set_error("host allocation failed"); return ADF_EOOM; }
+    t->hp = parent->hp; t->device = parent->device; t->num_cus = parent->num_cus;
+    t->rmx = parent->rmx; t->inc_on = parent->inc_on;
+    follow_settings(t, parent);
+    int32_t st = t->m_life.alloc(&t->flags, ADF_NFLAGS);
+    if (st == ADF_OK && hipMemset(t->flags, 0, sizeof(int32_t) * ADF_NFLAGS) != hipSuccess) st = ADF_EHIP;
+    if (st == ADF_OK) st = t->m_life.alloc(&t->kcount, 8);
+    if (st == ADF_OK && hipMemset(t->kcount, 0, 8 * sizeof(unsigned long long)) != hipSuccess) st = ADF_EHIP;
+    if (st == ADF_OK) st = t->m_life.alloc(&t->split_state, 16);
+    if (st == ADF_OK && hipStreamCreateWithFlags(reinterpret_cast<hipStream_t*>(&t->split_stream), hipStreamNonBlocking) != hipSuccess) st = ADF_EHIP;
+    for (int i = 0; i < 2 && st == ADF_OK; ++i)
+        if (hipEventCreateWithFlags(reinterpret_cast<hipEvent_t*>(&t->split_ev[i]), hipEventDisableTiming) != hipSuccess) st = ADF_EHIP;
+    if (st != ADF_OK) {
+        if (st == ADF_EHIP) adf_set_error("create_twin: %s", hipGetErrorString(hipGetLastError()));
+        t->parent = parent;
+        parent->twin = t;
+        adf_painn_destroy(t);
+        return st;
+    }
+    borrow_weights(t, parent, true);
+    t->prof.enable(parent->prof.on);
+    t->parent = parent;
+    parent->twin = t;
+    *out = t;
+    return ADF_OK;
+}
+
+extern "C" int32_t adf_painn_set_split(adf_painn_t h, int32_t on) {
+    if (!h) { adf_set_error("null handle"); return ADF_EINVAL; }
+    h->tune.sample_split = on != 0;
+    return ADF_OK;
+}
+
+extern "C" int32_t adf_split_stats(adf_painn_t h, int64_t* split_runs, int64_t* fallback_runs) {
+    if (!h) { adf_set_error("null handle"); return ADF_EINVAL; }
+    if (split_runs) *split_runs = (int64_t)h->split_runs;
+    if (fallback_runs) *fallback_runs = (int64_t)h->split_fallbacks;
+    return ADF_OK;
+}
+
+static void leave_split(adf_painn* h) {
+    if (!h || !h->split_last) return;
+    h->split_last = false;
+    h->cache_valid = false; h->rec0_valid = false; h->inc_valid = false;
+}
+
 extern "C" int32_t adf_painn_set_weights(adf_painn_t h, int32_t n_weights, const void* const* w,
                                          const float* scale_factors, void* stream) {
     if (!h || !w || !scale_factors) { adf_set_error("null argument"); return ADF_EINVAL; }
+    if (h->parent) { adf_set_error("set_weights: a twin reads its parent's weights; bind them there"); return ADF_EINVAL; }
+    if (h->twin) borrow_weights(h->twin, h, false);
     const int L = h->hp.num_layers;
     const int expect = 2 + ADF_WEIGHTS_PER_LAYER * L + ADF_WEIGHTS_PER_HEAD * h->hp.num_heads;
     if (n_weights != expect) {
@@ -249,6 +346,7 @@
     h->rec0_valid = false;
     h->inc_valid = false;
     adf_grad_invalidate(h);
+    if (h->twin) borrow_weights(h->twin, h, true);
     return ADF_OK;
 }
 
@@ -325,7 +423,13 @@
     int32_t f[ADF_NFLAGS];
     ADF_HIP_CHECK(hipMemcpyAsync(f, h->flags, sizeof(f), hipMemcpyDeviceToHost, s));
     ADF_HIP_CHECK(hipMemsetAsync(h->flags, 0, sizeof(f), s));
+    int32_t f2[ADF_NFLAGS] = {};
+    if (h->twin) {
+        ADF_HIP_CHECK(hipMemcpyAsync(f2, h->twin->flags, sizeof(f2), hipMemcpyDeviceToHost, s));
+        ADF_HIP_CHECK(hipMemsetAsync(h->twin->flags, 0, sizeof(f2), s));
+    }
     ADF_HIP_CHECK(hipStreamSynchronize(s));
+    for (int i = 0; i < ADF_NFLAGS; ++i) f[i] |= f2[i];
     if (f[4]) { adf_set_error("atomic number outside [1, %d] (rows of the embedding table)", h->hp.num_elements); return ADF_EINVAL; }
     if (f[0]) { adf_set_error("a centre atom has more than %d in-cutoff candidates", ADF_MAX_CAND); return ADF_EOVERFLOW; }
     if (f[2]) { adf_set_error("edge buffer overflow"); return ADF_EOVERFLOW; }
@@ -346,6 +450,7 @@
     if (!h) { adf_set_error("null handle"); return ADF_EINVAL; }
     if (moving && (!mov_idx || !mov_off)) { adf_set_error("moving mask needs mov_idx and mov_off"); return ADF_EINVAL; }
     h->moving = moving; h->mov_idx = mov_idx; h->mov_off = mov_off;
+    ++h->moving_serial;
     ADF_HIP_CHECK(hipMemset(h->flags, 0, sizeof(int32_t) * ADF_NFLAGS));
     h->cache_valid = false;
     h->rec0_valid = false;
@@ -355,6 +460,7 @@
 
 extern "C" int32_t adf_graph_build(adf_painn_t h, const adf_batch* b, void* stream, int64_t* num_edges) {
     ADF_TRY(check_batch(h, b));
+    leave_split(h);
     ADF_TRY(ensure_capacity(h, b->num_atoms, b->num_systems));
     hipStream_t s = (hipStream_t)stream;
     ADF_TRY(adf_graph_build_impl(h, b, s));
@@ -819,12 +925,14 @@
 }
 
 extern "C" int32_t adf_painn_forward(adf_painn_t h, const adf_batch* b, float* f1, float* f2, void* stream) {
+    leave_split(h);
     return forward_impl(h, b, nullptr, 0, f1, f2, stream);
 }
 
 extern "C" int32_t adf_painn_forward_subset(adf_painn_t h, const adf_batch* b, const int32_t* out_idx, int32_t n_out,
                                             float* f1, float* f2, void* stream) {
     if (!out_idx || n_out < 0) { adf_set_error("forward_subset: null index list"); return ADF_EINVAL; }
+    leave_split(h);
     return forward_impl(h, b, out_idx, n_out, f1, f2, stream);
 }
 
@@ -894,6 +1002,7 @@
     if (!energy || (h->hp.num_heads >= 1 && !forces)) { adf_set_error("forward_energy: null output"); return ADF_EINVAL; }
     if (h->hp.num_heads > 1) { adf_set_error("forward_energy: the S2EF model has one force head"); return ADF_EINVAL; }
     hipStream_t s = (hipStream_t)stream;
+    leave_split(h);
     ADF_TRY(forward_impl(h, b, nullptr, 0, forces, nullptr, stream));
     if (!h->x_last) { adf_set_error("internal: no node features after the forward"); return ADF_EINVAL; }
     const int N = b->num_atoms, H = h->hp.hidden_channels, H2 = H / 2;
@@ -951,10 +1060,15 @@
         }
     }
     h->inc_valid = false;
+    ++h->inc_set_serial;
     (void)inc_harvest(h, h->inc_slot, true);
     (void)inc_harvest(h, h->inc_slot ^ 1, true);
     h->inc_seen_valid = false;
     h->inc_rows = h->inc_rows_full = h->inc_edges = h->inc_launches = 0;
+    if (h->twin) {
+        ADF_TRY(adf_painn_set_incremental(h->twin, on));
+        h->twin->seen_inc_serial = h->inc_set_serial;
+    }
     return ADF_OK;
 }
 
@@ -1013,6 +1127,7 @@
                               const adf_step_coef* coefs_dev, int32_t num_steps, const float* z_tr_all,
                               const float* z_rot_all, int32_t early_stop_count, int32_t poll_every, int32_t* state,
                               const int32_t* out_idx, int32_t n_out, float* f1, float* f2, void* stream) {
+    leave_split(h);
     return adf_model_sample(model(h), b, pos, tags, fixed, coefs_dev, num_steps, z_tr_all, z_rot_all, early_stop_count,
                             poll_every, state, out_idx, n_out, f1, f2, nullptr, 0, (hipStream_t)stream);
 }
@@ -1022,6 +1137,7 @@
                                    const float* z_rot_all, int32_t early_stop_count, int32_t poll_every, int32_t* state,
                                    const int32_t* out_idx, int32_t n_out, float* f1, float* f2, adf_frames_t sink,
                                    int32_t frame_every, void* stream) {
+    leave_split(h);
     if (!sink) { adf_set_error("sample_traj: null sink"); return ADF_EINVAL; }
     return adf_model_sample(model(h), b, pos, tags, fixed, coefs_dev, num_steps, z_tr_all, z_rot_all, early_stop_count,
                             poll_every, state, out_idx, n_out, f1, f2, sink, frame_every, (hipStream_t)stream);
@@ -1038,6 +1154,7 @@
                                  const adf_tr_coef* coefs_dev, int32_t num_steps, const float* z_all,
                                  int32_t early_stop_count, int32_t poll_every, int32_t* state, const int32_t* out_idx,
                                  int32_t n_out, float* f1, void* stream) {
+    leave_split(h);
     return adf_model_tr_sample(model(h), b, pos, tags, coefs_dev, num_steps, z_all, early_stop_count, poll_every, state,
                                out_idx, n_out, f1, nullptr, 0, (hipStream_t)stream);
 }
@@ -1046,13 +1163,81 @@
                                       const adf_tr_coef* coefs_dev, int32_t num_steps, const float* z_all,
                                       int32_t early_stop_count, int32_t poll_every, int32_t* state, const int32_t* out_idx,
                                       int32_t n_out, float* f1, adf_frames_t sink, int32_t frame_every, void* stream) {
+    leave_split(h);
     if (!sink) { adf_set_error("tr_sample_traj: null sink"); return ADF_EINVAL; }
     return adf_model_tr_sample(model(h), b, pos, tags, coefs_dev, num_steps, z_all, early_stop_count, poll_every, state,
                                out_idx, n_out, f1, sink, frame_every, (hipStream_t)stream);
 }
 
-extern "C" int32_t adf_get_counters(adf_painn_t h, adf_counters* out, void* stream) {
-    if (!h || !out || h->lastN <= 0) { adf_set_error("no forward has run"); return ADF_EINVAL; }
+extern "C" int32_t adf_sample_split(adf_painn_t h, adf_painn_t t, const adf_batch* b, const adf_split_view* v, float* pos,
+                                    const int32_t* tags, const int32_t* fixed, const adf_step_coef* coefs_dev,
+                                    int32_t num_steps, const float* z_tr_all, const float* z_rot_all,
+                                    int32_t early_stop_count, int32_t poll_every, int32_t* state, const int32_t* out_idx,
+                                    int32_t n_out, float* f1, float* f2, void* stream) {
+    ADF_TRY(check_batch(h, b));
+    if (!t || t->parent != h) { adf_set_error("sample_split: the second handle is not this handle's twin"); return ADF_EINVAL; }
+    hipStream_t s = (hipStream_t)stream;
+    const bool per_system = h->ps_state != nullptr;
+    const bool split = h->tune.sample_split && b->num_systems >= 2 && !h->gemm_f32 && !(early_stop_count > 0 && !per_system);
+    if (!split) {
+        leave_split(h);
+        ++h->split_fallbacks;
+        return adf_model_sample(model(h), b, pos, tags, fixed, coefs_dev, num_steps, z_tr_all, z_rot_all, early_stop_count,
+                                poll_every, state, out_idx, n_out, f1, f2, nullptr, 0, s);
+    }
+    const int32_t B = b->num_systems, N = b->num_atoms;
+    if (!v || v->cut <= 0 || v->cut >= B || v->atoms_a <= 0 || v->atoms_a >= N || !v->atom_offset || !v->batch) {
+        adf_set_error("sample_split: the view does not cut the batch into two non-empty sides");
+        return ADF_EINVAL;
+    }
+    if (!pos || !tags || !f1 || !f2 || !state || num_steps <= 0) { adf_set_error("sample_split: bad argument"); return ADF_EINVAL; }
+    if (out_idx && (v->n_out_a < 0 || v->n_out_b < 0 || v->n_out_a + v->n_out_b != n_out || (v->n_out_b > 0 && !v->out_idx))) {
+        adf_set_error("sample_split: the view's share of out_idx does not add up to n_out = %d", (int)n_out);
+        return ADF_EINVAL;
+    }
+    if (h->moving && (!v->mov_idx || !v->mov_off)) { adf_set_error("sample_split: a static-atom promise is in force and the view has no moving lists"); return ADF_EINVAL; }
+    if (per_system && h->ps_B != B) { adf_set_error("per-system stop is set for %d systems, the batch has %d", (int)h->ps_B, (int)B); return ADF_EINVAL; }
+    const int32_t cut = v->cut, NA = v->atoms_a;
+    if (!h->split_last || h->split_cut != cut || h->split_N != N) { h->cache_valid = false; h->rec0_valid = false; h->inc_valid = false; }
+    h->split_last = true; h->split_cut = cut; h->split_N = N;
+    follow_settings(t, h);
+    const int32_t* movB = h->moving ? h->moving + NA : nullptr;
+    if (t->seen_moving_serial != h->moving_serial || t->moving != movB ||
+        (movB && (t->mov_idx != v->mov_idx || t->mov_off != v->mov_off))) {
+        ADF_TRY(adf_graph_set_moving(t, h->moving ? h->moving + NA : nullptr, h->moving ? v->mov_idx : nullptr,
+                                     h->moving ? v->mov_off : nullptr));
+        t->seen_moving_serial = h->moving_serial;
+    }
+    if (t->seen_inc_serial != h->inc_set_serial || t->inc_on != h->inc_on) {
+        ADF_TRY(adf_painn_set_incremental(t, h->inc_on ? 1 : 0));
+        t->seen_inc_serial = h->inc_set_serial;
+    }
+    if (!per_system && num_steps > t->split_hist_cap) {
+        ADF_HIP_CHECK(hipDeviceSynchronize());
+        t->split_hist_cap = 0;
+        ADF_TRY(t->m_life.alloc(&t->split_hist, (size_t)2 * num_steps));
+        t->split_hist_cap = num_steps;
+    }
+    adf_batch bA = *b, bB = *b;
+    bA.num_systems = cut; bA.num_atoms = NA;
+    bB.num_systems = B - cut; bB.num_atoms = N - NA;
+    bB.pos = b->pos + 3 * (size_t)NA; bB.cell = b->cell + 9 * (size_t)cut;
+    bB.atomic_numbers = b->atomic_numbers ? b->atomic_numbers + NA : nullptr;
+    bB.batch = v->batch; bB.atom_offset = v->atom_offset;
+    adf_model mA = model(h), mB = model(t);
+    if (per_system) { mA.sys_B = cut; mB.sys_state = h->ps_state + 4 * (size_t)cut; mB.sys_B = B - cut; }
+    else { mB.sys_state = nullptr; mB.sys_B = 0; }
+    adf_split_side A = {&bA, pos, tags, fixed, out_idx, out_idx ? v->n_out_a : 0, f1, f2, state,
+                        per_system ? nullptr : t->split_hist, 0, s};
+    adf_split_side Bv = {&bB, pos + 3 * (size_t)NA, tags + NA, fixed ? fixed + NA : nullptr, out_idx ? v->out_idx : nullptr,
+                         out_idx ? v->n_out_b : 0, f1 + 3 * (size_t)NA, f2 + 3 * (size_t)NA, t->split_state,
+                         per_system ? nullptr : t->split_hist + t->split_hist_cap, cut, (hipStream_t)t->split_stream};
+    ++h->split_runs;
+    return adf_model_sample_split(mA, mB, A, Bv, coefs_dev, num_steps, z_tr_all, z_rot_all, B, early_stop_count, poll_every,
+                                  t->split_state + 8, (hipEvent_t)t->split_ev[0], (hipEvent_t)t->split_ev[1]);
+}
+
+static int32_t handle_counters(adf_painn* h, adf_counters* out, void* stream) {
     hipStream_t s = (hipStream_t)stream;
     const int64_t N = h->lastN, H = h->hp.hidden_channels, R = h->hp.num_rbf, L = h->hp.num_layers;
     int32_t e = 0;
@@ -1071,3 +1256,18 @@
     out->inc_msg_launches = (int64_t)h->inc_launches; out->inc_msg_edges = (int64_t)h->inc_edges;
     return ADF_OK;
 }
+
+extern "C" int32_t adf_get_counters(adf_painn_t h, adf_counters* out, void* stream) {
+    if (!h || !out || h->lastN <= 0) { adf_set_error("no forward has run"); return ADF_EINVAL; }
+    ADF_TRY(handle_counters(h, out, stream));
+    if (!h->twin || h->twin->lastN <= 0) return ADF_OK;
+    adf_counters c;
+    ADF_TRY(handle_counters(h->twin, &c, stream));
+    if (h->split_last) {
+        out->num_edges += c.num_edges; out->num_atoms += c.num_atoms;
+        out->message_bytes_per_layer += c.message_bytes_per_layer; out->dense_flops += c.dense_flops;
+    }
+    out->inc_rows += c.inc_rows; out->inc_rows_full += c.inc_rows_full;
+    out->inc_msg_launches += c.inc_msg_launches; out->inc_msg_edges += c.inc_msg_edges;
+    return ADF_OK;
+}
diff --git a/adsorbdiff_amd/csrc/base.h b/adsorbdiff_amd/csrc/base.h
--- a/adsorbdiff_amd/csrc/base.h
+++ b/adsorbdiff_amd/csrc/base.h
@@ -6,6 +6,7 @@
 #include <vector>
 
 #include "../../include/adsorbdiff_hip.h"
+#include "../../include/adsorbdiff_split.h"
 
 void adf_set_error(const char* fmt, ...);
 
diff --git a/adsorbdiff_amd/csrc/common.h b/adsorbdiff_amd/csrc/common.h
--- a/adsorbdiff_amd/csrc/common.h
+++ b/adsorbdiff_amd/csrc/common.h
@@ -168,6 +168,17 @@
     int num_cus;
     adf_prof prof;
     unsigned long long* kcount;
+    adf_painn* twin;
+    adf_painn* parent;
+    bool split_last;
+    int32_t split_cut; int64_t split_N;
+    unsigned long long split_runs, split_fallbacks;
+    unsigned long long moving_serial, inc_set_serial;
+    unsigned long long seen_moving_serial, seen_inc_serial;
+    void* split_stream;
+    void* split_ev[2];
+    int32_t* split_state;
+    int32_t* split_hist; int64_t split_hist_cap;
     adf_pool m_life;
     adf_pool m_ws;
     adf_pool m_inc;
@@ -246,7 +257,8 @@
 int32_t adf_stepper_step(float* sys, const adf_batch* b, float* pos, const int32_t* tags, const int32_t* fixed,
                          const float* f1, const float* f2, const adf_step_coef* coef, const adf_step_coef* coefs_dev,
                          int num_steps, const float* z_tr, const float* z_rot, int32_t early_stop_count,
-                         int32_t* state, float* dcom, float* drot, hipStream_t s, int32_t* sys_state = nullptr);
+                         int32_t* state, float* dcom, float* drot, hipStream_t s, int32_t* sys_state = nullptr,
+                         int32_t* hist_t = nullptr);
 int32_t adf_stepper_tr_step(float* sys, const adf_batch* b, float* pos, const int32_t* tags, const float* f1,
                             const adf_tr_coef* coef, const adf_tr_coef* coefs_dev, int num_steps, const float* z,
                             int32_t early_stop_count, int32_t* state, float* dcom, hipStream_t s,
@@ -269,7 +281,7 @@
 int32_t adf_model_sde_step(const adf_model& m, const adf_batch* b, float* pos, const int32_t* tags, const int32_t* fixed,
                            const float* f1, const float* f2, const adf_step_coef* coef, const adf_step_coef* coefs_dev,
                            int32_t num_steps, const float* z_tr, const float* z_rot, int32_t early_stop_count,
-                           int32_t* state, float* dcom, float* drot, hipStream_t s);
+                           int32_t* state, float* dcom, float* drot, hipStream_t s, int32_t* hist_t = nullptr);
 int32_t adf_model_tr_step(const adf_model& m, const adf_batch* b, float* pos, const int32_t* tags, const float* f1,
                           const adf_tr_coef* coef, const adf_tr_coef* coefs_dev, int32_t num_steps, const float* z,
                           int32_t early_stop_count, int32_t* state, float* dcom, hipStream_t s);
@@ -281,3 +293,22 @@
                             const adf_tr_coef* coefs_dev, int32_t num_steps, const float* z_all, int32_t early_stop_count,
                             int32_t poll_every, int32_t* state, const int32_t* out_idx, int32_t n_out, float* f1,
                             adf_frames* sink, int32_t frame_every, hipStream_t s);
+
+struct adf_split_side {
+    const adf_batch* b;
+    float* pos;
+    const int32_t* tags;
+    const int32_t* fixed;
+    const int32_t* out_idx;
+    int32_t n_out;
+    float* f1;
+    float* f2;
+    int32_t* state;
+    int32_t* hist;
+    int32_t sys0;
+    hipStream_t s;
+};
+int32_t adf_model_sample_split(const adf_model& mA, const adf_model& mB, adf_split_side A, adf_split_side B,
+                               const adf_step_coef* coefs_dev, int32_t num_steps, const float* z_tr_all,
+                               const float* z_rot_all, int32_t total_systems, int32_t early_stop_count, int32_t poll_every,
+                               int32_t* state_init, hipEvent_t fork, hipEvent_t join);
diff --git a/adsorbdiff_amd/csrc/stepper.hip b/adsorbdiff_amd/csrc/stepper.hip
--- a/adsorbdiff_amd/csrc/stepper.hip
+++ b/adsorbdiff_amd/csrc/stepper.hip
@@ -1,3 +1,5 @@
+#include <stdlib.h>
+
 #include "common.h"
 
 struct StepParams {
@@ -168,6 +170,10 @@
     }
 }
 
+__global__ void adf_step_keep_flag_kernel(const int32_t* state, int32_t* hist_t) {
+    if (threadIdx.x == 0 && blockIdx.x == 0) *hist_t = state[2];
+}
+
 __global__ __launch_bounds__(64) void adf_step_apply_kernel(StepParams p) {
     if (p.state[1]) return;
     const int b = blockIdx.x, lane = threadIdx.x;
@@ -241,7 +247,7 @@
 int32_t adf_stepper_step(float* sys, const adf_batch* b, float* pos, const int32_t* tags, const int32_t* fixed,
                          const float* f1, const float* f2, const adf_step_coef* coef, const adf_step_coef* coefs_dev,
                          int num_steps, const float* z_tr, const float* z_rot, int32_t early_stop_count,
-                         int32_t* state, float* dcom, float* drot, hipStream_t s, int32_t* sys_state) {
+                         int32_t* state, float* dcom, float* drot, hipStream_t s, int32_t* sys_state, int32_t* hist_t) {
     StepParams p;
     p.cell = b->cell; p.atom_offset = b->atom_offset; p.tags = tags; p.fixed = fixed; p.pos = pos;
     p.f1 = f1; p.f2 = f2; p.z_tr = z_tr; p.z_rot = z_rot; p.sys = sys; p.state = state;
@@ -255,6 +261,7 @@
         return ADF_OK;
     }
     hipLaunchKernelGGL(adf_step_reduce_kernel, dim3(p.B), dim3(64), 0, s, p);
+    if (hist_t) hipLaunchKernelGGL(adf_step_keep_flag_kernel, dim3(1), dim3(64), 0, s, state, hist_t);
     hipLaunchKernelGGL(adf_step_decide_kernel, dim3(1), dim3(64), 0, s, state, early_stop_count);
     hipLaunchKernelGGL(adf_step_apply_kernel, dim3(p.B), dim3(64), 0, s, p);
     ADF_HIP_CHECK(hipGetLastError());
@@ -400,7 +407,7 @@
 int32_t adf_model_sde_step(const adf_model& m, const adf_batch* b, float* pos, const int32_t* tags, const int32_t* fixed,
                            const float* f1, const float* f2, const adf_step_coef* coef, const adf_step_coef* coefs_dev,
                            int32_t num_steps, const float* z_tr, const float* z_rot, int32_t early_stop_count,
-                           int32_t* state, float* dcom, float* drot, hipStream_t s) {
+                           int32_t* state, float* dcom, float* drot, hipStream_t s, int32_t* hist_t) {
     ADF_TRY(m.check(m.h, b));
     if (!pos || !tags || !f1 || !f2 || (!coef && !coefs_dev) || !state) { adf_set_error("null argument"); return ADF_EINVAL; }
     if (!coef && num_steps <= 0) { adf_set_error("num_steps must be positive"); return ADF_EINVAL; }
@@ -409,7 +416,7 @@
     ADF_TRY(m.grow(m.h, b, &sys));
     m.prof(m.h, true, s);
     const int32_t st = adf_stepper_step(sys, b, pos, tags, fixed, f1, f2, coef, coef ? nullptr : coefs_dev, num_steps, z_tr,
-                                        z_rot, early_stop_count, state, dcom, drot, s, m.sys_state);
+                                        z_rot, early_stop_count, state, dcom, drot, s, m.sys_state, hist_t);
     m.prof(m.h, false, s);
     return st;
 }
@@ -481,6 +488,97 @@
                        });
 }
 
+__global__ void adf_split_combine_kernel(int32_t* st, const int32_t* sb, const int32_t* init, const int32_t* hist_a,
+                                         const int32_t* hist_b, int steps, int B, int per_system) {
+    if (threadIdx.x != 0 || blockIdx.x != 0) return;
+    if (per_system) {
+        st[0] = st[0] + sb[0] - init[0];
+        st[1] = st[0] >= B ? 1 : 0;
+        st[3] = max(st[3], sb[3]);
+        return;
+    }
+    int both = 0;
+    for (int t = 0; t < steps; ++t) both += (hist_a[t] != 0 && hist_b[t] != 0) ? 1 : 0;
+    st[0] = init[0] + both;
+}
+
+int32_t adf_model_sample_split(const adf_model& mA, const adf_model& mB, adf_split_side A, adf_split_side B,
+                               const adf_step_coef* coefs_dev, int32_t num_steps, const float* z_tr_all,
+                               const float* z_rot_all, int32_t total_systems, int32_t early_stop_count, int32_t poll_every,
+                               int32_t* state_init, hipEvent_t fork, hipEvent_t join) {
+    ADF_TRY(mA.check(mA.h, A.b));
+    ADF_TRY(mB.check(mB.h, B.b));
+    if (num_steps <= 0 || !coefs_dev || !A.state || !B.state || !state_init || !A.f1 || !A.f2 || !A.pos || !A.tags) {
+        adf_set_error("sample_split: bad argument");
+        return ADF_EINVAL;
+    }
+    if ((z_tr_all == nullptr) != (z_rot_all == nullptr)) { adf_set_error("sample_split: need both noise tables or none"); return ADF_EINVAL; }
+    ADF_TRY(check_per_system(mA, A.b));
+    ADF_TRY(check_per_system(mB, B.b));
+    const bool per_system = mA.sys_state != nullptr;
+    if (!per_system && (!A.hist || !B.hist)) { adf_set_error("sample_split: no step history"); return ADF_EINVAL; }
+    ADF_HIP_CHECK(hipMemcpyAsync(state_init, A.state, 8 * sizeof(int32_t), hipMemcpyDeviceToDevice, A.s));
+    ADF_HIP_CHECK(hipEventRecord(fork, A.s));
+    ADF_HIP_CHECK(hipStreamWaitEvent(B.s, fork, 0));
+    ADF_HIP_CHECK(hipMemcpyAsync(B.state, state_init, 8 * sizeof(int32_t), hipMemcpyDeviceToDevice, B.s));
+    const size_t z_stride = (size_t)total_systems * 3;
+    auto one = [&](const adf_model& m, const adf_split_side& v, int t) -> int32_t {
+        ADF_TRY(m.forward(m.h, v.b, v.out_idx, v.out_idx ? v.n_out : 0, v.f1, v.f2, v.s));
+        const size_t z = (size_t)t * z_stride + (size_t)v.sys0 * 3;
+        return adf_model_sde_step(m, v.b, v.pos, v.tags, v.fixed, v.f1, v.f2, nullptr, coefs_dev, num_steps,
+                                  z_tr_all ? z_tr_all + z : nullptr, z_rot_all ? z_rot_all + z : nullptr, early_stop_count,
+                                  v.state, nullptr, nullptr, v.s, per_system ? nullptr : v.hist + t);
+    };
+    int32_t st = ADF_OK;
+    int steps = 0;
+    for (int t = 0; t < num_steps && st == ADF_OK; ++t) {
+        st = one(mA, A, t);
+        if (st == ADF_OK) st = one(mB, B, t);
+        if (st != ADF_OK) break;
+        steps = t + 1;
+        if (early_stop_count > 0 && poll_every > 0 && (t % poll_every) == poll_every - 1 && t + 1 < num_steps) {
+            int32_t fa = 0, fb = 0;
+            if (hipMemcpyAsync(&fa, A.state + 1, sizeof(int32_t), hipMemcpyDeviceToHost, A.s) != hipSuccess ||
+                hipMemcpyAsync(&fb, B.state + 1, sizeof(int32_t), hipMemcpyDeviceToHost, B.s) != hipSuccess ||
+                hipStreamSynchronize(A.s) != hipSuccess || hipStreamSynchronize(B.s) != hipSuccess) {
+                adf_set_error("sample_split: reading the frozen flags failed: %s", hipGetErrorString(hipGetLastError()));
+                st = ADF_EHIP;
+                break;
+            }
+            if (fa && fb) break;
+        }
+    }
+    if (hipEventRecord(join, B.s) != hipSuccess || hipStreamWaitEvent(A.s, join, 0) != hipSuccess) {
+        if (st == ADF_OK) { adf_set_error("sample_split: join failed: %s", hipGetErrorString(hipGetLastError())); st = ADF_EHIP; }
+        return st;
+    }
+    if (st != ADF_OK) return st;
+    hipLaunchKernelGGL(adf_split_combine_kernel, dim3(1), dim3(64), 0, A.s, A.state, B.state, state_init, A.hist, B.hist,
+                       steps, total_systems, per_system ? 1 : 0);
+    ADF_HIP_CHECK(hipGetLastError());
+    return ADF_OK;
+}
+
+extern "C" int32_t adf_split_choose_cut(const int32_t* natoms, const int64_t* edges, int32_t num_systems, int32_t* cut) {
+    if (!natoms || !cut || num_systems < 0) { adf_set_error("split_choose_cut: bad argument"); return ADF_EINVAL; }
+    *cut = 0;
+    if (num_systems < 2) return ADF_OK;
+    long long total = 0, etotal = 0;
+    for (int b = 0; b < num_systems; ++b) {
+        if (natoms[b] < 0 || (edges && edges[b] < 0)) { adf_set_error("split_choose_cut: negative count at system %d", b); return ADF_EINVAL; }
+        total += natoms[b];
+        if (edges) etotal += edges[b];
+    }
+    long long best = -1, best_e = -1, a = 0, e = 0;
+    for (int c = 1; c < num_systems; ++c) {
+        a += natoms[c - 1];
+        if (edges) e += edges[c - 1];
+        const long long d = llabs(2 * a - total), de = edges ? llabs(2 * e - etotal) : 0;
+        if (best < 0 || d < best || (d == best && de < best_e)) { best = d; best_e = de; *cut = c; }
+    }
+    return ADF_OK;
+}
+
 __global__ __launch_bounds__(64) void adf_lift_kernel(float* pos, const int32_t* tags, const int32_t* atom_offset,
                                                        float min_gap, float* lifted) {
     const int b = blockIdx.x, lane = threadIdx.x;
diff --git a/adsorbdiff_amd/denoising_torch.py b/adsorbdiff_amd/denoising_torch.py
--- a/adsorbdiff_amd/denoising_torch.py
+++ b/adsorbdiff_amd/denoising_torch.py
@@ -227,7 +227,7 @@
                         zt[t_idx].normal_()
                         zr[t_idx].normal_()
                 eng.sample(prep, pos, f1, f2, coefs_dev, T, state, zt, zr, early_stop_count=early, poll_every=poll_every,
-                           out_idx=out_idx, sink=sink, frame_every=1)
+                           out_idx=out_idx, sink=sink, frame_every=1, split_streams=params.get("split_streams"))
 
             def per_step(f1, state, out_idx):
                 f2 = torch.zeros(N, 3, dtype=torch.float32, device=dev)
diff --git a/adsorbdiff_amd/engine.py b/adsorbdiff_amd/engine.py
--- a/adsorbdiff_amd/engine.py
+++ b/adsorbdiff_amd/engine.py
@@ -56,6 +56,7 @@
     reps: List[int]
     tags: Optional[torch.Tensor] = None
     fixed: Optional[torch.Tensor] = None
+    edge_counts: Optional[Sequence[int]] = None
 
     def desc(self, pos: torch.Tensor) -> _lib.BatchDesc:
         d = _lib.BatchDesc()
@@ -71,6 +72,18 @@
 
 def image_repeats(batch, cutoff: float) -> List[int]:
     return cell_repeats(batch.cell, float(cutoff), batch_pbc(batch))
+
+
+def split_cut(natoms: Sequence[int], edges: Optional[Sequence[int]] = None) -> int:
+    n = (C.c_int32 * max(len(natoms), 1))(*[int(x) for x in natoms])
+    e = None
+    if edges is not None:
+        if len(edges) != len(natoms):
+            raise ValueError(f"split_cut: {len(natoms)} atom counts, {len(edges)} edge counts")
+        e = (C.c_int64 * max(len(edges), 1))(*[int(x) for x in edges])
+    cut = C.c_int32(-1)
+    _lib.check(_lib.load().adf_split_choose_cut(n, e, len(natoms), C.byref(cut)))
+    return int(cut.value)
 
 
 def _require_gpu(t: torch.Tensor, what: str) -> None:
@@ -225,7 +238,8 @@
 
     def sample(self, prep: PreparedBatch, pos, f1, f2, coefs_dev: torch.Tensor, num_steps: int, state,
                z_tr_all=None, z_rot_all=None, early_stop_count: int = 10, poll_every: int = 0,
-               out_idx: Optional[torch.Tensor] = None, sink=None, frame_every: int = 1) -> None:
+               out_idx: Optional[torch.Tensor] = None, sink=None, frame_every: int = 1,
+               split_streams: Optional[bool] = None) -> None:
         self._loop("sample", prep, pos, [_ptr(prep.fixed), coefs_dev.data_ptr(), num_steps, _ptr(z_tr_all),
                                          _ptr(z_rot_all), early_stop_count, poll_every, state.data_ptr(), _ptr(out_idx),
                                          _numel(out_idx), f1.data_ptr(), f2.data_ptr()], sink, frame_every)
@@ -262,6 +276,10 @@
         if getattr(self, "handle", None) is not None and self.handle:
             with torch.cuda.device(self.device):
                 torch.cuda.synchronize(self.device)
+                twin = getattr(self, "_twin", None)
+                if twin is not None and twin:
+                    self._c("destroy")(twin)
+                    self._twin = None
                 self._c("destroy")(self.handle)
             self.handle = None
 
@@ -294,6 +312,11 @@
         with torch.cuda.device(self.device):
             _lib.check(self.lib.adf_painn_create(C.byref(hp), C.byref(self.handle)))
         self._last_graph_N = 0
+        self._twin = None
+        self._split_keepalive = None
+        self._moving_gen = 0
+        self._split_moving = None
+        self._split_default = bool(self.get_tune()["sample_split"])
         floor = getattr(model, "distance_floor", None)
         if floor is not None:
             _lib.check(self.lib.adf_painn_set_distance_floor(self.handle, float(floor)))
@@ -345,6 +368,60 @@
             with torch.cuda.device(self.device):
                 _lib.check(self.lib.adf_painn_set_energy_head(self.handle, 4, eptrs, self._stream()))
 
+    def set_moving_atoms(self, prep, moving_mask) -> None:
+        self._moving_gen += 1
+        super().set_moving_atoms(prep, moving_mask)
+
+    def split_view(self, prep: PreparedBatch, out_idx: Optional[torch.Tensor]):
+        cached = getattr(prep, "_split_cut", None)
+        if cached is None:
+            off = prep.atom_offset.cpu()
+            cut = split_cut((off[1:] - off[:-1]).tolist(), prep.edge_counts)
+            na = int(off[cut])
+            cached = prep._split_cut = (cut, na, (prep.atom_offset[cut:] - na).contiguous(), (prep.batch[na:] - cut).contiguous())
+        cut, na, off_b, batch_b = cached
+        v = _lib.SplitView()
+        v.cut, v.atoms_a, v.atom_offset, v.batch = cut, na, off_b.data_ptr(), batch_b.data_ptr()
+        keep = [off_b, batch_b]
+        if out_idx is not None:
+            n_a = int((out_idx < na).sum().item())
+            keep.append((out_idx[n_a:] - na).contiguous())
+            v.n_out_a, v.n_out_b, v.out_idx = n_a, int(out_idx.numel()) - n_a, keep[-1].data_ptr()
+        if self._moving_keepalive is not None:
+            if self._split_moving is None or self._split_moving[0] != (self._moving_gen, cut, na):
+                _, idx, moff = self._moving_keepalive
+                m0 = int(moff[cut].item())
+                self._split_moving = ((self._moving_gen, cut, na), (idx[m0:] - na).contiguous(), (moff[cut:] - m0).contiguous())
+            v.mov_idx, v.mov_off = self._split_moving[1].data_ptr(), self._split_moving[2].data_ptr()
+        return v, keep
+
+    def split_stats(self):
+        a, b = C.c_int64(0), C.c_int64(0)
+        _lib.check(self.lib.adf_split_stats(self.handle, C.byref(a), C.byref(b)))
+        return int(a.value), int(b.value)
+
+    def sample(self, prep: PreparedBatch, pos, f1, f2, coefs_dev: torch.Tensor, num_steps: int, state,
+               z_tr_all=None, z_rot_all=None, early_stop_count: int = 10, poll_every: int = 0,
+               out_idx: Optional[torch.Tensor] = None, sink=None, frame_every: int = 1,
+               split_streams: Optional[bool] = None) -> None:
+        want = self._split_default if split_streams is None else bool(split_streams)
+        if not want or sink is not None or prep.num_systems < 2:
+            return super().sample(prep, pos, f1, f2, coefs_dev, num_steps, state, z_tr_all, z_rot_all, early_stop_count,
+                                  poll_every, out_idx, sink, frame_every)
+        with torch.cuda.device(self.device):
+            if self._twin is None:
+                twin = C.c_void_p()
+                _lib.check(self.lib.adf_painn_create_twin(self.handle, C.byref(twin)))
+                self._twin = twin
+            _lib.check(self.lib.adf_painn_set_split(self.handle, 1))
+            view, keep = self.split_view(prep, out_idx)
+            self._split_keepalive = keep
+            desc = prep.desc(pos)
+            _lib.check(self.lib.adf_sample_split(
+                self.handle, self._twin, C.byref(desc), C.byref(view), pos.data_ptr(), prep.tags.data_ptr(), _ptr(prep.fixed),
+                coefs_dev.data_ptr(), num_steps, _ptr(z_tr_all), _ptr(z_rot_all), early_stop_count, poll_every,
+                state.data_ptr(), _ptr(out_idx), _numel(out_idx), f1.data_ptr(), f2.data_ptr(), self._stream()))
+
     def forward_prepared(self, prep: PreparedBatch, pos: torch.Tensor, f1: torch.Tensor, f2: Optional[torch.Tensor],
                          out_idx: Optional[torch.Tensor] = None) -> None:
         desc = prep.desc(pos)
diff --git a/adsorbdiff_amd/lib.py b/adsorbdiff_amd/lib.py
--- a/adsorbdiff_amd/lib.py
+++ b/adsorbdiff_amd/lib.py
@@ -39,7 +39,13 @@
 class Tune(C.Structure):
     _fields_ = [(name, C.c_int32) for name in (
         "gemm_stream", "head_gate_fused", "lift_emit", "graph_sys_csr", "train_gemm16", "wgrad_f32",
-        "eqv2_gemm_tile256", "eqv2_rotin_generic", "eqv2_rotout_generic")]
+        "eqv2_gemm_tile256", "eqv2_rotin_generic", "eqv2_rotout_generic", "sample_split")]
+
+
+class SplitView(C.Structure):
+    _fields_ = [("cut", C.c_int32), ("atoms_a", C.c_int32), ("n_out_a", C.c_int32), ("n_out_b", C.c_int32),
+                ("atom_offset", C.c_void_p), ("batch", C.c_void_p), ("out_idx", C.c_void_p), ("mov_idx", C.c_void_p),
+                ("mov_off", C.c_void_p)]
 
 
 class BatchDesc(C.Structure):
@@ -122,6 +128,9 @@
 
 SIGNATURES = parse_header(HEADER.read_text())
 EXPORTS = tuple(SIGNATURES)
+SPLIT_HEADER = HEADER.with_name("adsorbdiff_split.h")
+SPLIT_SIGNATURES = {name: sig for name, sig in parse_header(HEADER.read_text() + "\n" + SPLIT_HEADER.read_text()).items()
+                    if name not in SIGNATURES}
 
 _LIB = None
 
@@ -146,7 +155,7 @@
             "(the HIP path has no CPU fallback)"
         )
     lib = C.CDLL(str(path))
-    for name, (restype, argtypes) in SIGNATURES.items():
+    for name, (restype, argtypes) in {**SIGNATURES, **SPLIT_SIGNATURES}.items():
         fn = getattr(lib, name)
         fn.restype, fn.argtypes = restype, argtypes
     _LIB = lib
diff --git a/include/adsorbdiff_hip.h b/include/adsorbdiff_hip.h
--- a/include/adsorbdiff_hip.h
+++ b/include/adsorbdiff_hip.h
@@ -66,6 +66,7 @@
     int32_t eqv2_gemm_tile256;
     int32_t eqv2_rotin_generic;
     int32_t eqv2_rotout_generic;
+    int32_t sample_split;
 } adf_tune;
 int32_t adf_painn_get_tune(adf_painn_t h, adf_tune* out);
 
diff --git a/include/adsorbdiff_split.h b/include/adsorbdiff_split.h
--- /dev/null
+++ b/include/adsorbdiff_split.h
@@ -0,0 +1,40 @@
+#ifndef ADSORBDIFF_SPLIT_H
+#define ADSORBDIFF_SPLIT_H
+
+#include "adsorbdiff_hip.h"
+
+#ifdef __cplusplus
+extern "C" {
+#endif
+
+typedef struct adf_painn* adf_painn_t;
+
+int32_t adf_painn_create_twin(adf_painn_t parent, adf_painn_t* out);
+
+int32_t adf_painn_set_split(adf_painn_t h, int32_t on);
+
+int32_t adf_split_choose_cut(const int32_t* natoms, const int64_t* edges, int32_t num_systems, int32_t* cut);
+
+typedef struct {
+    int32_t cut;
+    int32_t atoms_a;
+    int32_t n_out_a;
+    int32_t n_out_b;
+    const int32_t* atom_offset;
+    const int32_t* batch;
+    const int32_t* out_idx;
+    const int32_t* mov_idx;
+    const int32_t* mov_off;
+} adf_split_view;
+
+int32_t adf_sample_split(adf_painn_t h, adf_painn_t twin, const adf_batch* b, const adf_split_view* view, float* pos,
+                         const int32_t* tags, const int32_t* fixed, const adf_step_coef* coefs_dev, int32_t num_steps,
+                         const float* z_tr_all, const float* z_rot_all, int32_t early_stop_count, int32_t poll_every,
+                         int32_t* state, const int32_t* out_idx, int32_t n_out, float* f1, float* f2, void* stream);
+
+int32_t adf_split_stats(adf_painn_t h, int64_t* split_runs, int64_t* fallback_runs);
+
+#ifdef __cplusplus
+}
+#endif
+#endif
```

Result: faster. 253.2 (median of 6 runs) (+1.2%).
